# joejep/FOCNeRF

Measured on AMD Instinct MI355X. Metric: train_samples_per_sec, higher is better.
Workload: dtype f16

## Files before the change

focnerf_amd/_lib.py:

```python
import ctypes
import os

import torch

_HERE = os.path.dirname(os.path.abspath(__file__))
LIB_PATH = os.environ.get("FOCNERF_LIB_PATH") or os.path.join(_HERE, "libfocnerf_hip.so")

c_u8p = ctypes.c_void_p
c_vp = ctypes.c_void_p
u32 = ctypes.c_uint32
u64 = ctypes.c_uint64
f32 = ctypes.c_float
f64 = ctypes.c_double
i32 = ctypes.c_int

FOC_F32 = 0
FOC_F16 = 1
FOC_U8 = 2


class FocOccTrainNode(ctypes.Structure):
    _fields_ = [
        ("struct_bytes", u32),
        ("n_rays", u32), ("max_steps", u32), ("cascade", u32), ("grid_size", u32), ("cap", u32), ("pad_align", u32),
# ... 33 lines not shown
        ("ray_sumsq", c_vp),
        ("grad_sumsq", c_vp),
        ("grad_obj", c_vp),
    ]


class FocOccTrainTail(ctypes.Structure):
    _fields_ = [
        ("struct_bytes", u32),
        ("ray_dist", c_vp), ("ray_wm", c_vp), ("depth_raw", c_vp),
        ("grad_dist", c_vp), ("grad_depth", c_vp),
    ]


class FocCulledField(ctypes.Structure):
    _fields_ = [
        ("mask", c_vp), ("offsets", c_vp), ("sigma_c", c_vp), ("rgb_c", c_vp),
        ("m_occ", u32), ("density_scale", f32), ("thresh", f32), ("sigma_gain", f32),
    ]


class FocOptimTensor(ctypes.Structure):
    _fields_ = [
        ("param", c_vp), ("grad", c_vp), ("exp_avg", c_vp), ("exp_avg_sq", c_vp), ("step", c_vp),
        ("lr_tensor", c_vp),
        ("n", ctypes.c_int64),
        ("lr", f64), ("beta1", f64), ("beta2", f64), ("eps", f64), ("weight_decay", f64),
    ]


class FocOptimStep(ctypes.Structure):
    _fields_ = [
        ("struct_bytes", u32),
        ("tensor_bytes", u32),
        ("n_tensors", ctypes.c_int32),
        ("phase", u32), ("zero_grads", u32),
        ("growth_interval", ctypes.c_int32),
        ("growth_factor", f32), ("backoff_factor", f32),
        ("tensors", ctypes.POINTER(FocOptimTensor)),
        ("scale", c_vp),
        ("growth_tracker", c_vp),
        ("grad_scale", c_vp), ("found_inf", c_vp),
        ("workspace", c_vp),
        ("workspace_bytes", u64),
    ]


SIGNATURES = {
    "foc_abi_version": (i32, []),
    "foc_last_error": (ctypes.c_char_p, []),
    "foc_arch": (ctypes.c_char_p, []),
    "foc_near_far_from_aabb": (i32, [c_vp, c_vp, c_vp, u32, f32, c_vp, c_vp, c_vp]),
    "foc_sph_from_ray": (i32, [c_vp, c_vp, f32, u32, c_vp, c_vp]),
    "foc_morton3D": (i32, [c_vp, u32, c_vp, c_vp]),
    "foc_morton3D_invert": (i32, [c_vp, u32, c_vp, c_vp]),
    "foc_packbits": (i32, [c_vp, u32, f32, c_vp, c_vp]),
    "foc_march_rays_train": (i32, [c_vp, c_vp, c_vp, f32, f32, u32, u32, u32, u32, u32, c_vp, c_vp,
                                   c_vp, c_vp, c_vp, c_vp, c_vp, c_vp, c_vp, c_vp]),
    "foc_march_rays_train_field": (i32, [c_vp, c_vp, c_vp, f32, f32, u32, u32, u32, u32, u32, c_vp, c_vp,
                                         c_vp, c_vp, c_vp, c_vp, c_vp, c_vp, c_vp, u32, c_vp, f32, c_vp]),
    "foc_set_option": (i32, [ctypes.c_char_p, i32]),
    "foc_get_option": (i32, [ctypes.c_char_p, c_vp]),
    "foc_guard_pick_device": (i32, [i32, i32, i32, i32]),
    "foc_grid_forward_index_path": (i32, [u32, u32, u32]),
    "foc_view_tile_order": (i32, [c_vp, u32, u32, u32, c_vp, c_vp, c_vp]),
    "foc_occ_train_forward": (i32, [ctypes.POINTER(FocOccTrainNode), c_vp]),
    "foc_occ_train_backward": (i32, [ctypes.POINTER(FocOccTrainNode), c_vp]),
    "foc_occ_train_forward_pad31": (i32, [ctypes.POINTER(FocOccTrainNode), f32, c_vp]),
    "foc_occ_train_backward_pad31": (i32, [ctypes.POINTER(FocOccTrainNode), f32, c_vp]),
    "foc_occ_train_forward_obj": (i32, [ctypes.POINTER(FocOccTrainNode), ctypes.POINTER(FocOccTrainObject), c_vp]),
    "foc_occ_train_backward_obj": (i32, [ctypes.POINTER(FocOccTrainNode), ctypes.POINTER(FocOccTrainObject), c_vp]),
    "foc_occ_tail_forward_sumsq": (i32, [c_vp, c_vp, u32, c_vp, c_vp, u32, u32, f32, f32, c_vp, f32, c_vp, c_vp, c_vp, c_vp, c_vp, c_vp, c_vp, c_vp]),
    "foc_occ_tail_backward_sumsq": (i32, [c_vp, c_vp, c_vp, c_vp, u32, c_vp, c_vp, c_vp, c_vp, c_vp, u32, u32, f32, f32, c_vp, f32, c_vp, c_vp, c_vp, c_vp]),
    "foc_occ_tail_forward": (i32, [c_vp, c_vp, u32, c_vp, c_vp, u32, u32, f32, f32, c_vp, f32, c_vp, c_vp, c_vp, c_vp, c_vp, c_vp, c_vp]),
    "foc_occ_tail_backward": (i32, [c_vp, c_vp, c_vp, c_vp, u32, c_vp, c_vp, c_vp, c_vp, c_vp, u32, u32, f32, f32, c_vp, f32, c_vp, c_vp, c_vp]),
    "foc_occ_tail_forward_dist": (i32, [c_vp, c_vp, u32, c_vp, c_vp, u32, u32, f32, f32, c_vp, f32, c_vp, c_vp, c_vp, c_vp, c_vp, c_vp, c_vp, c_vp, c_vp,
                                        c_vp]),
    "foc_occ_tail_backward_dist": (i32, [c_vp, c_vp, c_vp, c_vp, u32, c_vp, c_vp, c_vp, c_vp, c_vp, u32, u32, f32, f32, c_vp, f32, c_vp, c_vp, c_vp, c_vp,
                                         c_vp, c_vp, c_vp]),
    "foc_occ_tail_forward_depth": (i32, [c_vp, c_vp, u32, c_vp, c_vp, u32, u32, f32, f32, c_vp, f32, c_vp, c_vp, c_vp, c_vp, c_vp, c_vp, c_vp, c_vp, c_vp,
                                         c_vp, c_vp]),
    "foc_occ_tail_backward_depth": (i32, [c_vp, c_vp, c_vp, c_vp, u32, c_vp, c_vp, c_vp, c_vp, c_vp, u32, u32, f32, f32, c_vp, f32, c_vp, c_vp, c_vp, c_vp,
                                          c_vp, c_vp, c_vp, c_vp, c_vp, c_vp, c_vp]),
    "foc_occ_train_forward_tail": (i32, [ctypes.POINTER(FocOccTrainNode), ctypes.POINTER(FocOccTrainObject), f32, ctypes.POINTER(FocOccTrainTail), c_vp]),
    "foc_occ_train_backward_tail": (i32, [ctypes.POINTER(FocOccTrainNode), ctypes.POINTER(FocOccTrainObject), f32, ctypes.POINTER(FocOccTrainTail), c_vp]),
    "foc_march_rays_train_scratch_bytes": (u64, [u32, u32]),
    "foc_composite_rays_train_forward": (i32, [c_vp, c_vp, c_vp, c_vp, u32, u32, f32, c_vp, c_vp, c_vp, c_vp]),
    "foc_composite_rays_train_backward": (i32, [c_vp, c_vp, c_vp, c_vp, c_vp, c_vp, c_vp, c_vp, u32, u32, f32,
                                                c_vp, c_vp, c_vp]),
    "foc_march_rays": (i32, [u32, u32, c_vp, c_vp, c_vp, c_vp, f32, f32, u32, u32, u32, c_vp, c_vp, c_vp,
                             c_vp, c_vp, c_vp, c_vp, c_vp]),
    "foc_composite_rays": (i32, [u32, u32, f32, c_vp, c_vp, c_vp, c_vp, c_vp, c_vp, c_vp, c_vp, c_vp]),
    "foc_compact_alive": (i32, [c_vp, u32, c_vp, c_vp, c_vp, c_vp]),
    "foc_march_rays_two_phase": (i32, [u32, u32, c_vp, c_vp, c_vp, c_vp, f32, f32, u32, u32, u32, c_vp, c_vp, c_vp, c_vp, c_vp, c_vp, c_vp, c_vp, i32, c_vp]),
    "foc_composite_compact": (i32, [u32, u32, f32, c_vp, c_vp, c_vp, c_vp, c_vp, c_vp, c_vp, c_vp, c_vp, c_vp, c_vp, c_vp, u32, u32, i32, c_vp]),
    "foc_march_rays_two_phase_fills": (i32, [u32, i32]),
    "foc_march_rays_two_phase_sample_major": (i32, [u32, u32, i32]),
    "foc_occ_render_step_scratch_bytes": (u64, [u32]),
    "foc_occ_render_step": (i32, [u32, u32, c_vp, c_vp, c_vp, c_vp, c_vp, c_vp, f32, f32, u32, u32, u32, c_vp, c_vp, c_vp, c_vp, c_vp, c_vp, c_vp, c_vp,
                                  c_vp, c_vp, c_vp, u32, f32, u32, c_vp, u32, c_vp, u32, u32, c_vp, f32, c_vp, c_vp, c_vp, c_vp, u32, c_vp, u32, u32, c_vp]),
    "foc_occ_render_step_pad31": (i32, [u32, u32, c_vp, c_vp, c_vp, c_vp, c_vp, c_vp, f32, f32, u32, u32, u32, c_vp, c_vp, c_vp, c_vp, c_vp, c_vp, c_vp, c_vp,
                                        c_vp, c_vp, c_vp, u32, f32, u32, c_vp, u32, c_vp, u32, u32, c_vp, f32, c_vp, c_vp, c_vp, c_vp, u32, c_vp, u32, u32, f32,
                                        c_vp]),
    "foc_occ_render_step_pad": (i32, [u32, u32, c_vp, c_vp, c_vp, c_vp, c_vp, c_vp, f32, f32, u32, u32, u32, c_vp, c_vp, c_vp, c_vp, c_vp, c_vp, c_vp, c_vp,
                                      c_vp, c_vp, c_vp, u32, f32, u32, c_vp, u32, c_vp, u32, u32, c_vp, f32, c_vp, c_vp, c_vp, c_vp, u32, c_vp, u32, u32, f32,
                                      c_vp]),
    "foc_grid_encode_forward": (i32, [c_vp, c_vp, c_vp, c_vp, u32, u32, u32, u32, f32, u32, c_vp, u32, i32, u32,
                                      i32, c_vp, c_vp]),
    "foc_grid_encode_forward_bl": (i32, [c_vp, c_vp, c_vp, c_vp, u32, u32, u32, u32, f32, u32, c_vp, u32, i32, u32,
                                         i32, c_vp, c_vp]),
    "foc_grid_encode_backward": (i32, [c_vp, c_vp, c_vp, c_vp, c_vp, u32, u32, u32, u32, f32, u32, c_vp, c_vp,
                                       u32, i32, u32, i32, i32, c_vp, c_vp]),
    "foc_grid_encode_backward_workspace_bytes": (u64, [u32, u32, u32, u32, i32]),
    "foc_grid_planes_to_rows": (i32, [c_vp, c_vp, u32, u32, u32, c_vp]),
    "foc_grid_rows_to_planes": (i32, [c_vp, c_vp, u32, u32, u32, c_vp]),
    "foc_grid_encode_backward_binned": (i32, [c_vp, c_vp, c_vp, c_vp, c_vp, u32, u32, u32, u32, f32, u32, c_vp, c_vp,
                                              u32, i32, u32, i32, i32, c_vp, c_vp, u64, c_vp]),
    "foc_grid_encode_forward_counted": (i32, [c_vp, c_vp, c_vp, c_vp, u32, u32, u32, u32, f32, u32, u32, i32, u32, i32, c_vp, c_vp, u64, c_vp]),
    "foc_grid_encode_backward_count": (i32, [c_vp, c_vp, u32, u32, u32, u32, f32, u32, u32, i32, u32, i32, c_vp, c_vp, u64, c_vp]),
    "foc_grid_encode_backward_binned_counted": (i32, [c_vp, c_vp, c_vp, c_vp, c_vp, u32, u32, u32, u32, f32, u32, c_vp, c_vp,
                                                      u32, i32, u32, i32, i32, c_vp, c_vp, u64, c_vp]),
    "foc_grad_total_variation": (i32, [c_vp, c_vp, c_vp, c_vp, f32, u32, u32, u32, u32, f32, u32, u32, i32, i32, c_vp]),
    "foc_freq_encode_forward": (i32, [c_vp, u32, u32, u32, u32, c_vp, c_vp]),
    "foc_freq_encode_backward": (i32, [c_vp, c_vp, u32, u32, u32, u32, c_vp, c_vp]),
    "foc_ffmlp_forward": (i32, [c_vp, c_vp, u32, u32, u32, u32, u32, u32, u32, c_vp, c_vp, c_vp]),
    "foc_ffmlp_inference": (i32, [c_vp, c_vp, u32, u32, u32, u32, u32, u32, u32, c_vp, c_vp, c_vp]),
    "foc_ffmlp_backward": (i32, [c_vp, c_vp, c_vp, c_vp, u32, u32, u32, u32, u32, u32, u32, i32,
                                 c_vp, c_vp, c_vp, c_vp, u64, c_vp]),
    "foc_ffmlp_backward_workspace_bytes": (u64, [u32, u32, u32]),
    "foc_ffmlp_forward_planar": (i32, [c_vp, c_vp, u32, u32, u32, u32, u32, u32, u32, c_vp, c_vp]),
    "foc_ffmlp_backward_planar": (i32, [c_vp, c_vp, c_vp, u32, u32, u32, u32, u32, u32, u32, i32, c_vp, c_vp, c_vp, u64, c_vp]),
    "foc_allocate_splitk": (i32, [u64]),
    "foc_free_splitk": (i32, []),
    "foc_combine_select": (i32, [c_vp, c_vp, c_vp, c_vp, u64, c_vp]),
    "foc_combine_pack_keys": (i32, [c_vp, u32, c_vp, u64, c_vp]),
    "foc_combine_unpack": (i32, [c_vp, u32, c_vp, c_vp, c_vp, u64, c_vp]),
    "foc_combine_select_composite": (i32, [c_vp, u32, c_vp, c_vp, u32, u32, c_vp, u32, c_vp, c_vp, c_vp, c_vp]),
    "foc_combine_select4": (i32, [c_vp, c_vp, u64, c_vp]),
    "foc_combine_select_composite_attr": (i32, [c_vp, u32, c_vp, c_vp, u32, c_vp, c_vp, u32, u32, c_vp, u32, c_vp, c_vp, c_vp, c_vp, c_vp, c_vp, c_vp, c_vp]),
    "foc_combine_select_composite_culled": (i32, [ctypes.POINTER(FocCulledField), u32, u32, c_vp, u32, c_vp, c_vp, u32, u32, c_vp, u32, c_vp, c_vp, c_vp, c_vp,
                                                  c_vp, c_vp, c_vp, c_vp]),
    "foc_combine_select4_ids": (i32, [c_vp, u32, c_vp, c_vp, u64, c_vp]),
    "foc_mo_select": (i32, [c_vp, c_vp, c_vp, c_vp, u64, u32, u32, c_vp]),
    "foc_fixed_field_pack": (i32, [c_vp, c_vp, c_vp, c_vp, c_vp, c_vp, f32, u32, u32, f32, f32, c_vp, c_vp, c_vp, c_vp, u32, c_vp]),
    "foc_fixed_cull_scratch_bytes": (u64, [u32, u32]),
    "foc_fixed_cull": (i32, [c_vp, c_vp, c_vp, c_vp, c_vp, u32, u32, f32, c_vp, u32, u32, c_vp, c_vp, c_vp, c_vp, u64, c_vp]),
    "foc_fixed_cull_emit": (i32, [c_vp, c_vp, c_vp, c_vp, c_vp, u32, u32, f32, c_vp, c_vp, u32, c_vp, c_vp, c_vp]),
    "foc_fixed_field_pack_culled": (i32, [c_vp, c_vp, c_vp, c_vp, u32, c_vp, c_vp, u32, u32, f32, f32, c_vp, c_vp]),
    "foc_fixed_cull_placed": (i32, [c_vp, c_vp, c_vp, c_vp, c_vp, u32, u32, c_vp, c_vp, f32, c_vp, u32, u32, c_vp, c_vp, c_vp, c_vp, u64, c_vp]),
    "foc_fixed_cull_emit_placed": (i32, [c_vp, c_vp, c_vp, c_vp, c_vp, u32, u32, c_vp, f32, f32, c_vp, c_vp, u32, c_vp, c_vp, c_vp]),
    "foc_fixed_field_pack_culled_gain": (i32, [c_vp, c_vp, c_vp, c_vp, u32, c_vp, c_vp, u32, u32, f32, f32, f32, c_vp, c_vp]),
    "foc_composite_fixed_steps":(i32, [c_vp, c_vp, c_vp, c_vp, u32, u32, f32, c_vp, c_vp, c_vp]),
    "foc_fixed_sample": (i32, [c_vp, c_vp, c_vp, c_vp, c_vp, c_vp, u32, u32, f32, c_vp, c_vp, c_vp, u32, c_vp]),
    "foc_fixed_tail_forward": (i32, [c_vp, c_vp, c_vp, c_vp, c_vp, c_vp, f32, u32, u32, f32, f32, c_vp, c_vp, c_vp, c_vp, c_vp, c_vp, u32, c_vp, c_vp]),
    "foc_fixed_tail_backward": (i32, [c_vp, c_vp, c_vp, c_vp, c_vp, c_vp, c_vp, c_vp, c_vp, c_vp, c_vp, f32, u32, u32, f32, f32, c_vp, c_vp, u32, c_vp, c_vp]),
    "foc_fixed_tail_forward_dist": (i32, [c_vp, c_vp, c_vp, c_vp, c_vp, c_vp, f32, u32, u32, f32, f32, c_vp, c_vp, c_vp, c_vp, c_vp, c_vp, u32, c_vp, c_vp,
                                          c_vp, c_vp]),
    "foc_fixed_tail_backward_dist": (i32, [c_vp, c_vp, c_vp, c_vp, c_vp, c_vp, c_vp, c_vp, c_vp, c_vp, c_vp, c_vp, f32, u32, u32, f32, f32, c_vp, c_vp, u32,
                                           c_vp, c_vp, c_vp, c_vp, c_vp]),
    "foc_fixed_head_forward": (i32, [c_vp, c_vp, c_vp, c_vp, c_vp, u32, u32, f32, c_vp, c_vp, c_vp, c_vp, c_vp, c_vp, c_vp, u32, c_vp]),
    "foc_fixed_head_backward": (i32, [c_vp, c_vp, c_vp, c_vp, c_vp, c_vp, c_vp, c_vp, c_vp, c_vp, u32, u32, f32, c_vp, u32, c_vp]),
    "foc_color_head_forward": (i32, [c_vp, c_vp, u32, c_vp, u32, u32, u32, u32, c_vp, u32, c_vp, c_vp]),
    "foc_field_forward_train": (i32, [c_vp, c_vp, u32, c_vp, u32, c_vp, u32, u32, u32, u32, c_vp, c_vp, u32, c_vp, c_vp]),
    "foc_color_head_backward": (i32, [c_vp, c_vp, c_vp, u32, c_vp, c_vp, u32, u32, u32, u32, c_vp, c_vp, c_vp, u64, u32, c_vp, c_vp, c_vp]),
    "foc_color_head_forward_pad": (i32, [c_vp, c_vp, u32, c_vp, u32, u32, u32, u32, c_vp, u32, c_vp, f32, c_vp]),
    "foc_color_head_backward_pad": (i32, [c_vp, c_vp, c_vp, u32, c_vp, c_vp, u32, u32, u32, u32, c_vp, c_vp, c_vp, u64, u32, c_vp, c_vp, f32, c_vp]),
    "foc_field_forward_train_pad": (i32, [c_vp, c_vp, u32, c_vp, u32, c_vp, u32, u32, u32, u32, c_vp, c_vp, u32, c_vp, f32, c_vp]),
    "foc_color_head_forward_pad31": (i32, [c_vp, c_vp, u32, c_vp, u32, u32, u32, u32, c_vp, u32, c_vp, f32, c_vp]),
    "foc_color_head_backward_pad31": (i32, [c_vp, c_vp, c_vp, u32, c_vp, c_vp, u32, u32, u32, u32, c_vp, c_vp, c_vp, u64, u32, c_vp, c_vp, f32, c_vp]),
    "foc_field_forward_train_pad31": (i32, [c_vp, c_vp, u32, c_vp, u32, c_vp, u32, u32, u32, u32, c_vp, c_vp, u32, c_vp, f32, c_vp]),
    "foc_fixed_composite_forward": (i32, [c_vp, c_vp, c_vp, f32, u32, u32, f32, c_vp, c_vp]),
    "foc_fixed_composite_backward": (i32, [c_vp, c_vp, c_vp, c_vp, f32, u32, u32, f32, c_vp, c_vp, c_vp]),
    "foc_sample_head_forward": (i32, [c_vp, c_vp, u64, c_vp, c_vp, c_vp, u32, c_vp]),
    "foc_sample_head_backward": (i32, [c_vp, c_vp, c_vp, u64, c_vp, u32, c_vp]),
    "foc_sh_encode": (i32, [c_vp, u64, c_vp, c_vp]),
    "foc_rgb_head_forward": (i32, [c_vp, u64, c_vp, c_vp]),
    "foc_rgb_head_backward": (i32, [c_vp, c_vp, u64, c_vp, c_vp]),
    "foc_fixed_render_inference": (i32, [c_vp, c_vp, c_vp, c_vp, c_vp, c_vp, f32, u32, u32, f32, f32, c_vp, c_vp, c_vp, c_vp, u32, c_vp, c_vp]),
    "foc_nerf_field_inference": (i32, [c_vp, i32, c_vp, u32, u32, u32, c_vp, u32, c_vp, u32, u32, u32, u32, c_vp, c_vp, c_vp, c_vp]),
    "foc_nerf_field_inference_pad": (i32, [c_vp, i32, c_vp, u32, u32, u32, c_vp, u32, c_vp, u32, u32, u32, u32, c_vp, c_vp, c_vp, f32, c_vp]),
    "foc_nerf_field_inference_pad31": (i32, [c_vp, i32, c_vp, u32, u32, u32, c_vp, u32, c_vp, u32, u32, u32, u32, c_vp, c_vp, c_vp, f32, c_vp]),
    "foc_field_normals": (i32, [c_vp, u32, c_vp, c_vp, u32, u32, u32, f32, u32, u32, i32, u32, i32, c_vp, c_vp, u32, u32, u32, c_vp, c_vp, c_vp, c_vp, c_vp,
                                c_vp]),
    "foc_mark_untrained_grid": (i32, [c_vp, u32, f32, f32, f32, f32, f32, u32, u32, c_vp, c_vp, c_vp]),
    "foc_grid_cells_xyz": (i32, [u32, u32, f32, c_vp, c_vp, c_vp]),
    "foc_grid_update_sample_workspace_bytes": (u64, [u32, u32]),
    "foc_grid_update_sample": (i32, [c_vp, u32, u32, f32, u32, c_vp, c_vp, c_vp, c_vp, c_vp, c_vp, u64, c_vp]),
    "foc_grid_update_apply_workspace_bytes": (u64, [u32, u32]),
    "foc_grid_update_apply": (i32, [c_vp, u32, u32, c_vp, c_vp, u32, f32, f32, f32, c_vp, c_vp, c_vp, u64, c_vp]),
    "foc_background_forward": (i32, [c_vp, c_vp, c_vp, f32, u32, c_vp, c_vp, f32, u32, c_vp, c_vp, c_vp]),
    "foc_background_backward_workspace_bytes": (u64, [u32]),
    "foc_background_backward": (i32, [c_vp, c_vp, c_vp, c_vp, f32, u32, c_vp, c_vp, f32, u32, c_vp, c_vp, c_vp, c_vp, u64, c_vp]),
    "foc_mc_workspace_bytes": (u64, [u32, u32, u32]),
    "foc_mc_count": (i32, [c_vp, u32, u32, u32, f32, c_vp, c_vp, c_vp]),
    "foc_mc_emit": (i32, [c_vp, u32, u32, u32, f32, c_vp, c_vp, c_vp, c_vp, c_vp, c_vp, c_vp]),
    "foc_lattice_cull_scratch_bytes": (u64, [u32]),
    "foc_lattice_cull": (i32, [c_vp, c_vp, c_vp, u32, u32, u32, u32, u32, c_vp, c_vp, f32, c_vp, u32, u32, c_vp, c_vp, c_vp, c_vp, u64, c_vp]),
    "foc_lattice_cull_emit": (i32, [c_vp, c_vp, c_vp, u32, u32, u32, u32, u32, c_vp, c_vp, c_vp, u32, c_vp, c_vp]),
    "foc_volume_scatter_max": (i32, [c_vp, c_vp, c_vp, f32, c_vp, u32, c_vp]),
    "foc_score_workspace_bytes": (u64, [u32, u32, u32]),
    "foc_score_quantize": (i32, [c_vp, c_vp, c_vp, c_vp, u32, u32, u32, c_vp, c_vp, c_vp, c_vp]),
    "foc_score_view": (i32, [c_vp, c_vp, u32, u32, u32, c_vp, u32, f64, f64, c_vp, c_vp, u64, c_vp]),
    "foc_optim_workspace_bytes": (ctypes.c_size_t, [i32]),
    "foc_optim_step": (i32, [ctypes.POINTER(FocOptimStep), c_vp]),
    "foc_philox4x32_10": (i32, [ctypes.POINTER(u32), ctypes.POINTER(u32), ctypes.POINTER(u32)]),
    "foc_batch_workspace_bytes": (u64, []),
    "foc_batch_sample": (i32, [c_vp, i32, u32, u32, u32, u32, c_vp, f32, f32, f32, f32, c_vp, c_vp, u64, u32, c_vp, i32, i32, c_vp, c_vp, c_vp, c_vp, c_vp, c_vp,
                               c_vp, u64, u32, c_vp]),
    "foc_view_rays": (i32, [c_vp, f32, f32, f32, f32, u32, u32, c_vp, c_vp, c_vp]),
    "foc_photo_loss_workspace_bytes": (u64, []),
    "foc_photo_loss": (i32, [c_vp, i32, c_vp, u32, i32, f32, c_vp, u32, c_vp, c_vp, c_vp, c_vp, c_vp, c_vp, u64, c_vp]),
}


def _load():
    if not os.path.exists(LIB_PATH):
        raise ImportError(
            f"focnerf_amd: {LIB_PATH} is missing. Build it with `python -c 'import __graft_entry__ as g; g.build()'` "
            f"or `make -C focnerf_amd/csrc`. There is no CPU or PyTorch fallback for these ops.")
    try:
        lib = ctypes.CDLL(LIB_PATH)
    except OSError as e:
        raise ImportError(f"focnerf_amd: failed to load {LIB_PATH}: {e}") from e
    for name, (res, args) in SIGNATURES.items():
        fn = getattr(lib, name)
        fn.restype = res
        fn.argtypes = args
    return lib


class _Stream(ctypes.c_void_p):
    device_index = None


_multi_device = None


def _on_tensor_device(fn):
    def call(*args):
        global _multi_device
        if _multi_device is None:
            _multi_device = torch.cuda.device_count() > 1
        if _multi_device and args:
            idx = getattr(args[-1], "device_index", None)
            if idx is not None and idx != torch.cuda.current_device():
                with torch.cuda.device(idx):
                    return fn(*args)
        return fn(*args)
    call.__name__ = getattr(fn, "__name__", "foc_call")
    return call


class _Lib:

    def __init__(self, cdll):
        self._cdll = cdll
        for name, (_, args) in SIGNATURES.items():
            fn = getattr(cdll, name)
            setattr(self, name, _on_tensor_device(fn) if args and args[-1] is c_vp and not name.endswith("_bytes") else fn)


lib = _Lib(_load())


def check(rc, what=""):
    if rc != 0:
        msg = lib.foc_last_error().decode("utf-8", "replace")
        raise RuntimeError(f"focnerf_amd {what}: {msg} (code {rc})")


def ptr(t):
    if t is None:
        return None
    return ctypes.c_void_p(t.data_ptr())


_raw_stream = getattr(torch._C, "_cuda_getCurrentRawStream", None) if os.environ.get("FOC_RAW_STREAM", "1") != "0" else None


def raw_stream(index):
    if _raw_stream is not None:
        return _raw_stream(index)
    return torch.cuda.current_stream(index).cuda_stream


def stream_of(t=None):
    dev = t.device if t is not None else None
    index = dev.index if dev is not None and dev.index is not None else torch.cuda.current_device()
    s = _Stream(raw_stream(index))
    s.device_index = index
    return s


def require_cuda(*tensors):
    for t in tensors:
        if t is not None and not t.is_cuda:
            raise RuntimeError("focnerf_amd: expected a CUDA(HIP) tensor; these ops have no CPU implementation")


def dtype_code(t):
    if t.dtype == torch.float32:
        return FOC_F32
    if t.dtype == torch.float16:
        return FOC_F16
    raise RuntimeError(f"focnerf_amd: unsupported dtype {t.dtype} (float32 or float16 expected)")


def get_option(name):
# ... 23 lines not shown
```

focnerf_amd/csrc/combine.hip:

```cpp
#include "common.h"
#include "fs_common.h"
#include <string.h>
#include <cmath>

static thread_local char g_err[512] = "";

void foc_set_error(const char *fmt, ...) {
    va_list ap;
    va_start(ap, fmt);
    vsnprintf(g_err, sizeof(g_err), fmt, ap);
    va_end(ap);
}

__global__ void __launch_bounds__(256) k_combine_select(const float *__restrict__ dens, const float *__restrict__ rgb,
                                                        float *__restrict__ max_dens, float *__restrict__ best_rgb, uint64_t n) {
    for (uint64_t i = (uint64_t)blockIdx.x * 256 + threadIdx.x; i < n; i += (uint64_t)gridDim.x * 256) {
        const float d = dens[i], m = max_dens[i];
        if (d > m) { best_rgb[i * 3] = rgb[i * 3]; best_rgb[i * 3 + 1] = rgb[i * 3 + 1]; best_rgb[i * 3 + 2] = rgb[i * 3 + 2]; }
        max_dens[i] = (d != d || m != m) ? __builtin_nanf("") : (d > m ? d : m);
    }
}

__global__ void __launch_bounds__(256) k_combine_pack(const float *__restrict__ dens, uint32_t rank, uint64_t *__restrict__ keys, uint64_t n) {
    for (uint64_t i = (uint64_t)blockIdx.x * 256 + threadIdx.x; i < n; i += (uint64_t)gridDim.x * 256) {
// ... 207 lines not shown
template <int KMAX> struct CulledObjs { CulledObj o[KMAX]; };

#define CC_NO_BIT 0xFFFFFFFFu
template <int KMAX, int NOBJ>
__global__ void __launch_bounds__(256) k_combine_culled(CulledObjs<KMAX> objs, CombineAttr at, uint32_t K, const float *__restrict__ nears,
                                                        const float *__restrict__ fars, uint32_t N, uint32_t T, float bg0, float bg1, uint32_t n_bg,
                                                        float *__restrict__ image4, float *__restrict__ depth, float4 *__restrict__ merged4) {
    const uint32_t lane = threadIdx.x & 63;
    const uint32_t n = __builtin_amdgcn_readfirstlane(blockIdx.x * 4 + (threadIdx.x >> 6));
    if (n >= N) return;
    const FsGeom geo = fs_geom(nears, fars, n, T);
    const uint32_t bit = n % FS_RAY_BLOCK;
    const uint64_t below = (1ull << bit) - 1ull;
    const uint64_t row0 = (uint64_t)(n / FS_RAY_BLOCK) * T;
    CombineAcc<NOBJ> A;
    combine_acc_init(A);
    float Tk[KMAX];
#pragma unroll
    for (int k = 0; k < KMAX; k++) Tk[k] = 1.0f;
    for (uint32_t base = 0; base < T; base += 64) {
        const uint32_t i = base + lane;
        const bool valid = i < T;
        const uint32_t ic = valid ? i : T - 1;
        const uint64_t row = row0 + ic, s = (uint64_t)n * T + ic;
        const FsSample p = fs_sample(geo, i, ic, T, false, 0.0f, 0.0f);
        uint32_t pre[KMAX];
        bool any = false, plain = fabsf(p.delta) < INFINITY && p.oz == p.oz;
#pragma unroll
        for (int k = 0; k < KMAX; k++) {
            pre[k] = CC_NO_BIT;
            if ((uint32_t)k < K) {
                const uint64_t m = objs.o[k].mask[row];
                if (valid && ((m >> bit) & 1ull)) { pre[k] = (uint32_t)__popcll(m & below); any = true; }
                plain = plain && fabsf(p.delta * objs.o[k].density_scale) < INFINITY;
            }
        }
        if (__ballot(any || !plain) == 0 && fabsf(A.Tc) < INFINITY) {
            if (valid) {
                uint32_t win = 0xFFu;
                if constexpr (NOBJ > 0) win = at.id[0];
                combine_store<NOBJ>(make_float4(0.0f, 0.0f, 0.0f, 0.0f), win, s, merged4, &at);
            }
            continue;
        }
        float4 best = make_float4(0.0f, 0.0f, 0.0f, 0.0f);
        uint32_t win = 0xFFu;
#pragma unroll
        for (int k = 0; k < KMAX; k++) {
            if ((uint32_t)k < K) {
                const CulledObj &o = objs.o[k];
                float sigma = 0, c0 = 0, c1 = 0, c2 = 0;
                if (pre[k] != CC_NO_BIT) {
                    const uint32_t slot = o.offsets[row] + pre[k];
                    if (slot < o.m_occ) {
                        sigma = o.sigma_c[slot];
                        if (o.sigma_gain != 1.0f) sigma *= o.sigma_gain;
                        c0 = o.rgb_c[(uint64_t)slot * 3]; c1 = o.rgb_c[(uint64_t)slot * 3 + 1]; c2 = o.rgb_c[(uint64_t)slot * 3 + 2];
                    }
                }
                const bool on = fs_infer_weight(Tk[k], p, valid, sigma, o.density_scale, lane) > o.thresh;
                const float4 f = make_float4(sigma, on ? c0 : 0.0f, on ? c1 : 0.0f, on ? c2 : 0.0f);
                if (k == 0) {
                    best = f;
                    if constexpr (NOBJ > 0) win = at.id[0];
                } else {
                    combine_select_step<NOBJ>(best, win, f, at.id[k]);
                }
            }
        }
        CombineSample q = combine_no_sample();
        if (valid) {
            combine_store<NOBJ>(best, win, s, merged4, &at);
            q = combine_take(best, win, p);
        }
        combine_accumulate(A, q, valid, lane);
    }
    combine_finish(A, &at, n, N, lane, bg0, bg1, n_bg, image4, depth);
}

struct CulledLaunch {
    const FocCulledField *objs; uint32_t K; CombineAttr at; const float *nears, *fars; uint32_t N, T; float bg0, bg1; uint32_t n_bg;
    float *image4, *depth; float4 *merged4; hipStream_t stream;
};
template <int KMAX, int NOBJ>
static void cc_launch(const CulledLaunch &L) {
    CulledObjs<KMAX> o;
    memset(&o, 0, sizeof(o));
    for (uint32_t k = 0; k < L.K; k++) {
        const FocCulledField &f = L.objs[k];
        o.o[k] = CulledObj{f.mask, f.offsets, f.sigma_c, f.rgb_c, f.m_occ, f.density_scale, f.thresh, f.sigma_gain};
    }
    hipLaunchKernelGGL((k_combine_culled<KMAX, NOBJ>), dim3(foc_div_up(L.N, 4)), dim3(256), 0, L.stream, o, L.at, L.K, L.nears, L.fars, L.N, L.T, L.bg0,
                       L.bg1, L.n_bg, L.image4, L.depth, L.merged4);
}
template <int KMAX>
static void cc_launch_k(const CulledLaunch &L, uint32_t n_obj) {
    if (n_obj == 0) cc_launch<KMAX, 0>(L);
    else if (n_obj <= 4) cc_launch<KMAX, 4>(L);
    else if (n_obj <= 8) cc_launch<KMAX, 8>(L);
    else cc_launch<KMAX, 16>(L);
}

__global__ void __launch_bounds__(256) k_combine_select4(const float4 *__restrict__ f4, float4 *__restrict__ acc4, uint64_t n) {
    for (uint64_t i = (uint64_t)blockIdx.x * 256 + threadIdx.x; i < n; i += (uint64_t)gridDim.x * 256) {
        const float4 f = f4[i];
        float4 best = acc4[i];
        const float m = best.x;
        if (f.x > m) { best.y = f.y; best.z = f.z; best.w = f.w; }
        best.x = (f.x != f.x || m != m) ? __builtin_nanf("") : (f.x > m ? f.x : m);
        acc4[i] = best;
    }
}

__global__ void __launch_bounds__(256) k_combine_select4_ids(const float4 *__restrict__ f4, uint8_t id, float4 *__restrict__ acc4,
                                                             uint8_t *__restrict__ acc_ids, uint64_t n) {
    for (uint64_t i = (uint64_t)blockIdx.x * 256 + threadIdx.x; i < n; i += (uint64_t)gridDim.x * 256) {
        const float4 f = f4[i];
        float4 best = acc4[i];
        const float m = best.x;
        if (f.x > m) { best.y = f.y; best.z = f.z; best.w = f.w; acc_ids[i] = id; }
        best.x = (f.x != f.x || m != m) ? __builtin_nanf("") : (f.x > m ? f.x : m);
        acc4[i] = best;
    }
}

template <typename T>
__global__ void __launch_bounds__(256) k_mo_select(const T *__restrict__ sig_new, const T *__restrict__ feat_new, T *__restrict__ sig_best,
                                                   T *__restrict__ feat_best, uint64_t n, uint32_t width) {
    const uint64_t s0 = ((uint64_t)blockIdx.x * 4u + (threadIdx.x >> 6)) * 64u;
    if (s0 >= n) return;
    const uint32_t lane = threadIdx.x & 63u;
    bool take = false;
    if (s0 + lane < n) {
        const T a_raw = sig_new[s0 + lane];
        const float a = (float)a_raw, b = (float)sig_best[s0 + lane];
        take = (a != a) || (b == b && a >= b);
        if (take) sig_best[s0 + lane] = a_raw;
    }
    const uint64_t rows = __ballot(take);
    const uint32_t live = (uint32_t)(n - s0 < 64u ? n - s0 : 64u);
    const uint64_t base = s0 * width;
    for (uint32_t e = lane; e < live * width; e += 64u)
        if ((rows >> (e / width)) & 1ull) feat_best[base + e] = feat_new[base + e];
}

#include <stdlib.h>
#include <string.h>
#include <atomic>
#include <mutex>
struct FocOptionRow { const char *name; std::atomic<int> value; };
static FocOptionRow foc_option_table[FOC_OPT_COUNT] = {
    {"FOC_MLP_BWD_FUSED", 1}, {"FOC_FIELD_FWD_FUSED", 1}, {"FOC_GB_MERGE_MAX_RES", 480}, {"FOC_GB_FACTORED", 1}, {"FOC_GB_TAIL_SPLIT", 16}, {"FOC_GRID_FUSE_SMALL", 1},
    {"FOC_GRID_PAIRS", 1}, {"FOC_GRID_FAST", 1}, {"FOC_MARCH_SERIAL", -1}, {"FOC_MARCH_RAYS_ROW_MAX", 131072}, {"FOC_OCC_MARCH_FORM", -1},
    {"FOC_OCC_SAMPLE_MAJOR", 1}, {"FOC_OCC_FIELD_PIECE", 1 << 23}, {"FOC_DETERMINISTIC", 0},
};
static int foc_option_parse(int which, const char *text) {
    if (which == FOC_OPT_OCC_MARCH_FORM) {
        if (text[0] == 't') return 0;
        if (text[0] == 'r') return 1;
        if (text[0] == 'l') return 2;
        if (text[0] == 's') return 3;
    }
    return atoi(text);
}
static void foc_options_init() {
    static std::once_flag once;
    std::call_once(once, [] {
        for (int i = 0; i < FOC_OPT_COUNT; i++) {
            const char *e = getenv(foc_option_table[i].name);
            if (e && e[0]) foc_option_table[i].value.store(foc_option_parse(i, e), std::memory_order_relaxed);
        }
    });
}
int foc_opt(FocOpt which) { foc_options_init(); return foc_option_table[which].value.load(std::memory_order_relaxed); }

extern "C" {

int foc_set_option(const char *name, int value) {
    foc_options_init();
    for (int i = 0; i < FOC_OPT_COUNT; i++)
        if (name && strcmp(name, foc_option_table[i].name) == 0) { foc_option_table[i].value.store(value, std::memory_order_relaxed); return FOC_OK; }
    foc_set_error("set_option: unknown option '%s'", name ? name : "(null)");
    return FOC_E_INVALID;
}

int foc_get_option(const char *name, int *value) {
    foc_options_init();
    for (int i = 0; i < FOC_OPT_COUNT; i++)
        if (name && value && strcmp(name, foc_option_table[i].name) == 0) { *value = foc_option_table[i].value.load(std::memory_order_relaxed); return FOC_OK; }
    foc_set_error("get_option: unknown option '%s'", name ? name : "(null)");
    return FOC_E_INVALID;
}

int foc_guard_pick_device(int stream_is_null, int stream_device, int pointer_device, int current_device) {
    return foc_guard_pick(stream_is_null != 0, stream_device, pointer_device, current_device);
}


int foc_combine_select_composite(const float *const *fields4, uint32_t K, const float *nears, const float *fars, uint32_t N, uint32_t T,
                                 const float *bgs, uint32_t n_bg, float *image4, float *depth, float *merged4, void *stream) {
    FocDeviceGuard foc_guard_(stream, nears);
    FOC_REQUIRE(K >= 1 && K <= FOC_COMBINE_MAX_OBJECTS, FOC_E_INVALID, "combine_select_composite: 1 <= K <= %d objects per call (got %u)",
                FOC_COMBINE_MAX_OBJECTS, K);
    FOC_REQUIRE(n_bg >= 1 && n_bg <= 2 && bgs, FOC_E_INVALID, "combine_select_composite: one or two backgrounds");
    FOC_REQUIRE(T >= 2, FOC_E_INVALID, "combine_select_composite: T must be >= 2");
    if (N == 0) return FOC_OK;
    FOC_REQUIRE(fields4 && nears && fars && image4 && depth, FOC_E_INVALID, "combine_select_composite: null pointer");
    CombineFields f;
    for (uint32_t k = 0; k < FOC_COMBINE_MAX_OBJECTS; k++) {
        f.p[k] = reinterpret_cast<const float4 *>(k < K ? fields4[k] : fields4[0]);
        FOC_REQUIRE(f.p[k] && ((uintptr_t)f.p[k] & 15) == 0, FOC_E_INVALID, "combine_select_composite: field %u is null or not 16-byte aligned", k);
    }
    FOC_REQUIRE(((uintptr_t)merged4 & 15) == 0, FOC_E_INVALID, "combine_select_composite: merged4 must be 16-byte aligned");
    hipLaunchKernelGGL(k_combine_select_composite, dim3(foc_div_up(N, 4)), dim3(256), 0, (hipStream_t)stream, f, K, nears, fars, N, T, bgs[0],
                       n_bg > 1 ? bgs[1] : 0.0f, n_bg, image4, depth, reinterpret_cast<float4 *>(merged4));
    FOC_CHECK_LAUNCH("combine_select_composite");
    return FOC_OK;
}

int foc_combine_select4(const float *field4, float *acc4, uint64_t n, void *stream) {
    FocDeviceGuard foc_guard_(stream, field4);
    FOC_REQUIRE(n == 0 || (field4 && acc4), FOC_E_INVALID, "combine_select4: null pointer");
    FOC_REQUIRE((((uintptr_t)field4 | (uintptr_t)acc4) & 15) == 0, FOC_E_INVALID, "combine_select4: fields must be 16-byte aligned");
    if (n == 0) return FOC_OK;
    hipLaunchKernelGGL(k_combine_select4, dim3(foc_grid_1d(n, 256)), dim3(256), 0, (hipStream_t)stream, reinterpret_cast<const float4 *>(field4),
                       reinterpret_cast<float4 *>(acc4), n);
    FOC_CHECK_LAUNCH("combine_select4");
    return FOC_OK;
}

int foc_combine_select_composite_attr(const float *const *fields4, uint32_t K, const uint8_t *const *id_planes, const uint32_t *ids,
                                      uint32_t n_obj, const float *nears, const float *fars, uint32_t N, uint32_t T, const float *bgs,
                                      uint32_t n_bg, float *image4, float *depth, float *merged4, float *obj_weights, float *obj_depth,
                                      int32_t *instance, uint8_t *winner, void *stream) {
    FocDeviceGuard foc_guard_(stream, nears);
    FOC_REQUIRE(K >= 1 && K <= FOC_COMBINE_MAX_OBJECTS, FOC_E_INVALID, "combine_select_composite_attr: 1 <= K <= %d fields per call (got %u)",
                FOC_COMBINE_MAX_OBJECTS, K);
    FOC_REQUIRE(n_obj >= 1 && n_obj <= FOC_COMBINE_MAX_OBJECTS, FOC_E_INVALID, "combine_select_composite_attr: 1 <= n_obj <= %d objects (got %u)",
                FOC_COMBINE_MAX_OBJECTS, n_obj);
    FOC_REQUIRE(n_bg >= 1 && n_bg <= 2 && bgs, FOC_E_INVALID, "combine_select_composite_attr: one or two backgrounds");
    FOC_REQUIRE(T >= 2, FOC_E_INVALID, "combine_select_composite_attr: T must be >= 2");
    FOC_REQUIRE(fields4, FOC_E_INVALID, "combine_select_composite_attr: fields4 is null");
    CombineFields f;
    CombineAttr at;
    for (uint32_t k = 0; k < FOC_COMBINE_MAX_OBJECTS; k++) {
        const uint32_t j = k < K ? k : 0;
        at.plane[k] = id_planes ? id_planes[j] : nullptr;
        FOC_REQUIRE(at.plane[k] || ids, FOC_E_INVALID, "combine_select_composite_attr: field %u has neither an id plane nor a constant id (ids is null)", j);
        at.id[k] = at.plane[k] ? 0u : ids[j];
        FOC_REQUIRE(at.id[k] < n_obj, FOC_E_INVALID, "combine_select_composite_attr: ids[%u] = %u is not below n_obj = %u", j, at.id[k], n_obj);
    }
    if (N == 0) return FOC_OK;
    FOC_REQUIRE(nears && fars && image4 && depth, FOC_E_INVALID, "combine_select_composite_attr: null pointer");
    FOC_REQUIRE(obj_weights && obj_depth && instance, FOC_E_INVALID, "combine_select_composite_attr: obj_weights, obj_depth and instance must not be null");
    for (uint32_t k = 0; k < FOC_COMBINE_MAX_OBJECTS; k++) {
        f.p[k] = reinterpret_cast<const float4 *>(k < K ? fields4[k] : fields4[0]);
        FOC_REQUIRE(f.p[k] && ((uintptr_t)f.p[k] & 15) == 0, FOC_E_INVALID, "combine_select_composite_attr: field %u is null or not 16-byte aligned", k);
    }
    FOC_REQUIRE(((uintptr_t)merged4 & 15) == 0, FOC_E_INVALID, "combine_select_composite_attr: merged4 must be 16-byte aligned");
    FOC_REQUIRE(((uintptr_t)obj_weights & 3) == 0 && ((uintptr_t)obj_depth & 3) == 0 && ((uintptr_t)instance & 3) == 0, FOC_E_INVALID,
                "combine_select_composite_attr: obj_weights, obj_depth and instance must be 4-byte aligned");
    at.n_obj = n_obj;
    at.obj_weights = obj_weights; at.obj_depth = obj_depth; at.instance = instance; at.winner = winner;
    const dim3 grid(foc_div_up(N, 4)), block(256);
    const float bg1 = n_bg > 1 ? bgs[1] : 0.0f;
    float4 *m4 = reinterpret_cast<float4 *>(merged4);
    if (n_obj <= 4)
        hipLaunchKernelGGL(k_combine_select_composite_attr<4>, grid, block, 0, (hipStream_t)stream, f, at, K, nears, fars, N, T, bgs[0], bg1, n_bg, image4, depth, m4);
    else if (n_obj <= 8)
        hipLaunchKernelGGL(k_combine_select_composite_attr<8>, grid, block, 0, (hipStream_t)stream, f, at, K, nears, fars, N, T, bgs[0], bg1, n_bg, image4, depth, m4);
    else
        hipLaunchKernelGGL(k_combine_select_composite_attr<16>, grid, block, 0, (hipStream_t)stream, f, at, K, nears, fars, N, T, bgs[0], bg1, n_bg, image4, depth, m4);
    FOC_CHECK_LAUNCH("combine_select_composite_attr");
    return FOC_OK;
}

int foc_combine_select_composite_culled(const FocCulledField *objs, uint32_t K, uint32_t struct_bytes, const uint32_t *ids, uint32_t n_obj,
                                        const float *nears, const float *fars, uint32_t N, uint32_t T, const float *bgs, uint32_t n_bg, float *image4,
                                        float *depth, float *merged4, float *obj_weights, float *obj_depth, int32_t *instance, uint8_t *winner,
                                        void *stream) {
    const char *who = "combine_select_composite_culled";
    FocDeviceGuard foc_guard_(stream, nears);
    FOC_REQUIRE(K >= 1 && K <= FOC_COMBINE_MAX_OBJECTS, FOC_E_INVALID, "%s: 1 <= K <= %d objects per call (got %u)", who, FOC_COMBINE_MAX_OBJECTS, K);
    FOC_REQUIRE(struct_bytes == sizeof(FocCulledField), FOC_E_INVALID, "%s: FocCulledField of %u bytes, this library's has %u", who, struct_bytes,
                (uint32_t)sizeof(FocCulledField));
    FOC_REQUIRE(objs, FOC_E_INVALID, "%s: objs is null", who);
    FOC_REQUIRE(n_obj <= FOC_COMBINE_MAX_OBJECTS, FOC_E_INVALID, "%s: n_obj <= %d objects (got %u)", who, FOC_COMBINE_MAX_OBJECTS, n_obj);
    FOC_REQUIRE(n_bg >= 1 && n_bg <= 2 && bgs, FOC_E_INVALID, "%s: one or two backgrounds", who);
    FOC_REQUIRE(T >= 2, FOC_E_INVALID, "%s: T must be >= 2", who);
    FOC_REQUIRE((uint64_t)foc_div_up(N, FS_RAY_BLOCK) * FS_RAY_BLOCK * T < (1ull << 31), FOC_E_INVALID,
                "%s: ceil(N/64)*64*T must stay below 2^31 (foc_fixed_cull's limit)", who);
    CulledLaunch L;
    memset(&L.at, 0, sizeof(L.at));
    for (uint32_t k = 0; k < K; k++) {
        const FocCulledField &f = objs[k];
        FOC_REQUIRE(std::isfinite(f.sigma_gain) && f.sigma_gain > 0, FOC_E_INVALID, "%s: object %u: sigma_gain must be finite and > 0 (got %g)", who, k,
                    (double)f.sigma_gain);
        L.at.id[k] = ids ? ids[k] : k;
        FOC_REQUIRE(n_obj == 0 || L.at.id[k] < n_obj, FOC_E_INVALID, "%s: ids[%u] = %u is not below n_obj = %u", who, k, L.at.id[k], n_obj);
    }
    if (N == 0) return FOC_OK;
    FOC_REQUIRE(nears && fars && image4 && depth, FOC_E_INVALID, "%s: null pointer", who);
    FOC_REQUIRE(n_obj == 0 || (obj_weights && obj_depth && instance), FOC_E_INVALID, "%s: obj_weights, obj_depth and instance must not be null when n_obj > 0", who);
    for (uint32_t k = 0; k < K; k++) {
        const FocCulledField &f = objs[k];
        FOC_REQUIRE(f.mask && f.offsets, FOC_E_INVALID, "%s: object %u: null pointer (mask / offsets)", who, k);
        FOC_REQUIRE(f.m_occ == 0 || (f.sigma_c && f.rgb_c), FOC_E_INVALID, "%s: object %u: null sigma / rgb with %u occupied samples", who, k, f.m_occ);
// ... 93 lines not shown
```

focnerf_amd/csrc/common.h:

```cpp
#pragma once
#include <hip/hip_runtime.h>
#include <hip/hip_fp16.h>
#include <stdint.h>
#include <stdio.h>
#include <stdarg.h>
#include <map>
#include <mutex>
#include <tuple>
#include "../../include/focnerf.h"

#define FOC_WAVE 64

void foc_set_error(const char *fmt, ...);

enum FocOpt {
    FOC_OPT_MLP_BWD_FUSED,
    FOC_OPT_FIELD_FWD_FUSED,
    FOC_OPT_GB_MERGE_MAX_RES,
    FOC_OPT_GB_FACTORED,
    FOC_OPT_GB_TAIL_SPLIT,
    FOC_OPT_GRID_FUSE_SMALL,
    FOC_OPT_GRID_PAIRS,
    FOC_OPT_GRID_FAST,
    FOC_OPT_MARCH_SERIAL,
    FOC_OPT_MARCH_RAYS_ROW_MAX,
    FOC_OPT_OCC_MARCH_FORM,
    FOC_OPT_OCC_SAMPLE_MAJOR,
    FOC_OPT_OCC_FIELD_PIECE,
    FOC_OPT_DETERMINISTIC,
    FOC_OPT_COUNT
};
int foc_opt(FocOpt which);

#define FOC_REQUIRE(cond, code, ...)                    \
    do {                                                \
        if (!(cond)) {                                  \
            foc_set_error(__VA_ARGS__);                 \
            return (code);                              \
        }                                               \
    } while (0)

#define FOC_CHECK_LAUNCH(name)                                                     \
    do {                                                                           \
        hipError_t e_ = hipGetLastError();                                         \
        if (e_ != hipSuccess) {                                                    \
            foc_set_error("%s: launch failed: %s", name, hipGetErrorString(e_));   \
            return FOC_E_LAUNCH;                                                   \
        }                                                                          \
    } while (0)

static inline int foc_guard_pick(bool stream_is_null, int stream_device, int pointer_device, int current_device) {
    if (!stream_is_null && stream_device >= 0) return stream_device;
    if (pointer_device >= 0) return pointer_device;
    return current_device;
}
struct FocDeviceGuard {
    int prev = -1;
    explicit FocDeviceGuard(void *stream, const void *first_pointer = nullptr) {
        static int n_devices = -1;
        if (n_devices < 0 && hipGetDeviceCount(&n_devices) != hipSuccess) { (void)hipGetLastError(); n_devices = 0; }
        if (n_devices == 1) return;
        int cur = 0;
        if (hipGetDevice(&cur) != hipSuccess) return;
        int sdev = -1, pdev = -1;
        if (stream != nullptr) {
            if (hipStreamGetDevice(static_cast<hipStream_t>(stream), &sdev) != hipSuccess) { (void)hipGetLastError(); sdev = -1; }
        } else if (first_pointer != nullptr) {
            hipPointerAttribute_t attr;
            if (hipPointerGetAttributes(&attr, first_pointer) == hipSuccess && attr.type == hipMemoryTypeDevice) pdev = attr.device;
            else (void)hipGetLastError();
        }
        const int want = foc_guard_pick(stream == nullptr, sdev, pdev, cur);
        if (want != cur && hipSetDevice(want) == hipSuccess) prev = cur;
    }
    ~FocDeviceGuard() { if (prev >= 0) (void)hipSetDevice(prev); }
    FocDeviceGuard(const FocDeviceGuard &) = delete;
    FocDeviceGuard &operator=(const FocDeviceGuard &) = delete;
};

static inline uint32_t foc_div_up(uint64_t a, uint64_t b) { return (uint32_t)((a + b - 1) / b); }

static inline uint32_t foc_grid_1d(uint64_t n, uint32_t block, uint32_t max_blocks = 256 * 8) {
    uint64_t g = (n + block - 1) / block;
    if (g < 1) g = 1;
    if (g > max_blocks) g = max_blocks;
    return (uint32_t)g;
}

static inline int foc_current_device() {
    int dev = 0;
    if (hipGetDevice(&dev) != hipSuccess || dev < 0) dev = 0;
    return dev;
}
static inline uint32_t foc_num_cus(int dev = foc_current_device()) {
    static std::mutex mu;
    static std::map<int, uint32_t> cus;
    std::lock_guard<std::mutex> lock(mu);
    uint32_t &n = cus[dev];
    if (!n) {
        int v = 0;
        if (hipDeviceGetAttribute(&v, hipDeviceAttributeMultiprocessorCount, dev) != hipSuccess || v <= 0) v = 256;
        n = (uint32_t)v;
    }
    return n;
}
static inline uint32_t foc_resident_blocks(const void *kern, uint32_t block, size_t lds, int dev = foc_current_device()) {
    static std::mutex mu;
    static std::map<std::tuple<int, const void *, uint32_t, size_t>, uint32_t> seen;
    std::lock_guard<std::mutex> lock(mu);
    uint32_t &n = seen[std::make_tuple(dev, kern, block, lds)];
    if (!n) {
        int v = 0;
        if (hipOccupancyMaxActiveBlocksPerMultiprocessor(&v, kern, (int)block, lds) != hipSuccess || v < 1) v = 2;
        n = (uint32_t)(v > 8 ? 8 : v);
    }
    return n;
}
template <typename K>
static inline uint32_t foc_persistent_grid(K kern, uint32_t block, size_t lds, uint32_t grid, uint32_t per_cu = 0) {
    const void *k = reinterpret_cast<const void *>(kern);
    if (lds > 64 * 1024) (void)hipFuncSetAttribute(k, hipFuncAttributeMaxDynamicSharedMemorySize, (int)lds);
    const int dev = foc_current_device();
    const uint32_t cap = foc_num_cus(dev) * (per_cu ? per_cu : foc_resident_blocks(k, block, lds, dev));
    return grid < cap ? grid : cap;
}

__device__ __forceinline__ _Float16 foc_f2h(float v) { asm volatile("" : "+v"(v)); return (_Float16)v; }

__global__ static void __launch_bounds__(256) k_foc_zero(uint32_t *__restrict__ p, uint64_t n_words) {
    for (uint64_t i = (uint64_t)blockIdx.x * 256 + threadIdx.x; i < n_words; i += (uint64_t)gridDim.x * 256) p[i] = 0u;
}
static inline hipError_t foc_zero_async(void *p, size_t bytes, hipStream_t st) {
    const uint64_t n = bytes / 4;
    if (n == 0) return hipSuccess;
    uint64_t blocks = (n + 255) / 256;
    if (blocks > 4096) blocks = 4096;
    hipLaunchKernelGGL(k_foc_zero, dim3((uint32_t)blocks), dim3(256), 0, st, reinterpret_cast<uint32_t *>(p), n);
    return hipGetLastError();
}

__device__ __forceinline__ void foc_lds_barrier() { asm volatile("s_waitcnt lgkmcnt(0)\n\ts_barrier" ::: "memory"); }

__device__ __forceinline__ float wave_sum(float v) {
#pragma unroll
    for (int o = 32; o > 0; o >>= 1) v += __shfl_xor(v, o, 64);
    return v;
}
__device__ __forceinline__ int wave_sum_i(int v) {
#pragma unroll
    for (int o = 32; o > 0; o >>= 1) v += __shfl_xor(v, o, 64);
    return v;
}
__device__ __forceinline__ float wave_incl_prod(float v, int lane) {
#pragma unroll
    for (int o = 1; o < 64; o <<= 1) {
        float u = __shfl_up(v, o, 64);
        if (lane >= o) v *= u;
    }
    return v;
}
__device__ __forceinline__ float wave_prod_scan(float om, uint32_t lane, float &P) {
    P = wave_incl_prod(om, (int)lane);
    float Pex = __shfl_up(P, 1, 64);
    if (lane == 0) Pex = 1.0f;
    return Pex;
}
__device__ __forceinline__ float wave_incl_sum(float v, int lane) {
#pragma unroll
    for (int o = 1; o < 64; o <<= 1) {
        float u = __shfl_up(v, o, 64);
        if (lane >= o) v += u;
    }
    return v;
}
__device__ __forceinline__ int wave_incl_sum_i(int v, int lane) {
#pragma unroll
    for (int o = 1; o < 64; o <<= 1) {
        int u = __shfl_up(v, o, 64);
        if (lane >= o) v += u;
    }
    return v;
}
// ... 1 lines not shown
```

focnerf_amd/csrc/fixedstep.hip:

```cpp
#include "common.h"
#include "fs_common.h"
#include <float.h>

__global__ void __launch_bounds__(256) k_fs_sample(const float *__restrict__ rays_o, const float *__restrict__ rays_d, const float *__restrict__ nears,
                                                   const float *__restrict__ fars, const float *__restrict__ aabb, const float *__restrict__ noise,
                                                   uint32_t N, uint32_t T, float bound, float *__restrict__ xyzs, float *__restrict__ enc_in,
                                                   _Float16 *__restrict__ ray_sh, uint32_t ray_block) {
    const uint64_t total = ray_block ? (uint64_t)((N + FS_RAY_BLOCK - 1) / FS_RAY_BLOCK) * FS_RAY_BLOCK * T : (uint64_t)N * T;
    const FsBox box = fs_box(aabb);
    const float two_b = 2 * bound;
    for (uint64_t s = (uint64_t)blockIdx.x * 256 + threadIdx.x; s < total; s += (uint64_t)gridDim.x * 256) {
        uint32_t n, i;
        bool own = true;
        if (ray_block) {
            const uint32_t blk = (uint32_t)(s / ((uint64_t)FS_RAY_BLOCK * T)), in = (uint32_t)(s - (uint64_t)blk * FS_RAY_BLOCK * T);
            i = in / FS_RAY_BLOCK;
            n = blk * FS_RAY_BLOCK + in % FS_RAY_BLOCK;
            own = n < N;
            n = own ? n : N - 1;
        } else {
            n = (uint32_t)(s / T); i = (uint32_t)(s - (uint64_t)n * T);
        }
        const FsGeom g = fs_geom(nears, fars, n, T);
        const float z = fs_z(g, i, T, noise, (uint64_t)n * T + i);
        float x, y, w;
        fs_point(rays_o[n * 3], rays_o[n * 3 + 1], rays_o[n * 3 + 2], rays_d[n * 3], rays_d[n * 3 + 1], rays_d[n * 3 + 2], z, box, x, y, w);
        if (xyzs) { xyzs[s * 3] = x; xyzs[s * 3 + 1] = y; xyzs[s * 3 + 2] = w; }
        if (enc_in) { enc_in[s * 3] = fs_norm(x, bound, two_b); enc_in[s * 3 + 1] = fs_norm(y, bound, two_b); enc_in[s * 3 + 2] = fs_norm(w, bound, two_b); }
        if (ray_sh && i == 0 && own) {
            h8 lo, hi;
            foc_sh16_h(rays_d[n * 3], rays_d[n * 3 + 1], rays_d[n * 3 + 2], lo, hi);
            h8 *dst = reinterpret_cast<h8 *>(ray_sh + (uint64_t)n * 16);
            dst[0] = lo; dst[1] = hi;
        }
    }
}

__global__ void __launch_bounds__(256) k_fs_head_fwd(const _Float16 *__restrict__ h, const float *__restrict__ rays_d, const float *__restrict__ nears,
                                                     const float *__restrict__ fars, const float *__restrict__ noise, uint32_t N, uint32_t T,
                                                     float density_scale, float *__restrict__ sigma_out, float *__restrict__ trans_out,
                                                     float *__restrict__ weights_out, float *__restrict__ weights_sum, float *__restrict__ depth,
                                                     _Float16 *__restrict__ cin, const _Float16 *__restrict__ obj, uint32_t cin_ld) {
    const uint32_t lane = threadIdx.x & 63;
    const uint32_t n = blockIdx.x * 4 + (threadIdx.x >> 6);
    if (n >= N) return;
    const FsGeom g = fs_geom(nears, fars, n, T);
    h8 shlo, shhi;
    h8 ob1 = {0, 0, 0, 0, 0, 0, 0, 0}, ob2 = {0, 0, 0, 0, 0, 0, 0, 0};
    _Float16 ob0 = (_Float16)0;
    if (cin) {
        foc_sh16_h(rays_d[n * 3], rays_d[n * 3 + 1], rays_d[n * 3 + 2], shlo, shhi);
        if (obj) {
            ob0 = obj[0];
#pragma unroll
            for (int k = 0; k < 8; k++) ob1[k] = obj[1 + k];
#pragma unroll
            for (int k = 0; k < 7; k++) ob2[k] = obj[9 + k];
        }
    }
    float Tc = 1.0f, ws = 0, dp = 0;
    for (uint32_t base = 0; base < T; base += 64) {
        const uint32_t i = base + lane;
        const bool valid = i < T;
        const uint64_t s = (uint64_t)n * T + (valid ? i : T - 1);
        h8 r0, r1;
        if (cin) { r0 = *reinterpret_cast<const h8 *>(h + s * 16); r1 = *reinterpret_cast<const h8 *>(h + s * 16 + 8); }
        else r0[0] = h[s * 16];
        const float sigma = expf((float)r0[0]);
        const FsSample p = fs_sample_ld(g, i, valid ? i : T - 1, T, noise, s);
        const float alpha = valid ? 1 - expf((-p.delta * density_scale) * sigma) : 0.0f;
        const float om = valid ? (1 - alpha + 1e-15f) : 1.0f;
        const float Tb = fs_trans_scan(om, lane, Tc);
        const float w = alpha * Tb;
        if (valid) {
            sigma_out[s] = sigma; trans_out[s] = Tb; weights_out[s] = w;
            ws += w; dp += w * p.oz;
            if (cin) {
                h8 c2, c3;
#pragma unroll
                for (int k = 0; k < 7; k++) { c2[k] = r0[k + 1]; c3[k] = r1[k + 1]; }
                c2[7] = r1[0]; c3[7] = ob0;
                h8 *dst = reinterpret_cast<h8 *>(cin + s * cin_ld);
                dst[0] = shlo; dst[1] = shhi; dst[2] = c2; dst[3] = c3;
                if (cin_ld == 48) { dst[4] = ob1; dst[5] = ob2; }
            }
        }
    }
    ws = wave_sum(ws); dp = wave_sum(dp);
    if (lane == 0) { weights_sum[n] = ws; depth[n] = dp; }
}

__global__ void __launch_bounds__(256) k_fs_head_bwd(const _Float16 *__restrict__ h, const float *__restrict__ sigma_in, const float *__restrict__ trans_in,
                                                     const float *__restrict__ nears, const float *__restrict__ fars, const float *__restrict__ noise,
                                                     const float *__restrict__ grad_w, const float *__restrict__ grad_ws, const float *__restrict__ grad_depth,
                                                     const _Float16 *__restrict__ grad_cin, uint32_t N, uint32_t T, float density_scale,
                                                     _Float16 *__restrict__ grad_h, uint32_t cin_ld) {
    const uint32_t lane = threadIdx.x & 63;
    const uint32_t n = blockIdx.x * 4 + (threadIdx.x >> 6);
    if (n >= N) return;
    const FsGeom g = fs_geom(nears, fars, n, T);
    const float gws = grad_ws ? grad_ws[n] : 0.0f, gdp = grad_depth ? grad_depth[n] : 0.0f;
    float S_carry = 0.0f;
    const uint32_t n_chunks = (T + 63) / 64;
    for (uint32_t cidx = n_chunks; cidx-- > 0;) {
        const uint32_t i = cidx * 64 + lane;
        const bool valid = i < T;
        const uint64_t s = (uint64_t)n * T + (valid ? i : T - 1);
        const float sigma = sigma_in[s], Tb = trans_in[s];
        const FsSample p = fs_sample_ld(g, i, valid ? i : T - 1, T, noise, s);
        const float dsigma = fs_head_bwd_step(p, valid, sigma, Tb, (grad_w ? grad_w[s] : 0.0f) + gws, gdp, density_scale, lane, S_carry);
        const float dh0 = dsigma * foc_trunc_exp_bwd((float)h[s * 16]);
        if (valid) {
            h8 o0, o1;
            if (grad_cin) {
                const h8 c2 = *reinterpret_cast<const h8 *>(grad_cin + s * cin_ld + 16), c3 = *reinterpret_cast<const h8 *>(grad_cin + s * cin_ld + 24);
#pragma unroll
                for (int k = 0; k < 7; k++) { o0[k + 1] = c2[k]; o1[k + 1] = c3[k]; }
                o1[0] = c2[7];
            } else {
#pragma unroll
                for (int k = 0; k < 8; k++) { o0[k] = (_Float16)0; o1[k] = (_Float16)0; }
            }
            o0[0] = foc_f2h(dh0);
            h8 *dst = reinterpret_cast<h8 *>(grad_h + s * 16);
            dst[0] = o0; dst[1] = o1;
        }
    }
}

__global__ void __launch_bounds__(256) k_fs_composite_fwd(const _Float16 *__restrict__ c, const float *__restrict__ weights, const float *__restrict__ bg_ray,
                                                          float bg_scalar, uint32_t N, uint32_t T, float thresh, float *__restrict__ image) {
    const uint32_t lane = threadIdx.x & 63;
    const uint32_t n = blockIdx.x * 4 + (threadIdx.x >> 6);
    if (n >= N) return;
    float r = 0, g = 0, b = 0, ws = 0;
    for (uint32_t i = lane; i < T; i += 64) {
        const uint64_t s = (uint64_t)n * T + i;
        const float w = weights[s];
        ws += w;
        if (w > thresh) {
            const uint2 raw = *reinterpret_cast<const uint2 *>(c + s * 16);
            const _Float16 *cc = reinterpret_cast<const _Float16 *>(&raw);
            r += w * foc_sigmoid_h((float)cc[0]); g += w * foc_sigmoid_h((float)cc[1]); b += w * foc_sigmoid_h((float)cc[2]);
        }
    }
    r = wave_sum(r); g = wave_sum(g); b = wave_sum(b); ws = wave_sum(ws);
    if (lane == 0) {
        const FocBg bg = foc_bg(bg_ray, bg_scalar, n);
        image[n * 3] = r + (1 - ws) * bg.b0; image[n * 3 + 1] = g + (1 - ws) * bg.b1; image[n * 3 + 2] = b + (1 - ws) * bg.b2;
    }
}

__global__ void __launch_bounds__(256) k_fs_composite_bwd(const float *__restrict__ grad_image, const _Float16 *__restrict__ c, const float *__restrict__ weights,
                                                          const float *__restrict__ bg_ray, float bg_scalar, uint32_t N, uint32_t T, float thresh,
                                                          _Float16 *__restrict__ grad_c, float *__restrict__ grad_w) {
    const uint64_t total = (uint64_t)N * T;
    for (uint64_t s = (uint64_t)blockIdx.x * 256 + threadIdx.x; s < total; s += (uint64_t)gridDim.x * 256) {
        const uint32_t n = (uint32_t)(s / T);
        const FsRayGrad q = fs_ray_grad(grad_image, bg_ray, bg_scalar, n);
        h8 o0;
        const h8 o1 = {0, 0, 0, 0, 0, 0, 0, 0};
        grad_w[s] = fs_composite_bwd_sample(q, weights[s], thresh, c + s * 16, o0);
        h8 *dst = reinterpret_cast<h8 *>(grad_c + s * 16);
        dst[0] = o0; dst[1] = o1;
    }
}

template <bool NOISE, bool DIST>
__global__ void __launch_bounds__(256) k_fs_tail_fwd(const _Float16 *__restrict__ h, const _Float16 *__restrict__ c, const float *__restrict__ nears,
                                                     const float *__restrict__ fars, const float *__restrict__ noise, const float *__restrict__ bg_ray,
                                                     float bg_scalar, uint32_t N, uint32_t T, float density_scale, float thresh,
                                                     float *__restrict__ sigma_out, float *__restrict__ trans_out, float *__restrict__ weights_out,
                                                     float *__restrict__ weights_sum, float *__restrict__ depth, float *__restrict__ image, uint32_t c_ld,
                                                     float *__restrict__ ray_sumsq, float *__restrict__ ray_dist, float *__restrict__ ray_wm) {
    const uint32_t lane = threadIdx.x & 63;
    const uint32_t n = blockIdx.x * 4 + (threadIdx.x >> 6);
    if (n >= N) return;
    const FsGeom g = fs_geom(nears, fars, n, T);
    float Tc = 1.0f, ws = 0, dp = 0, r = 0, gg = 0, b = 0, sq = 0;
    FsDist dist = {0, 0, 0};
    const bool live = g.far > g.near;
    for (uint32_t base = 0; base < T; base += 64) {
        const uint32_t i = base + lane;
        const bool valid = i < T;
        const uint32_t ic = valid ? i : T - 1;
        const uint64_t s = (uint64_t)n * T + ic;
        const _Float16 h0 = h[s * 16];
        const uint2 raw = *reinterpret_cast<const uint2 *>(c + s * c_ld);
        float u0 = 0.0f, u1 = 0.0f;
        if (NOISE) { u0 = noise[s]; u1 = noise[(uint64_t)n * T + min(ic + 1u, T - 1u)]; }
        const float sigma = expf((float)h0);
        const FsSample p = fs_sample(g, i, ic, T, NOISE, u0, u1);
        const float alpha = valid ? 1 - expf((-p.delta * density_scale) * sigma) : 0.0f;
        const float om = valid ? (1 - alpha + 1e-15f) : 1.0f;
        const float Tb = fs_trans_scan(om, lane, Tc);
        const float w = alpha * Tb;
        if constexpr (DIST) {
            if (live) fs_dist_fwd_step(dist, w, fs_dist_m(g, p), p.delta, lane);
        }
        if (valid) {
            sigma_out[s] = sigma; trans_out[s] = Tb; weights_out[s] = w;
            ws += w; dp += w * p.oz; sq = fmaf(sigma, sigma, sq);
            if (w > thresh) {
                const _Float16 *cc = reinterpret_cast<const _Float16 *>(&raw);
                r += w * foc_sigmoid_h((float)cc[0]); gg += w * foc_sigmoid_h((float)cc[1]); b += w * foc_sigmoid_h((float)cc[2]);
            }
        }
    }
    ws = wave_sum(ws); dp = wave_sum(dp); r = wave_sum(r); gg = wave_sum(gg); b = wave_sum(b);
    if (ray_sumsq) {
        sq = wave_sum(sq);
        if (lane == 0) ray_sumsq[n] = sq;
    }
    if constexpr (DIST) {
        const float ds = wave_sum(dist.acc);
        if (lane == 0) { ray_dist[n] = ds; ray_wm[n] = dist.WM; }
    }
    if (lane == 0) {
        const FocBg bg = foc_bg(bg_ray, bg_scalar, n);
        image[n * 3] = r + (1 - ws) * bg.b0; image[n * 3 + 1] = gg + (1 - ws) * bg.b1; image[n * 3 + 2] = b + (1 - ws) * bg.b2;
        weights_sum[n] = ws; depth[n] = dp;
    }
}

template <bool NOISE, bool DIST>
__global__ void __launch_bounds__(256) k_fs_tail_bwd(const float *__restrict__ grad_image, const float *__restrict__ grad_ws, const float *__restrict__ grad_depth,
                                                     const _Float16 *__restrict__ c, const float *__restrict__ sigma_in, const float *__restrict__ trans_in,
                                                     const float *__restrict__ weights, const float *__restrict__ nears, const float *__restrict__ fars,
                                                     const float *__restrict__ noise, const float *__restrict__ bg_ray, float bg_scalar, uint32_t N, uint32_t T,
                                                     float density_scale, float thresh, _Float16 *__restrict__ grad_c, _Float16 *__restrict__ grad_h0, uint32_t c_ld,
                                                     const float *__restrict__ grad_sumsq, const float *__restrict__ weights_sum,
                                                     const float *__restrict__ ray_wm, const float *__restrict__ grad_dist) {
    const uint32_t lane = threadIdx.x & 63;
    const uint32_t n = blockIdx.x * 4 + (threadIdx.x >> 6);
    if (n >= N) return;
    const FsGeom g = fs_geom(nears, fars, n, T);
    const float gws = grad_ws ? grad_ws[n] : 0.0f, gdp = grad_depth ? grad_depth[n] : 0.0f;
    const float gsq2 = grad_sumsq ? 2.0f * grad_sumsq[n] : 0.0f;
    float gdist = 0.0f, W_total = 0.0f, WM_total = 0.0f;
    FsDist dist = {0, 0, 0};
    if constexpr (DIST) {
        if (g.far > g.near) gdist = grad_dist[n];
        W_total = weights_sum[n]; WM_total = ray_wm[n];
    }
    const FsRayGrad q = fs_ray_grad(grad_image, bg_ray, bg_scalar, n);
    const FocExp15 e15 = foc_exp15();
    float S_carry = 0.0f;
    const uint32_t n_chunks = (T + 63) / 64;
    for (uint32_t cidx = n_chunks; cidx-- > 0;) {
        const uint32_t i = cidx * 64 + lane;
        const bool valid = i < T;
        const uint32_t ic = valid ? i : T - 1;
        const uint64_t s = (uint64_t)n * T + ic;
        const float sigma = sigma_in[s], Tb = trans_in[s], w = weights[s];
        const uint2 raw = *reinterpret_cast<const uint2 *>(c + s * c_ld);
        float u0 = 0.0f, u1 = 0.0f;
        if (NOISE) { u0 = noise[s]; u1 = noise[(uint64_t)n * T + min(ic + 1u, T - 1u)]; }
        h8 o0;
        const h8 o1 = {0, 0, 0, 0, 0, 0, 0, 0};
        const float gw = fs_composite_bwd_sample(q, w, thresh, reinterpret_cast<const _Float16 *>(&raw), o0);
        if (valid) {
            if (c_ld == 4u) *reinterpret_cast<uint2 *>(grad_c + s * 4) = *reinterpret_cast<const uint2 *>(&o0);
            else { h8 *dst = reinterpret_cast<h8 *>(grad_c + s * 16); dst[0] = o0; dst[1] = o1; }
        }
        const FsSample p = fs_sample(g, i, ic, T, NOISE, u0, u1);
        float gi = gw + gws;
        if constexpr (DIST) {
            if (gdist != 0.0f) gi = fmaf(gdist, fs_dist_bwd_step(dist, valid ? w : 0.0f, fs_dist_m(g, p), p.delta, W_total, WM_total, lane), gi);
        }
        float dsigma = fs_head_bwd_step(p, valid, sigma, Tb, gi, gdp, density_scale, lane, S_carry);
        if (gsq2 != 0.0f) dsigma = fmaf(gsq2, sigma, dsigma);
        const float dh0 = dsigma * foc_trunc_exp_bwd_of_sigma(sigma, e15);
        if (valid) grad_h0[s] = foc_f2h(dh0);
    }
}


template <bool PACK>
__device__ __forceinline__ void fs_infer_finish(FsRayAcc &a, uint32_t n, uint32_t lane, const float *__restrict__ bg_ray, float bg_scalar,
                                                float *__restrict__ image, float *__restrict__ depth, float *__restrict__ weights_sum) {
    const float ws = wave_sum(a.ws), dp = wave_sum(a.dp), r = wave_sum(a.r), gg = wave_sum(a.g), b = wave_sum(a.b);
    if (lane == 0 && (!PACK || image)) {
        const FocBg bg = foc_bg(bg_ray, bg_scalar, n);
        image[n * 3] = r + (1 - ws) * bg.b0; image[n * 3 + 1] = gg + (1 - ws) * bg.b1; image[n * 3 + 2] = b + (1 - ws) * bg.b2;
        depth[n] = dp;
        weights_sum[n] = ws;
    }
}

template <bool PACK>
__global__ void __launch_bounds__(256) k_fs_render_infer(const float *__restrict__ sigma_in, const float *__restrict__ rgb_in, const float *__restrict__ nears,
                                                         const float *__restrict__ fars, const float *__restrict__ noise, const float *__restrict__ bg_ray,
                                                         float bg_scalar, uint32_t N, uint32_t T, float density_scale, float thresh,
                                                         float *__restrict__ image, float *__restrict__ depth, float *__restrict__ weights_sum,
                                                         float *__restrict__ rgb_masked, float4 *__restrict__ field4) {
    const uint32_t lane = threadIdx.x & 63;
    const uint32_t n = blockIdx.x * 4 + (threadIdx.x >> 6);
    if (n >= N) return;
    const FsGeom g = fs_geom(nears, fars, n, T);
    FsRayAcc a = {1.0f, 0, 0, 0, 0, 0};
    for (uint32_t base = 0; base < T; base += 64) {
        const uint32_t i = base + lane;
        const bool valid = i < T;
        const uint64_t s = (uint64_t)n * T + (valid ? i : T - 1);
        const float sigma = sigma_in[s];
        float c0 = 0, c1 = 0, c2 = 0;
        if (valid) { c0 = rgb_in[s * 3]; c1 = rgb_in[s * 3 + 1]; c2 = rgb_in[s * 3 + 2]; }
        fs_infer_tile<PACK>(a, g, n, i, lane, T, sigma, c0, c1, c2, noise, density_scale, thresh, rgb_masked, field4, nullptr);
    }
    fs_infer_finish<PACK>(a, n, lane, bg_ray, bg_scalar, image, depth, weights_sum);
}

#define FS_BLK_RAYS 16u
template <bool PACK>
__global__ void __launch_bounds__(1024) k_fs_render_infer_blk(const float *__restrict__ sigma_in, const float *__restrict__ rgb_in, const float *__restrict__ nears,
                                                              const float *__restrict__ fars, const float *__restrict__ noise, const float *__restrict__ bg_ray,
                                                              float bg_scalar, uint32_t N, uint32_t T, float density_scale, float thresh,
                                                              float *__restrict__ image, float *__restrict__ depth, float *__restrict__ weights_sum,
                                                              float *__restrict__ rgb_masked, float4 *__restrict__ field4, float *__restrict__ sigma_rm) {
    __shared__ float tile_s[64][FS_BLK_RAYS + 1];
    __shared__ float tile_c[64][FS_BLK_RAYS * 3 + 1];
    const uint32_t tid = threadIdx.x, lane = tid & 63;
    const uint32_t wv = __builtin_amdgcn_readfirstlane(tid >> 6);
    const uint32_t n0 = blockIdx.x * FS_BLK_RAYS;
    const uint64_t row0 = fs_block_row(n0, 0, T);
    const bool is_s = tid < 256;
    const uint32_t li = is_s ? tid : tid - 256;
    const uint32_t l_step = is_s ? li >> 2 : li / 12, l_part = is_s ? (li & 3) : li % 12;
    const float *src = is_s ? sigma_in + row0 + l_part * 4 : rgb_in + row0 * 3 + l_part * 4;
    const uint32_t src_ld = is_s ? FS_RAY_BLOCK : FS_RAY_BLOCK * 3;
    float *dst = is_s ? &tile_s[l_step][l_part * 4] : &tile_c[l_step][l_part * 4];
    float4 nx = make_float4(0, 0, 0, 0);
    if (l_step < T) nx = *reinterpret_cast<const float4 *>(src + (uint64_t)l_step * src_ld);
    const uint32_t n = n0 + wv;
    const bool own = n < N;
    const FsGeom g = fs_geom(nears, fars, own ? n : N - 1, T);
    FsRayAcc a = {1.0f, 0, 0, 0, 0, 0};
    for (uint32_t base = 0; base < T; base += 64) {
        dst[0] = nx.x; dst[1] = nx.y; dst[2] = nx.z; dst[3] = nx.w;
        __syncthreads();
        if (base + 64 + l_step < T) nx = *reinterpret_cast<const float4 *>(src + (uint64_t)(base + 64 + l_step) * src_ld);
        if (own)
            fs_infer_tile<PACK>(a, g, n, base + lane, lane, T, tile_s[lane][wv], tile_c[lane][wv * 3], tile_c[lane][wv * 3 + 1], tile_c[lane][wv * 3 + 2],
                                noise, density_scale, thresh, rgb_masked, field4, sigma_rm);
        __syncthreads();
    }
    if (own) fs_infer_finish<PACK>(a, n, lane, bg_ray, bg_scalar, image, depth, weights_sum);
}

struct VtState { uint32_t count, first_enc, bad, pad; };

__device__ __forceinline__ bool vt_turn(const float *__restrict__ d, uint32_t i) {
    const float ax = d[(i + 1) * 3] - d[i * 3], ay = d[(i + 1) * 3 + 1] - d[i * 3 + 1], az = d[(i + 1) * 3 + 2] - d[i * 3 + 2];
    const float bx = d[(i + 2) * 3] - d[(i + 1) * 3], by = d[(i + 2) * 3 + 1] - d[(i + 1) * 3 + 1], bz = d[(i + 2) * 3 + 2] - d[(i + 1) * 3 + 2];
    return (bx * ax + by * ay) + bz * az < 0.0f;
}

__global__ void __launch_bounds__(256) k_vt_find(const float *__restrict__ d, uint32_t N, VtState *__restrict__ st) {
    for (uint32_t i = blockIdx.x * 256 + threadIdx.x; i + 2 < N; i += gridDim.x * 256)
        if (vt_turn(d, i)) { atomicAdd(&st->count, 1u); atomicMax(&st->first_enc, N - i); }
}

__global__ void __launch_bounds__(256) k_vt_check(const float *__restrict__ d, uint32_t N, VtState *__restrict__ st) {
    const uint32_t fe = st->first_enc;
    if (fe == 0u) return;
    const uint32_t W = N - fe + 2u;
    for (uint32_t i = blockIdx.x * 256 + threadIdx.x; i + 2 < N; i += gridDim.x * 256) {
        const bool expect = (i + 2u) % W == 0u || (i + 1u) % W == 0u;
        if (vt_turn(d, i) != expect) st->bad = 1u;
    }
}

__global__ void __launch_bounds__(256) k_vt_perm(uint32_t N, uint32_t th, uint32_t tw, const VtState *__restrict__ st, int64_t *__restrict__ perm) {
    const uint32_t fe = st->first_enc, W = fe ? N - fe + 2u : 0u;
    const uint32_t H = W ? N / W : 0u;
    const bool grid = W >= 16u && N % W == 0u && H >= 8u && st->count == 2u * (H - 1u) && st->bad == 0u;
    for (uint32_t p = blockIdx.x * 256 + threadIdx.x; p < N; p += gridDim.x * 256) {
        uint32_t src = p;
        if (grid) {
            const uint64_t wt = (uint64_t)W * th;
            const uint32_t ty = (uint32_t)(p / wt), rem = (uint32_t)(p - ty * wt);
            const uint32_t rows_here = min(th, H - ty * th);
            const uint32_t tx = min(rem / (rows_here * tw), (W - 1u) / tw), r2 = rem - tx * rows_here * tw;
            const uint32_t cols_here = min(tw, W - tx * tw);
            src = (ty * th + r2 / cols_here) * W + tx * tw + r2 % cols_here;
        }
        perm[p] = (int64_t)src;
    }
}

extern "C" {

int foc_fixed_sample(const float *rays_o, const float *rays_d, const float *nears, const float *fars, const float *aabb, const float *noise,
                     uint32_t N, uint32_t T, float bound, float *xyzs, float *enc_in, void *ray_sh, uint32_t ray_block, void *stream) {
    FocDeviceGuard foc_guard_(stream, rays_o);
    if (N == 0) return FOC_OK;
    FOC_REQUIRE(rays_o && rays_d && nears && fars && aabb && (xyzs || enc_in), FOC_E_INVALID, "fixed_sample: null pointer");
    FOC_REQUIRE(T >= 2, FOC_E_INVALID, "fixed_sample: T must be >= 2");
    FOC_REQUIRE(ray_block == 0 || ray_block == FS_RAY_BLOCK, FOC_E_INVALID, "fixed_sample: ray_block must be 0 (ray-major) or %u (got %u)", FS_RAY_BLOCK, ray_block);
    const uint64_t rows = ray_block ? (uint64_t)foc_div_up(N, FS_RAY_BLOCK) * FS_RAY_BLOCK * T : (uint64_t)N * T;
    hipLaunchKernelGGL(k_fs_sample, dim3(foc_grid_1d(rows, 256, 256 * 16)), dim3(256), 0, (hipStream_t)stream, rays_o, rays_d, nears, fars, aabb,
                       noise, N, T, bound, xyzs, enc_in, (_Float16 *)ray_sh, ray_block);
    FOC_CHECK_LAUNCH("fixed_sample");
    return FOC_OK;
}

int foc_fixed_head_forward(const void *h, const float *rays_d, const float *nears, const float *fars, const float *noise, uint32_t N, uint32_t T,
                           float density_scale, float *sigma, float *trans, float *weights, float *weights_sum, float *depth, void *cin,
                           const void *obj_feat, uint32_t cin_width, void *stream) {
    FocDeviceGuard foc_guard_(stream, h);
    if (N == 0) return FOC_OK;
    FOC_REQUIRE(h && rays_d && nears && fars && sigma && trans && weights && weights_sum && depth, FOC_E_INVALID, "fixed_head_forward: null pointer");
    FOC_REQUIRE(T >= 2, FOC_E_INVALID, "fixed_head_forward: T must be >= 2");
    FOC_REQUIRE(cin_width == 32 || cin_width == 48, FOC_E_INVALID, "fixed_head_forward: cin_width must be 32 or 48 (got %u)", cin_width);
    FOC_REQUIRE(!obj_feat || cin_width == 48, FOC_E_INVALID, "fixed_head_forward: an object feature needs the 48-wide colour input");
    hipLaunchKernelGGL(k_fs_head_fwd, dim3(foc_div_up(N, 4)), dim3(256), 0, (hipStream_t)stream, (const _Float16 *)h, rays_d, nears, fars, noise, N, T,
                       density_scale, sigma, trans, weights, weights_sum, depth, (_Float16 *)cin, (const _Float16 *)obj_feat, cin_width);
    FOC_CHECK_LAUNCH("fixed_head_forward");
    return FOC_OK;
}

int foc_fixed_head_backward(const void *h, const float *sigma, const float *trans, const float *nears, const float *fars, const float *noise,
                            const float *grad_w, const float *grad_ws, const float *grad_depth, const void *grad_cin, uint32_t N, uint32_t T,
                            float density_scale, void *grad_h, uint32_t cin_width, void *stream) {
    FocDeviceGuard foc_guard_(stream, h);
    if (N == 0) return FOC_OK;
    FOC_REQUIRE(h && sigma && trans && nears && fars && grad_h, FOC_E_INVALID, "fixed_head_backward: null pointer");
    FOC_REQUIRE(T >= 2, FOC_E_INVALID, "fixed_head_backward: T must be >= 2");
    FOC_REQUIRE(cin_width == 32 || cin_width == 48, FOC_E_INVALID, "fixed_head_backward: cin_width must be 32 or 48 (got %u)", cin_width);
    hipLaunchKernelGGL(k_fs_head_bwd, dim3(foc_div_up(N, 4)), dim3(256), 0, (hipStream_t)stream, (const _Float16 *)h, sigma, trans, nears, fars, noise,
                       grad_w, grad_ws, grad_depth, (const _Float16 *)grad_cin, N, T, density_scale, (_Float16 *)grad_h, cin_width);
    FOC_CHECK_LAUNCH("fixed_head_backward");
    return FOC_OK;
}

int foc_fixed_composite_forward(const void *c, const float *weights, const float *bg_ray, float bg_scalar, uint32_t N, uint32_t T, float thresh,
                                float *image, void *stream) {
    FocDeviceGuard foc_guard_(stream, c);
    if (N == 0) return FOC_OK;
    FOC_REQUIRE(c && weights && image, FOC_E_INVALID, "fixed_composite_forward: null pointer");
    hipLaunchKernelGGL(k_fs_composite_fwd, dim3(foc_div_up(N, 4)), dim3(256), 0, (hipStream_t)stream, (const _Float16 *)c, weights, bg_ray, bg_scalar, N, T,
                       thresh, image);
    FOC_CHECK_LAUNCH("fixed_composite_forward");
    return FOC_OK;
}

int foc_fixed_composite_backward(const float *grad_image, const void *c, const float *weights, const float *bg_ray, float bg_scalar, uint32_t N,
                                 uint32_t T, float thresh, void *grad_c, float *grad_w, void *stream) {
    FocDeviceGuard foc_guard_(stream, grad_image);
    if (N == 0) return FOC_OK;
    FOC_REQUIRE(grad_image && c && weights && grad_c && grad_w, FOC_E_INVALID, "fixed_composite_backward: null pointer");
    hipLaunchKernelGGL(k_fs_composite_bwd, dim3(foc_grid_1d((uint64_t)N * T, 256, 256 * 16)), dim3(256), 0, (hipStream_t)stream, grad_image,
                       (const _Float16 *)c, weights, bg_ray, bg_scalar, N, T, thresh, (_Float16 *)grad_c, grad_w);
    FOC_CHECK_LAUNCH("fixed_composite_backward");
    return FOC_OK;
}

static int fixed_tail_forward(const char *who, const void *h, const void *c, const float *nears, const float *fars, const float *noise, const float *bg_ray,
                              float bg_scalar, uint32_t N, uint32_t T, float density_scale, float thresh, float *sigma, float *trans, float *weights,
                              float *weights_sum, float *depth, float *image, uint32_t c_width, float *ray_sumsq, float *ray_dist, float *ray_wm, void *stream) {
    FocDeviceGuard foc_guard_(stream, h);
    if (N == 0) return FOC_OK;
    FOC_REQUIRE(c_width == 16 || c_width == 4, FOC_E_INVALID, "%s: c_width must be 16 or 4 (got %u)", who, c_width);
    FOC_REQUIRE(h && c && nears && fars && sigma && trans && weights && weights_sum && depth && image, FOC_E_INVALID, "%s: null pointer", who);
    FOC_REQUIRE(T >= 2, FOC_E_INVALID, "%s: T must be >= 2", who);
    auto kern = ray_dist ? (noise ? k_fs_tail_fwd<true, true> : k_fs_tail_fwd<false, true>) : (noise ? k_fs_tail_fwd<true, false> : k_fs_tail_fwd<false, false>);
    hipLaunchKernelGGL(kern, dim3(foc_div_up(N, 4)), dim3(256), 0, (hipStream_t)stream, (const _Float16 *)h, (const _Float16 *)c, nears, fars, noise,
                       bg_ray, bg_scalar, N, T, density_scale, thresh, sigma, trans, weights, weights_sum, depth, image, c_width, ray_sumsq, ray_dist, ray_wm);
    FOC_CHECK_LAUNCH(who);
    return FOC_OK;
}

int foc_fixed_tail_forward(const void *h, const void *c, const float *nears, const float *fars, const float *noise, const float *bg_ray, float bg_scalar,
                           uint32_t N, uint32_t T, float density_scale, float thresh, float *sigma, float *trans, float *weights, float *weights_sum,
                           float *depth, float *image, uint32_t c_width, float *ray_sumsq, void *stream) {
    return fixed_tail_forward("fixed_tail_forward", h, c, nears, fars, noise, bg_ray, bg_scalar, N, T, density_scale, thresh, sigma, trans, weights, weights_sum,
                              depth, image, c_width, ray_sumsq, nullptr, nullptr, stream);
}

int foc_fixed_tail_forward_dist(const void *h, const void *c, const float *nears, const float *fars, const float *noise, const float *bg_ray, float bg_scalar,
                                uint32_t N, uint32_t T, float density_scale, float thresh, float *sigma, float *trans, float *weights, float *weights_sum,
                                float *depth, float *image, uint32_t c_width, float *ray_sumsq, float *ray_dist, float *ray_wm, void *stream) {
    FOC_REQUIRE((ray_dist && ray_wm) || N == 0, FOC_E_INVALID, "fixed_tail_forward_dist: null ray_dist / ray_wm");
    return fixed_tail_forward("fixed_tail_forward_dist", h, c, nears, fars, noise, bg_ray, bg_scalar, N, T, density_scale, thresh, sigma, trans, weights,
                              weights_sum, depth, image, c_width, ray_sumsq, ray_dist, ray_wm, stream);
}

static int fixed_tail_backward(const char *who, const float *grad_image, const float *grad_ws, const float *grad_depth, const void *c, const float *sigma,
                               const float *trans, const float *weights, const float *nears, const float *fars, const float *noise, const float *bg_ray,
                               float bg_scalar, uint32_t N, uint32_t T, float density_scale, float thresh, void *grad_c, void *grad_h0, uint32_t c_width,
                               const float *grad_sumsq, const float *weights_sum, const float *ray_wm, const float *grad_dist, void *stream) {
    FocDeviceGuard foc_guard_(stream, grad_image);
    if (N == 0) return FOC_OK;
    FOC_REQUIRE(c_width == 16 || c_width == 4, FOC_E_INVALID, "%s: c_width must be 16 or 4 (got %u)", who, c_width);
    FOC_REQUIRE(grad_image && c && sigma && trans && weights && nears && fars && grad_c && grad_h0, FOC_E_INVALID, "%s: null pointer", who);
    FOC_REQUIRE(T >= 2, FOC_E_INVALID, "%s: T must be >= 2", who);
    auto kern = grad_dist ? (noise ? k_fs_tail_bwd<true, true> : k_fs_tail_bwd<false, true>) : (noise ? k_fs_tail_bwd<true, false> : k_fs_tail_bwd<false, false>);
    hipLaunchKernelGGL(kern, dim3(foc_div_up(N, 4)), dim3(256), 0, (hipStream_t)stream, grad_image, grad_ws, grad_depth, (const _Float16 *)c, sigma,
                       trans, weights, nears, fars, noise, bg_ray, bg_scalar, N, T, density_scale, thresh, (_Float16 *)grad_c, (_Float16 *)grad_h0, c_width,
                       grad_sumsq, weights_sum, ray_wm, grad_dist);
    FOC_CHECK_LAUNCH(who);
    return FOC_OK;
}

int foc_fixed_tail_backward(const float *grad_image, const float *grad_ws, const float *grad_depth, const void *c, const float *sigma, const float *trans,
                            const float *weights, const float *nears, const float *fars, const float *noise, const float *bg_ray, float bg_scalar,
                            uint32_t N, uint32_t T, float density_scale, float thresh, void *grad_c, void *grad_h0, uint32_t c_width, const float *grad_sumsq,
                            void *stream) {
    return fixed_tail_backward("fixed_tail_backward", grad_image, grad_ws, grad_depth, c, sigma, trans, weights, nears, fars, noise, bg_ray, bg_scalar, N, T,
                               density_scale, thresh, grad_c, grad_h0, c_width, grad_sumsq, nullptr, nullptr, nullptr, stream);
}

int foc_fixed_tail_backward_dist(const float *grad_image, const float *grad_ws, const float *grad_depth, const void *c, const float *sigma, const float *trans,
                                 const float *weights, const float *weights_sum, const float *nears, const float *fars, const float *noise, const float *bg_ray,
                                 float bg_scalar, uint32_t N, uint32_t T, float density_scale, float thresh, void *grad_c, void *grad_h0, uint32_t c_width,
                                 const float *grad_sumsq, const float *ray_wm, const float *ray_dist, const float *grad_dist, void *stream) {
    (void)ray_dist;
    FOC_REQUIRE(!grad_dist || (weights_sum && ray_wm) || N == 0, FOC_E_INVALID, "fixed_tail_backward_dist: grad_dist needs weights_sum and ray_wm");
    return fixed_tail_backward("fixed_tail_backward_dist", grad_image, grad_ws, grad_depth, c, sigma, trans, weights, nears, fars, noise, bg_ray, bg_scalar, N,
                               T, density_scale, thresh, grad_c, grad_h0, c_width, grad_sumsq, weights_sum, ray_wm, grad_dist, stream);
}

int foc_fixed_render_inference(const float *sigma, const float *rgb, const float *nears, const float *fars, const float *noise, const float *bg_ray,
                               float bg_scalar, uint32_t N, uint32_t T, float density_scale, float thresh, float *image, float *depth, float *weights_sum,
                               float *rgb_masked, uint32_t ray_block, float *sigma_raymajor, void *stream) {
    FocDeviceGuard foc_guard_(stream, sigma);
    if (N == 0) return FOC_OK;
    FOC_REQUIRE(sigma && rgb && nears && fars && image && depth && weights_sum, FOC_E_INVALID, "fixed_render_inference: null pointer");
    FOC_REQUIRE(T >= 2, FOC_E_INVALID, "fixed_render_inference: T must be >= 2");
    FOC_REQUIRE(ray_block == 0 || ray_block == FS_RAY_BLOCK, FOC_E_INVALID, "fixed_render_inference: ray_block must be 0 or %u (got %u)", FS_RAY_BLOCK, ray_block);
    FOC_REQUIRE(ray_block || !sigma_raymajor, FOC_E_INVALID, "fixed_render_inference: sigma_raymajor is the un-blocked copy of a blocked sigma (ray_block == 0: sigma already is ray-major)");
    if (ray_block) {
        FOC_REQUIRE((((uintptr_t)sigma | (uintptr_t)rgb) & 15) == 0, FOC_E_INVALID, "fixed_render_inference: blocked sigma / rgb must be 16-byte aligned");
        hipLaunchKernelGGL(k_fs_render_infer_blk<false>, dim3(foc_div_up(N, FS_BLK_RAYS)), dim3(1024), 0, (hipStream_t)stream, sigma, rgb, nears, fars, noise, bg_ray, bg_scalar,
                           N, T, density_scale, thresh, image, depth, weights_sum, rgb_masked, (float4 *)nullptr, sigma_raymajor);
        FOC_CHECK_LAUNCH("fixed_render_inference");
        return FOC_OK;
    }
    hipLaunchKernelGGL(k_fs_render_infer<false>, dim3(foc_div_up(N, 4)), dim3(256), 0, (hipStream_t)stream, sigma, rgb, nears, fars, noise, bg_ray, bg_scalar, N, T,
                       density_scale, thresh, image, depth, weights_sum, rgb_masked, (float4 *)nullptr);
    FOC_CHECK_LAUNCH("fixed_render_inference");
    return FOC_OK;
}

int foc_fixed_field_pack(const float *sigma, const float *rgb, const float *nears, const float *fars, const float *noise, const float *bg_ray,
                         float bg_scalar, uint32_t N, uint32_t T, float density_scale, float thresh, float *image, float *depth, float *weights_sum,
                         float *field4, uint32_t ray_block, void *stream) {
    FocDeviceGuard foc_guard_(stream, sigma);
    if (N == 0) return FOC_OK;
    FOC_REQUIRE(sigma && rgb && nears && fars && field4, FOC_E_INVALID, "fixed_field_pack: null pointer");
    FOC_REQUIRE((image && depth && weights_sum) || (!image && !depth && !weights_sum), FOC_E_INVALID,
                "fixed_field_pack: image, depth and weights_sum go together (all or none)");
    FOC_REQUIRE(((uintptr_t)field4 & 15) == 0, FOC_E_INVALID, "fixed_field_pack: field4 must be 16-byte aligned");
    FOC_REQUIRE(T >= 2, FOC_E_INVALID, "fixed_field_pack: T must be >= 2");
    FOC_REQUIRE(ray_block == 0 || ray_block == FS_RAY_BLOCK, FOC_E_INVALID, "fixed_field_pack: ray_block must be 0 or %u (got %u)", FS_RAY_BLOCK, ray_block);
    if (ray_block) {
        FOC_REQUIRE((((uintptr_t)sigma | (uintptr_t)rgb) & 15) == 0, FOC_E_INVALID, "fixed_field_pack: blocked sigma / rgb must be 16-byte aligned");
        hipLaunchKernelGGL(k_fs_render_infer_blk<true>, dim3(foc_div_up(N, FS_BLK_RAYS)), dim3(1024), 0, (hipStream_t)stream, sigma, rgb, nears, fars, noise, bg_ray, bg_scalar,
                           N, T, density_scale, thresh, image, depth, weights_sum, (float *)nullptr, (float4 *)field4, (float *)nullptr);
        FOC_CHECK_LAUNCH("fixed_field_pack");
        return FOC_OK;
    }
    hipLaunchKernelGGL(k_fs_render_infer<true>, dim3(foc_div_up(N, 4)), dim3(256), 0, (hipStream_t)stream, sigma, rgb, nears, fars, noise, bg_ray, bg_scalar, N, T,
                       density_scale, thresh, image, depth, weights_sum, (float *)nullptr, (float4 *)field4);
    FOC_CHECK_LAUNCH("fixed_field_pack");
    return FOC_OK;
}

int foc_view_tile_order(const float *rays_d, uint32_t N, uint32_t tile_h, uint32_t tile_w, int64_t *perm, void *state16, void *stream) {
    FocDeviceGuard foc_guard_(stream, rays_d);
    if (N == 0) return FOC_OK;
    FOC_REQUIRE(rays_d && perm && state16, FOC_E_INVALID, "view_tile_order: null pointer");
    FOC_REQUIRE(tile_h >= 1 && tile_w >= 1 && tile_h * tile_w <= 4096, FOC_E_INVALID, "view_tile_order: tile %u x %u", tile_h, tile_w);
    FOC_REQUIRE(N < (1u << 31), FOC_E_INVALID, "view_tile_order: N too large");
    hipStream_t st = (hipStream_t)stream;
    VtState *state = reinterpret_cast<VtState *>(state16);
    if (foc_zero_async(state, sizeof(VtState), st) != hipSuccess) { foc_set_error("view_tile_order: zero fill failed"); return FOC_E_LAUNCH; }
    if (N >= 3) {
        hipLaunchKernelGGL(k_vt_find, dim3(foc_grid_1d(N, 256)), dim3(256), 0, st, rays_d, N, state);
        hipLaunchKernelGGL(k_vt_check, dim3(foc_grid_1d(N, 256)), dim3(256), 0, st, rays_d, N, state);
    }
    hipLaunchKernelGGL(k_vt_perm, dim3(foc_grid_1d(N, 256)), dim3(256), 0, st, N, tile_h, tile_w, state, perm);
    FOC_CHECK_LAUNCH("view_tile_order");
    return FOC_OK;
}

}
```

focnerf_amd/csrc/fs_common.h:

```cpp
#pragma once
#include "common.h"
#include "sample_math.h"

struct FsGeom { float near, far, span, sample_dist, step; };

#define FS_RAY_BLOCK 64u
__host__ __device__ __forceinline__ uint64_t fs_block_row(uint32_t n, uint32_t i, uint32_t T) {
    return (uint64_t)(n / FS_RAY_BLOCK) * FS_RAY_BLOCK * T + (uint64_t)i * FS_RAY_BLOCK + n % FS_RAY_BLOCK;
}

__device__ __forceinline__ FsGeom fs_geom(const float *__restrict__ nears, const float *__restrict__ fars, uint32_t n, uint32_t T) {
    FsGeom g;
    g.near = nears[n]; g.far = fars[n];
    g.span = g.far - g.near;
    g.sample_dist = g.span / (float)T;
    g.step = 1.0f / (float)(T - 1);
    return g;
}
__device__ __forceinline__ float fs_z0(const FsGeom &g, uint32_t i, uint32_t T) {
    const float lin = (i < T / 2) ? (g.step * (float)i) : fmaf(-g.step, (float)(T - 1 - i), 1.0f);
    return g.near + g.span * lin;
}
__device__ __forceinline__ float fs_jitter(const FsGeom &g, float z, float u) { return z + (u - 0.5f) * g.sample_dist; }
__device__ __forceinline__ float fs_z(const FsGeom &g, uint32_t i, uint32_t T, const float *__restrict__ noise, uint64_t s) {
    float z = fs_z0(g, i, T);
    if (noise) z = fs_jitter(g, z, noise[s]);
    return z;
}
__device__ __forceinline__ float fs_zu(const FsGeom &g, uint32_t i, uint32_t T, bool jitter, float u) {
    float z = fs_z0(g, i, T);
    if (jitter) z = fs_jitter(g, z, u);
    return z;
}

struct FsSample { float z, delta, oz; };
__device__ __forceinline__ FsSample fs_sample(const FsGeom &g, uint32_t i, uint32_t ic, uint32_t T, bool jitter, float u0, float u1) {
    FsSample p;
    p.z = fs_zu(g, ic, T, jitter, u0);
    p.delta = g.sample_dist;
    if (i + 1 < T) p.delta = fs_zu(g, i + 1, T, jitter, u1) - p.z;
    p.oz = (p.z - g.near) / g.span;
    p.oz = p.oz < 0.0f ? 0.0f : (p.oz > 1.0f ? 1.0f : p.oz);
    return p;
}
__device__ __forceinline__ FsSample fs_sample_ld(const FsGeom &g, uint32_t i, uint32_t ic, uint32_t T, const float *__restrict__ noise, uint64_t s) {
    const bool jitter = noise != nullptr;
    return fs_sample(g, i, ic, T, jitter, jitter ? noise[s] : 0.0f, jitter && i + 1 < T ? noise[s + 1] : 0.0f);
}

__device__ __forceinline__ float fs_trans_scan(float om, uint32_t lane, float &Tc) {
    float P;
    const float Tb = Tc * wave_prod_scan(om, lane, P);
    Tc *= __shfl(P, 63, 64);
    return Tb;
}

__device__ __forceinline__ float wave_suffix_incl_sum(float v, int lane) {
#pragma unroll
    for (int o = 1; o < 64; o <<= 1) {
        const float u = __shfl_down(v, o, 64);
        if (lane + o < 64) v += u;
    }
    return v;
}
__device__ __forceinline__ float fs_head_bwd_step(const FsSample &p, bool valid, float sigma, float Tb, float gi, float gdp, float density_scale, uint32_t lane,
                                                  float &S_carry) {
    const float ex = expf((-p.delta * density_scale) * sigma);
    const float alpha = 1 - ex;
    const float om = 1 - alpha + 1e-15f;
    if (gdp != 0.0f) gi += gdp * p.oz;
    const float gw_i = valid ? gi * (alpha * Tb) : 0.0f;
    const float incl = wave_suffix_incl_sum(gw_i, (int)lane);
    const float S_i = S_carry + (incl - gw_i);
    const float dalpha = gi * Tb - S_i / om;
    S_carry += __shfl(incl, 0, 64);
    return dalpha * (p.delta * density_scale) * ex;
}

struct FsDist { float W, WM, acc; };
__device__ __forceinline__ float fs_dist_m(const FsGeom &g, const FsSample &p) { return (p.z - g.near) + 0.5f * p.delta; }
__device__ __forceinline__ void fs_dist_fwd_step(FsDist &d, float w, float m, float delta, uint32_t lane) {
    const float wm = w * m;
    const float iw = wave_incl_sum(w, (int)lane), iwm = wave_incl_sum(wm, (int)lane);
    float ew = __shfl_up(iw, 1, 64), ewm = __shfl_up(iwm, 1, 64);
    if (lane == 0) { ew = 0.0f; ewm = 0.0f; }
    const float Wb = d.W + ew, WMb = d.WM + ewm;
    d.acc += (1.0f / 3.0f) * delta * (w * w) + 2.0f * (w * (m * Wb - WMb));
    d.W += __shfl(iw, 63, 64); d.WM += __shfl(iwm, 63, 64);
}
__device__ __forceinline__ float fs_dist_bwd_step(FsDist &d, float w, float m, float delta, float W_total, float WM_total, uint32_t lane) {
    const float wm = w * m;
    const float iw = wave_suffix_incl_sum(w, (int)lane), iwm = wave_suffix_incl_sum(wm, (int)lane);
    float ew = __shfl_down(iw, 1, 64), ewm = __shfl_down(iwm, 1, 64);
    if (lane == 63) { ew = 0.0f; ewm = 0.0f; }
    const float Wa = d.W + ew, WMa = d.WM + ewm;
    const float Wb = (W_total - Wa) - w, WMb = (WM_total - WMa) - wm;
    d.W += __shfl(iw, 0, 64); d.WM += __shfl(iwm, 0, 64);
    return (2.0f / 3.0f) * delta * w + 2.0f * (m * (Wb - Wa) + (WMa - WMb));
}

struct FsRayGrad { float g0, g1, g2; FocBg bg; };
__device__ __forceinline__ FsRayGrad fs_ray_grad(const float *__restrict__ grad_image, const float *__restrict__ bg_ray, float bg_scalar, uint32_t n) {
    return FsRayGrad{grad_image[n * 3], grad_image[n * 3 + 1], grad_image[n * 3 + 2], foc_bg(bg_ray, bg_scalar, n)};
}
__device__ __forceinline__ float fs_composite_bwd_sample(const FsRayGrad &q, float w, float thresh, const _Float16 *cc, h8 &o0) {
    float gw = -(q.g0 * q.bg.b0 + q.g1 * q.bg.b1 + q.g2 * q.bg.b2);
#pragma unroll
    for (int k = 0; k < 8; k++) o0[k] = (_Float16)0;
    if (w > thresh) {
        const uint2 raw = *reinterpret_cast<const uint2 *>(cc);
        const _Float16 *y = reinterpret_cast<const _Float16 *>(&raw);
        const float y0 = foc_sigmoid_h((float)y[0]), y1 = foc_sigmoid_h((float)y[1]), y2 = foc_sigmoid_h((float)y[2]);
        gw += q.g0 * y0 + q.g1 * y1 + q.g2 * y2;
        o0[0] = foc_f2h(q.g0 * w * y0 * (1 - y0)); o0[1] = foc_f2h(q.g1 * w * y1 * (1 - y1)); o0[2] = foc_f2h(q.g2 * w * y2 * (1 - y2));
    }
    return gw;
}

struct FsBox { float a0, a1, a2, a3, a4, a5; };
__device__ __forceinline__ FsBox fs_box(const float *__restrict__ aabb) { return FsBox{aabb[0], aabb[1], aabb[2], aabb[3], aabb[4], aabb[5]}; }
__device__ __forceinline__ void fs_point(float ox, float oy, float oz, float dx, float dy, float dz, float z, const FsBox &b, float &x, float &y, float &w) {
    x = ox + dx * z; y = oy + dy * z; w = oz + dz * z;
    x = fminf(fmaxf(x, b.a0), b.a3); y = fminf(fmaxf(y, b.a1), b.a4); w = fminf(fmaxf(w, b.a2), b.a5);
}
__device__ __forceinline__ float fs_norm(float x, float bound, float two_b) { return (x + bound) / two_b; }

struct FsRayAcc { float Tc, ws, dp, r, g, b; };

__device__ __forceinline__ float fs_infer_weight(float &Tc, const FsSample &p, bool valid, float sigma, float density_scale, uint32_t lane) {
    const float alpha = valid ? 1 - expf((-p.delta * density_scale) * sigma) : 0.0f;
    const float om = valid ? (1 - alpha + 1e-15f) : 1.0f;
    return alpha * fs_trans_scan(om, lane, Tc);
}

template <bool PACK>
__device__ __forceinline__ void fs_infer_tile(FsRayAcc &a, const FsGeom &g, uint32_t n, uint32_t i, uint32_t lane, uint32_t T, float sigma, float c0, float c1,
                                              float c2, const float *__restrict__ noise, float density_scale, float thresh, float *__restrict__ rgb_masked,
                                              float4 *__restrict__ field4, float *__restrict__ sigma_rm) {
    const bool valid = i < T;
    const uint64_t s = (uint64_t)n * T + (valid ? i : T - 1);
    const FsSample p = fs_sample_ld(g, i, valid ? i : T - 1, T, noise, s);
    const float w = fs_infer_weight(a.Tc, p, valid, sigma, density_scale, lane);
    if (valid) {
        a.ws += w; a.dp += w * p.oz;
        const bool on = w > thresh;
        if (on) { a.r += w * c0; a.g += w * c1; a.b += w * c2; }
        if (rgb_masked) { rgb_masked[s * 3] = on ? c0 : 0.0f; rgb_masked[s * 3 + 1] = on ? c1 : 0.0f; rgb_masked[s * 3 + 2] = on ? c2 : 0.0f; }
        if (PACK) field4[s] = make_float4(sigma, on ? c0 : 0.0f, on ? c1 : 0.0f, on ? c2 : 0.0f);
        if (sigma_rm) sigma_rm[s] = sigma;
    }
}
```

focnerf_amd/csrc/raymarching.hip:

```cpp
#include "common.h"
#include "occ_cell.h"
#include "sample_math.h"
#include "ragged.h"
#include <float.h>

#define RM_SQRT3 1.7320508075688772f
#define RM_RPI   0.3183098861837907f

__device__ __forceinline__ float rm_sign(float x) { return copysignf(1.0f, x); }

__device__ __forceinline__ void rm_near_far(float ox, float oy, float oz, float dx, float dy, float dz, float a0, float a1, float a2, float a3, float a4, float a5,
                                            float min_near, float &near_out, float &far_out) {
    const float rdx = 1 / dx, rdy = 1 / dy, rdz = 1 / dz;
    float near = (a0 - ox) * rdx, far = (a3 - ox) * rdx, t;
    if (near > far) { t = near; near = far; far = t; }
    float near_y = (a1 - oy) * rdy, far_y = (a4 - oy) * rdy;
    if (near_y > far_y) { t = near_y; near_y = far_y; far_y = t; }
    bool miss = (near > far_y || near_y > far);
    if (!miss) {
        if (near_y > near) near = near_y;
        if (far_y < far) far = far_y;
        float near_z = (a2 - oz) * rdz, far_z = (a5 - oz) * rdz;
        if (near_z > far_z) { t = near_z; near_z = far_z; far_z = t; }
        miss = (near > far_z || near_z > far);
        if (!miss) {
            if (near_z > near) near = near_z;
            if (far_z < far) far = far_z;
            if (near < min_near) near = min_near;
        }
    }
    near_out = miss ? FLT_MAX : near;
    far_out = miss ? FLT_MAX : far;
}

__global__ void __launch_bounds__(256) k_near_far_from_aabb(const float *__restrict__ rays_o, const float *__restrict__ rays_d,
                                     const float *__restrict__ aabb, uint32_t N, float min_near,
                                     float *__restrict__ nears, float *__restrict__ fars) {
    const float a0 = aabb[0], a1 = aabb[1], a2 = aabb[2], a3 = aabb[3], a4 = aabb[4], a5 = aabb[5];
    for (uint32_t n = blockIdx.x * blockDim.x + threadIdx.x; n < N; n += gridDim.x * blockDim.x) {
        float near, far;
        rm_near_far(rays_o[n * 3], rays_o[n * 3 + 1], rays_o[n * 3 + 2], rays_d[n * 3], rays_d[n * 3 + 1], rays_d[n * 3 + 2], a0, a1, a2, a3, a4, a5, min_near, near, far);
        nears[n] = near;
        fars[n] = far;
    }
}

__global__ void __launch_bounds__(256) k_sph_from_ray(const float *__restrict__ rays_o, const float *__restrict__ rays_d, float radius,
                               uint32_t N, float *__restrict__ coords) {
    for (uint32_t n = blockIdx.x * blockDim.x + threadIdx.x; n < N; n += gridDim.x * blockDim.x) {
        const float ox = rays_o[n * 3], oy = rays_o[n * 3 + 1], oz = rays_o[n * 3 + 2];
        const float dx = rays_d[n * 3], dy = rays_d[n * 3 + 1], dz = rays_d[n * 3 + 2];
        const float A = fmaf(dz, dz, fmaf(dy, dy, dx * dx));
        const float B = fmaf(oz, dz, fmaf(oy, dy, ox * dx));
        const float C = fmaf(-radius, radius, fmaf(oz, oz, fmaf(oy, oy, ox * ox)));
        const float t = (-B + sqrtf(fmaf(B, B, -(A * C)))) / A;
        const float x = fmaf(t, dx, ox), y = fmaf(t, dy, oy), z = fmaf(t, dz, oz);
        const float theta = atan2f(sqrtf(fmaf(z, z, x * x)), y);
        const float phi = atan2f(z, x);
        coords[n * 2] = fmaf(2 * theta, RM_RPI, -1.0f);
        coords[n * 2 + 1] = phi * RM_RPI;
    }
}

__global__ void __launch_bounds__(256) k_morton3D(const int32_t *__restrict__ coords, uint32_t N, int32_t *__restrict__ indices) {
    for (uint32_t n = blockIdx.x * blockDim.x + threadIdx.x; n < N; n += gridDim.x * blockDim.x)
        indices[n] = (int32_t)rm_morton3D((uint32_t)coords[n * 3], (uint32_t)coords[n * 3 + 1], (uint32_t)coords[n * 3 + 2]);
}
__global__ void __launch_bounds__(256) k_morton3D_invert(const int32_t *__restrict__ indices, uint32_t N, int32_t *__restrict__ coords) {
    for (uint32_t n = blockIdx.x * blockDim.x + threadIdx.x; n < N; n += gridDim.x * blockDim.x) {
        const int32_t ind = indices[n];
        coords[n * 3] = (int32_t)rm_morton3D_invert((uint32_t)(ind >> 0));
        coords[n * 3 + 1] = (int32_t)rm_morton3D_invert((uint32_t)(ind >> 1));
        coords[n * 3 + 2] = (int32_t)rm_morton3D_invert((uint32_t)(ind >> 2));
    }
}

__global__ void __launch_bounds__(256) k_packbits_x4(const float4 *__restrict__ grid4, uint32_t N4, float thresh,
                              uint32_t *__restrict__ bitfield4) {
    for (uint32_t n = blockIdx.x * blockDim.x + threadIdx.x; n < N4; n += gridDim.x * blockDim.x) {
        uint32_t bits = 0;
#pragma unroll
        for (int q = 0; q < 8; q++) {
            const float4 v = grid4[(uint64_t)n * 8 + q];
            bits |= (v.x > thresh ? 1u : 0u) << (q * 4 + 0);
            bits |= (v.y > thresh ? 1u : 0u) << (q * 4 + 1);
            bits |= (v.z > thresh ? 1u : 0u) << (q * 4 + 2);
            bits |= (v.w > thresh ? 1u : 0u) << (q * 4 + 3);
        }
        bitfield4[n] = bits;
    }
}
__global__ void __launch_bounds__(256) k_packbits_tail(const float *__restrict__ grid, uint32_t n0, uint32_t N, float thresh,
                                uint8_t *__restrict__ bitfield) {
    for (uint32_t n = n0 + blockIdx.x * blockDim.x + threadIdx.x; n < N; n += gridDim.x * blockDim.x) {
        uint32_t bits = 0;
#pragma unroll
        for (int i = 0; i < 8; i++) bits |= (grid[(uint64_t)n * 8 + i] > thresh ? 1u : 0u) << i;
        bitfield[n] = (uint8_t)bits;
    }
}

struct RmCell { float x, y, z, dt, mip_bound; int nx, ny, nz; };

struct RmParams {
    float bound, dt_gamma, dt_min, dt_max, rH, H3, Hf, Cf, Hm1;
    uint32_t H;
    float norm_inv;
    int rederive;
    int gamma_pow2;
};
__device__ __forceinline__ float rm_out(const RmParams &p, float x) { return p.norm_inv != 0.0f ? (x + p.bound) * p.norm_inv : x; }

struct RmRay { float ox, oy, oz, dx, dy, dz, rdx, rdy, rdz; };
template <typename I>
__device__ __forceinline__ RmRay rm_load_ray(const float *__restrict__ rays_o, const float *__restrict__ rays_d, I i) {
    RmRay r;
    r.ox = rays_o[i * 3]; r.oy = rays_o[i * 3 + 1]; r.oz = rays_o[i * 3 + 2];
    r.dx = rays_d[i * 3]; r.dy = rays_d[i * 3 + 1]; r.dz = rays_d[i * 3 + 2];
    r.rdx = 1 / r.dx; r.rdy = 1 / r.dy; r.rdz = 1 / r.dz;
    return r;
}
__device__ __forceinline__ float rm_dt(const RmParams &p, float t) { return rm_clamp(t * p.dt_gamma, p.dt_min, p.dt_max); }
__device__ __forceinline__ float rm_start(const RmParams &p, float t, float noise) { return fmaf(rm_dt(p, t), noise, t); }
__device__ __forceinline__ void rm_pos(const RmParams &p, const RmRay &r, float t, float &x, float &y, float &z) {
    x = rm_clamp(fmaf(t, r.dx, r.ox), -p.bound, p.bound);
    y = rm_clamp(fmaf(t, r.dy, r.oy), -p.bound, p.bound);
    z = rm_clamp(fmaf(t, r.dz, r.oz), -p.bound, p.bound);
}

__device__ __forceinline__ bool rm_cell(const uint8_t *__restrict__ grid, const RmParams &p, const RmRay &r, float t, RmCell &c) {
    rm_pos(p, r, t, c.x, c.y, c.z);
    c.dt = rm_dt(p, t);
    const int l1 = rm_mip_from_pos(c.x, c.y, c.z, p.Cf);
    const float mdt = (float)((double)(c.dt * p.Hf) * 0.5);
    const int l2 = (int)fminf(p.Cf - 1, fmaxf(0.0f, (float)rm_frexp_exp(mdt)));
    const int level = l1 > l2 ? l1 : l2;
    return rm_cell_bit(grid, rm_cell_index(c.x, c.y, c.z, level, p.bound, p.H, p.Hm1, p.H3, c.mip_bound, c.nx, c.ny, c.nz));
}

__device__ __forceinline__ float rm_skip_target(const RmParams &p, const RmCell &c, float t, const RmRay &r) {
    const float tx = fmaf(fmaf(fmaf(0.5f, rm_sign(r.dx), (float)c.nx + 0.5f) * p.rH, 2.0f, -1.0f), c.mip_bound, -c.x) * r.rdx;
    const float ty = fmaf(fmaf(fmaf(0.5f, rm_sign(r.dy), (float)c.ny + 0.5f) * p.rH, 2.0f, -1.0f), c.mip_bound, -c.y) * r.rdy;
    const float tz = fmaf(fmaf(fmaf(0.5f, rm_sign(r.dz), (float)c.nz + 0.5f) * p.rH, 2.0f, -1.0f), c.mip_bound, -c.z) * r.rdz;
    return t + fmaxf(0.0f, fminf(tx, fminf(ty, tz)));
}

__device__ __forceinline__ float rm_skip(const RmParams &p, const RmCell &c, float t, const RmRay &r) {
    const float tt = rm_skip_target(p, c, t, r);
    do { t += rm_dt(p, t); } while (t < tt);
    return t;
}

static RmParams rm_make_params(float bound, float dt_gamma, uint32_t max_steps, uint32_t C, uint32_t H) {
    RmParams p;
    p.bound = bound; p.dt_gamma = dt_gamma;
    p.dt_min = 2 * RM_SQRT3 / (float)max_steps;
    p.dt_max = 2 * RM_SQRT3 * (float)(1 << (C - 1)) / (float)H;
    p.rH = 1 / (float)H;
    p.H3 = (float)(H * H * H);
    p.Hf = (float)H; p.Cf = (float)C; p.Hm1 = (float)(H - 1);
    p.H = H;
    p.norm_inv = 0.0f;
    p.rederive = 0;
    int e = 0;
    p.gamma_pow2 = (dt_gamma > 0.0f && frexpf(dt_gamma, &e) == 0.5f) ? 1 : 0;
    return p;
}

__device__ __forceinline__ void rm_train_range(const RmRay &r, uint32_t n, const float *__restrict__ aabb, float min_near, bool writer,
                                               float *__restrict__ nears, float *__restrict__ fars, float &near, float &far) {
    if (aabb) {
        rm_near_far(r.ox, r.oy, r.oz, r.dx, r.dy, r.dz, aabb[0], aabb[1], aabb[2], aabb[3], aabb[4], aabb[5], min_near, near, far);
        if (writer) { nears[n] = near; fars[n] = far; }
    } else { near = nears[n]; far = fars[n]; }
}

template <int DPP, uint32_t COUNT, bool MED3>
__device__ __forceinline__ void rm_lattice(const RmParams &p, float t_cur, float &T, float &t_next) {
    constexpr uint32_t UNROLL = COUNT > 16u ? 8u : COUNT;
    T = t_cur; t_next = t_cur;
#pragma unroll UNROLL
    for (uint32_t j = 0; j < COUNT; j++) {
        T = __builtin_bit_cast(float, __builtin_amdgcn_update_dpp(__builtin_bit_cast(int, t_next), __builtin_bit_cast(int, T), DPP, 0xf, 0xf, false));
        const float raw = t_next * p.dt_gamma;
        t_next += MED3 ? __builtin_amdgcn_fmed3f(raw, p.dt_min, p.dt_max) : rm_clamp(raw, p.dt_min, p.dt_max);
    }
// ... 1033 lines not shown
```

focnerf_amd/csrc/sample_math.h:

```cpp
#pragma once
#include "common.h"

typedef _Float16 h8 __attribute__((ext_vector_type(8)));

__device__ __forceinline__ void foc_sh16(float x, float y, float z, float (&o)[16]) {
    const float xy = x * y, xz = x * z, yz = y * z, x2 = x * x, y2 = y * y, z2 = z * z;
    o[0] = 0.28209479177387814f;
    o[1] = -0.48860251190291987f * y;
    o[2] = 0.48860251190291987f * z;
    o[3] = -0.48860251190291987f * x;
    o[4] = 1.0925484305920792f * xy;
    o[5] = -1.0925484305920792f * yz;
    o[6] = 0.94617469575755997f * z2 - 0.31539156525251999f;
    o[7] = -1.0925484305920792f * xz;
    o[8] = 0.54627421529603959f * x2 - 0.54627421529603959f * y2;
    o[9] = 0.59004358992664352f * y * (-3.0f * x2 + y2);
    o[10] = 2.8906114426405538f * xy * z;
    o[11] = 0.45704579946446572f * y * (1.0f - 5.0f * z2);
    o[12] = 0.3731763325901154f * z * (5.0f * z2 - 3.0f);
    o[13] = 0.45704579946446572f * x * (1.0f - 5.0f * z2);
    o[14] = 1.4453057213202769f * z * (x2 - y2);
    o[15] = 0.59004358992664352f * x * (-x2 + 3.0f * y2);
}
__device__ __forceinline__ void foc_sh16_h(float x, float y, float z, h8 &lo, h8 &hi) {
    float sh[16];
    foc_sh16(x, y, z, sh);
#pragma unroll
    for (int k = 0; k < 8; k++) { lo[k] = foc_f2h(sh[k]); hi[k] = foc_f2h(sh[8 + k]); }
}

__device__ __forceinline__ float foc_sigmoid_h(float x) { return (float)(_Float16)(1.0f / (1.0f + expf(-x))); }

__device__ __forceinline__ float foc_clamp15(float x) { return x < -15.0f ? -15.0f : (x > 15.0f ? 15.0f : x); }
__device__ __forceinline__ float foc_trunc_exp_bwd(float x) { return expf(foc_clamp15(x)); }
__device__ __forceinline__ float foc_trunc_exp_bwd(float x, float e) {
    const float xc = foc_clamp15(x);
    return xc != x ? expf(xc) : e;
}
struct FocExp15 { float lo, hi; };
__device__ __forceinline__ FocExp15 foc_exp15() {
    float a = -15.0f, b = 15.0f;
    asm volatile("" : "+v"(a));
    asm volatile("" : "+v"(b));
    return FocExp15{expf(a), expf(b)};
}
__device__ __forceinline__ float foc_trunc_exp_bwd_of_sigma(float sigma, const FocExp15 &e) { return fminf(fmaxf(sigma, e.lo), e.hi); }

struct FocBg { float b0, b1, b2; };
__device__ __forceinline__ FocBg foc_bg(const float *__restrict__ bg_ray, float bg_scalar, uint32_t k) {
    return FocBg{bg_ray ? bg_ray[k * 3] : bg_scalar, bg_ray ? bg_ray[k * 3 + 1] : bg_scalar, bg_ray ? bg_ray[k * 3 + 2] : bg_scalar};
}
```

focnerf_amd/fixedstep.py:

```python
import torch
from torch.autograd import Function

from . import raymarching
from ._lib import lib, ptr, stream_of, check
from .gridencoder import grid_encode


RAY_BLOCK = 64


def ray_block_default():
    import os
    return RAY_BLOCK if os.environ.get("FOC_RAY_BLOCK", str(RAY_BLOCK)) != "0" else 0


def blocked_rows(N, T, ray_block):
    return N * T if not ray_block else -(-N // ray_block) * ray_block * T


def fixed_sample(rays_o, rays_d, nears, fars, aabb, noise, T, bound, want_xyzs=False, want_ray_sh=False, ray_block=0):
    N = rays_o.shape[0]
    dev = rays_o.device
    rows = blocked_rows(N, T, ray_block)
    enc_in = torch.empty(rows, 3, dtype=torch.float32, device=dev)
    xyzs = torch.empty(rows, 3, dtype=torch.float32, device=dev) if want_xyzs else None
    ray_sh = torch.empty(N, 16, dtype=torch.float16, device=dev) if want_ray_sh else None
    check(lib.foc_fixed_sample(ptr(rays_o), ptr(rays_d), ptr(nears), ptr(fars), ptr(aabb), ptr(noise), N, T, float(bound), ptr(xyzs), ptr(enc_in),
                               ptr(ray_sh), int(ray_block), stream_of(rays_o)), "fixed_sample")
    if want_ray_sh:
        return enc_in, xyzs, ray_sh
    return enc_in, xyzs


def ray_sh_rows(rays_d):
    rays_d = rays_d.contiguous().float()
    N, dev = rays_d.shape[0], rays_d.device
    zeros, ones = torch.zeros(N, device=dev), torch.ones(N, device=dev)
    aabb = torch.tensor([-1., -1., -1., 1., 1., 1.], device=dev)
    return fixed_sample(torch.zeros_like(rays_d), rays_d, zeros, ones, aabb, None, 2, 1.0, want_ray_sh=True)[2]


class _density_head(Function):

    @staticmethod
    def forward(ctx, h, rays_d, nears, fars, noise, N, T, density_scale, obj_feat=None):
        from .field import object_feature_half
        h = h.contiguous()
        assert h.dtype == torch.float16 and h.shape == (N * T, 16)
        dev = h.device
        M = N * T
        sigma = torch.empty(M, dtype=torch.float32, device=dev)
        trans = torch.empty(M, dtype=torch.float32, device=dev)
        weights = torch.empty(M, dtype=torch.float32, device=dev)
        ws = torch.empty(N, dtype=torch.float32, device=dev)
        depth = torch.empty(N, dtype=torch.float32, device=dev)
        width = 32 if obj_feat is None else 48
        obj_feat = object_feature_half(obj_feat, "_density_head")
        cin = torch.empty(M, width, dtype=torch.float16, device=dev)
        check(lib.foc_fixed_head_forward(ptr(h), ptr(rays_d), ptr(nears), ptr(fars), ptr(noise), N, T, float(density_scale), ptr(sigma), ptr(trans),
                                         ptr(weights), ptr(ws), ptr(depth), ptr(cin), ptr(obj_feat), width, stream_of(h)), "fixed_head_forward")
        ctx.save_for_backward(h, sigma, trans, nears, fars, noise if noise is not None else torch.empty(0, device=dev))
        ctx.has_noise = noise is not None
        ctx.dims = (N, T, float(density_scale))
        ctx.width = width
        ctx.mark_non_differentiable(sigma)
        ctx.set_materialize_grads(False)
        return weights, ws, depth, sigma, cin

    @staticmethod
    def backward(ctx, g_weights, g_ws, g_depth, g_sigma, g_cin):
        h, sigma, trans, nears, fars, noise = ctx.saved_tensors
        N, T, ds = ctx.dims
        noise = noise if ctx.has_noise else None
        g_weights = g_weights.contiguous().float() if g_weights is not None else None
        g_ws = g_ws.contiguous().float() if g_ws is not None else None
        g_depth = g_depth.contiguous().float() if g_depth is not None else None
        g_cin = g_cin.contiguous().half() if g_cin is not None else None
        grad_h = torch.empty_like(h)
        check(lib.foc_fixed_head_backward(ptr(h), ptr(sigma), ptr(trans), ptr(nears), ptr(fars), ptr(noise), ptr(g_weights), ptr(g_ws), ptr(g_depth),
                                          ptr(g_cin), N, T, ds, ptr(grad_h), ctx.width, stream_of(h)), "fixed_head_backward")
        g_obj = None
        if ctx.width == 48 and ctx.needs_input_grad[8] and g_cin is not None:
            g_obj = g_cin[:, 31:47].float().sum(0)
        return grad_h, None, None, None, None, None, None, None, g_obj


class _fixed_composite(Function):

    @staticmethod
    def forward(ctx, c, weights, bg_ray, bg_scalar, N, T, thresh, weights_sum=None):
        c = c.contiguous()
        weights = weights.contiguous()
        assert c.dtype == torch.float16 and c.shape == (N * T, 16) and weights.dtype == torch.float32
        image = torch.empty(N, 3, dtype=torch.float32, device=c.device)
        check(lib.foc_fixed_composite_forward(ptr(c), ptr(weights), ptr(bg_ray), float(bg_scalar), N, T, float(thresh), ptr(image), stream_of(c)),
              "fixed_composite_forward")
        ctx.bg_grad = bg_ray is not None and ctx.needs_input_grad[2]
        if ctx.bg_grad and weights_sum is None:
            raise RuntimeError("_fixed_composite: a background that needs a gradient needs weights_sum")
        empty = torch.empty(0, device=c.device)
        ctx.save_for_backward(c, weights, bg_ray if bg_ray is not None else empty, weights_sum.detach() if ctx.bg_grad else empty)
        ctx.has_bg = bg_ray is not None
        ctx.dims = (N, T, float(thresh), float(bg_scalar))
        return image

    @staticmethod
    def backward(ctx, g_image):
        c, weights, bg_ray, weights_sum = ctx.saved_tensors
        N, T, thresh, bg_scalar = ctx.dims
        bg_ray = bg_ray if ctx.has_bg else None
        g_image = g_image.contiguous().float()
        grad_c = torch.empty_like(c)
        grad_w = torch.empty_like(weights)
        check(lib.foc_fixed_composite_backward(ptr(g_image), ptr(c), ptr(weights), ptr(bg_ray), bg_scalar, N, T, thresh, ptr(grad_c), ptr(grad_w),
                                               stream_of(c)), "fixed_composite_backward")
        g_bg = g_image * (1 - weights_sum).unsqueeze(-1) if ctx.bg_grad else None
        return grad_c, grad_w, g_bg, None, None, None, None, None


_C_WIDTH = 4


class _render_tail(Function):

    @staticmethod
    def forward(ctx, h, cweights, ray_sh, nears, fars, noise, bg_ray, bg_scalar, N, T, density_scale, thresh, num_layers, activation, obj_feat=None,
                want_sumsq=False, c_pre=None, w16_pre=None, input_pad=0.0, want_dist=False):
        from .field import _half_of, pad_twin, object_feature_half
        h = h.contiguous()
        assert h.dtype == torch.float16 and h.shape == (N * T, 16)
        assert ray_sh.dtype == torch.float16 and ray_sh.shape == (N, 16) and ray_sh.is_contiguous()
        dev, M = h.device, N * T
        st = stream_of(h)
        w16 = w16_pre if w16_pre is not None else _half_of(cweights)
        obj16 = object_feature_half(obj_feat, "_render_tail")
        assert obj16 is None or w16.numel() == 64 * (48 + 64 * (int(num_layers) - 1) + 16)
        if c_pre is not None:
            assert c_pre.dtype == torch.float16 and c_pre.shape == (M, _C_WIDTH) and c_pre.is_contiguous()
            c = c_pre
        else:
            c = torch.empty(M, _C_WIDTH, dtype=torch.float16, device=dev)
            args = (ptr(h), ptr(ray_sh), T, ptr(w16), M, 64, int(num_layers), int(activation), ptr(c), _C_WIDTH, ptr(obj16))
            fn, extra = pad_twin("foc_color_head_forward", input_pad, obj16 is not None)
            check(fn(*args, *extra, st), "color_head_forward")
        sigma = torch.empty(M, dtype=torch.float32, device=dev)
        trans = torch.empty(M, dtype=torch.float32, device=dev)
        weights = torch.empty(M, dtype=torch.float32, device=dev)
        ws = torch.empty(N, dtype=torch.float32, device=dev)
        depth = torch.empty(N, dtype=torch.float32, device=dev)
        image = torch.empty(N, 3, dtype=torch.float32, device=dev)
        sumsq = torch.empty(N, dtype=torch.float32, device=dev) if want_sumsq else None
        tail = (ptr(h), ptr(c), ptr(nears), ptr(fars), ptr(noise), ptr(bg_ray), float(bg_scalar), N, T, float(density_scale), float(thresh), ptr(sigma),
                ptr(trans), ptr(weights), ptr(ws), ptr(depth), ptr(image), _C_WIDTH, ptr(sumsq))
        dist = wm = None
        if want_dist:
            dist, wm = torch.empty(N, dtype=torch.float32, device=dev), torch.empty(N, dtype=torch.float32, device=dev)
            check(lib.foc_fixed_tail_forward_dist(*tail, ptr(dist), ptr(wm), st), "fixed_tail_forward_dist")
        else:
            check(lib.foc_fixed_tail_forward(*tail, st), "fixed_tail_forward")
        empty = torch.empty(0, device=dev)
        ctx.bg_grad = bg_ray is not None and ctx.needs_input_grad[6]
        ctx.save_for_backward(h, w16, sigma, trans, weights, c, ray_sh, nears, fars, noise if noise is not None else empty,
                              bg_ray if bg_ray is not None else empty, obj16 if obj16 is not None else empty,
                              ws if ctx.bg_grad or want_dist else empty, wm if want_dist else empty)
        ctx.outputs = (bool(want_sumsq), bool(want_dist))
        ctx.flags = (noise is not None, bg_ray is not None, obj16 is not None, obj_feat.dtype if obj_feat is not None else None,
                     tuple(obj_feat.shape) if obj_feat is not None else None)
        ctx.dims = (N, T, float(density_scale), float(thresh), float(bg_scalar), int(num_layers), int(activation), float(input_pad))
        ctx.mark_non_differentiable(sigma, weights, c)
        ctx.set_materialize_grads(False)
        return (image, ws, depth, sigma, weights, c) + ((sumsq,) if want_sumsq else ()) + ((dist,) if want_dist else ())

    @staticmethod
    def backward(ctx, g_image, g_ws, g_depth, _g_sigma, _g_weights, _g_c, *g_extra):
        from .backend import _scratch
        from .field import pad_twin
        h, w16, sigma, trans, weights, c, ray_sh, nears, fars, noise, bg_ray, obj16, ws, wm = ctx.saved_tensors
        g_extra = list(g_extra)
        g_sumsq = g_extra.pop(0) if ctx.outputs[0] else None
        g_dist = g_extra.pop(0) if ctx.outputs[1] else None
        has_noise, has_bg, has_obj, obj_dtype, obj_shape = ctx.flags
        obj16 = obj16 if has_obj else None
        N, T, ds, thresh, bg_scalar, num_layers, activation, input_pad = ctx.dims
        noise = noise if has_noise else None
        bg_ray = bg_ray if has_bg else None
        dev, M = h.device, N * T
        st = stream_of(h)
        g_image = g_image.contiguous().float() if g_image is not None else torch.zeros(N, 3, dtype=torch.float32, device=dev)
        g_ws = g_ws.contiguous().float() if g_ws is not None else None
        g_depth = g_depth.contiguous().float() if g_depth is not None else None
        g_sumsq = g_sumsq.contiguous().float() if g_sumsq is not None else None
        grad_c = torch.empty_like(c)
        grad_h0 = torch.empty(M, dtype=torch.float16, device=dev)
        if g_dist is not None:
            g_dist = g_dist.contiguous().float()
            check(lib.foc_fixed_tail_backward_dist(ptr(g_image), ptr(g_ws), ptr(g_depth), ptr(c), ptr(sigma), ptr(trans), ptr(weights), ptr(ws), ptr(nears),
                                                   ptr(fars), ptr(noise), ptr(bg_ray), bg_scalar, N, T, ds, thresh, ptr(grad_c), ptr(grad_h0), _C_WIDTH,
                                                   ptr(g_sumsq), ptr(wm), None, ptr(g_dist), st), "fixed_tail_backward_dist")
        else:
            check(lib.foc_fixed_tail_backward(ptr(g_image), ptr(g_ws), ptr(g_depth), ptr(c), ptr(sigma), ptr(trans), ptr(weights), ptr(nears), ptr(fars),
                                              ptr(noise), ptr(bg_ray), bg_scalar, N, T, ds, thresh, ptr(grad_c), ptr(grad_h0), _C_WIDTH, ptr(g_sumsq), st),
                  "fixed_tail_backward")
        grad_h = torch.empty_like(h)
        g_w = torch.empty_like(w16)
        wsb = _scratch.get("ffmlp_ws", lib.foc_ffmlp_backward_workspace_bytes(48 if has_obj else 32, 64, num_layers), dev)
        g_obj32 = torch.empty(16, dtype=torch.float32, device=dev) if has_obj and ctx.needs_input_grad[14] else None
        args = (ptr(grad_c), ptr(h), ptr(ray_sh), T, ptr(grad_h0), ptr(w16), M, 64, num_layers, activation, ptr(grad_h), ptr(g_w), ptr(wsb),
                wsb.numel(), _C_WIDTH, ptr(obj16), ptr(g_obj32))
        fn, extra = pad_twin("foc_color_head_backward", input_pad, has_obj)
        check(fn(*args, *extra, st), "color_head_backward")
        g_obj = g_obj32.to(obj_dtype).view(obj_shape) if g_obj32 is not None else None
        g_bg = g_image * (1 - ws).unsqueeze(-1) if ctx.bg_grad else None
        return (grad_h, g_w, None, None, None, None, g_bg) + (None,) * 7 + (g_obj, None, None, None, None, None)


class _masked_norm(Function):

    @staticmethod
    def forward(ctx, sumsq, outside):
        crit = torch.sqrt((sumsq * outside).sum())
        ctx.save_for_backward(crit, outside)
        return crit

    @staticmethod
    def backward(ctx, g):
        crit, outside = ctx.saved_tensors
        coef = torch.where(crit > 0, g / (2 * crit), torch.zeros_like(crit))
        return outside * coef, None


def _unfused_distortion(weights, nears, fars, noise, N, T):
    from .loss import ray_distortion
    span = (fars - nears).unsqueeze(-1)
    z = span * torch.linspace(0.0, 1.0, T, device=weights.device).unsqueeze(0)
    if noise is not None:
        z = z + (noise.view(N, T) - 0.5) * (span / T)
    delta = torch.cat([z[:, 1:] - z[:, :-1], span / T], dim=-1)
    live = (fars > nears).unsqueeze(-1)
    zero = torch.zeros_like(z)
    return ray_distortion(torch.where(live, weights.view(N, T), zero), torch.where(live, z + 0.5 * delta, zero), torch.where(live, delta, zero))


def _background(bg_color, N, dev):
    if bg_color is None:
        return None, 1.0
    if torch.is_tensor(bg_color):
        if bg_color.numel() > 1:
            return bg_color.to(dev, torch.float32).reshape(-1, 3).expand(N, 3).contiguous(), 0.0
        return None, float(bg_color)
    return None, float(bg_color)


def render_fixed_steps(model, rays_o, rays_d, yolo_details=None, num_steps=512, bg_color=None, perturb=False, weight_thresh=1e-10,
                       return_fields=None, _out=None, distortion=False, **kwargs):
    import time
    if return_fields is None:
        return_fields = not model.training
    t_start = time.time()
    prefix = rays_o.shape[:-1]
    rays_o = rays_o.contiguous().view(-1, 3).float()
    rays_d = rays_d.contiguous().view(-1, 3).float()
    N, T = rays_o.shape[0], int(num_steps)
    dev = rays_o.device
    aabb = model.aabb_train if model.training else model.aabb_infer
    nears, fars = raymarching.near_far_from_aabb(rays_o, rays_d, aabb, model.min_near)
    noise = torch.rand(N * T, dtype=torch.float32, device=dev) if perturb else None
    from .field import field_plan, field_infer
    plan = field_plan(model)
    if getattr(model, "bg_radius", 0) > 0:
        bg_color = model._background_colour(rays_o, rays_d, bg_color)
    want_tail = plan.tail and model.training and torch.is_grad_enabled()
    fused_infer = not torch.is_grad_enabled() and plan.infer
    if distortion and not torch.is_grad_enabled():
        raise ValueError("render_fixed_steps: distortion=True needs the training route (gradients enabled): the inference paths form no "
                         "differentiable weights; call it under torch.enable_grad() with model.train()")
    rb = ray_block_default() if fused_infer else 0
    enc_in, _, ray_sh = fixed_sample(rays_o, rays_d, nears, fars, aabb, noise, T, model.bound, want_ray_sh=True) if want_tail else \
        fixed_sample(rays_o, rays_d, nears, fars, aabb, noise, T, model.bound, ray_block=rb) + (None,)

    if fused_infer:
        obj_feat = model.encode_object_feature(yolo_details, dev) if plan.uses_object_feature else None
        sigma, rgb = field_infer(model, enc_in, rays_d, dir_div=T, dir_block=rb, obj_feat=obj_feat)
        bg_ray, bg_scalar = _background(bg_color, N, dev)
        direct = (_out is not None and _out[0].dtype == torch.float32 and _out[1].dtype == torch.float32 and _out[0].is_contiguous()
                  and _out[1].is_contiguous() and _out[0].numel() == N and _out[1].numel() == 3 * N and _out[0].device == dev)
        depth, image = (_out[0].view(N), _out[1].view(N, 3)) if direct else (torch.empty(N, dtype=torch.float32, device=dev),
                                                                              torch.empty(N, 3, dtype=torch.float32, device=dev))
        weights_sum = torch.empty(N, dtype=torch.float32, device=dev)
        rgb_masked = densities = None
        if return_fields:
            if direct and len(_out) == 4 and all(t.dtype == torch.float32 and t.is_contiguous() and t.device == dev for t in _out[2:]) \
                    and _out[2].numel() == N * T and _out[3].numel() == 3 * N * T and rb:
                densities, rgb_masked = _out[2].view(N * T), _out[3].view(N * T, 3)
            else:
                rgb_masked = torch.empty(N * T, 3, dtype=torch.float32, device=dev)
                densities = torch.empty(N * T, dtype=torch.float32, device=dev) if rb else None
        check(lib.foc_fixed_render_inference(ptr(sigma), ptr(rgb), ptr(nears), ptr(fars), ptr(noise), ptr(bg_ray), float(bg_scalar), N, T,
                                             float(model.density_scale), float(weight_thresh), ptr(image), ptr(depth), ptr(weights_sum), ptr(rgb_masked),
                                             rb, ptr(densities), stream_of(sigma)), "fixed_render_inference")
        t_mid = time.time()
        results = {'depth': depth.view(*prefix), 'image': image.view(*prefix, 3), 'weights_sum': weights_sum, 'criterion_outside_mask': None,
                   'timing': [t_mid - t_start, time.time() - t_mid]}
        if return_fields:
            results['densities'] = (densities if rb else sigma).view(N, T, 1)
            results['rgbs'] = rgb_masked.view(N, T, 3)
        return results

    enc = model.encoder
    from .field import hashgrid_mlp, fused_mlp
    c_pre = obj_feat = None
    cweights = fused_mlp(model, "color_net").weights if want_tail else None
    with torch.autocast("cuda", dtype=torch.float16):
        if plan.uses_object_feature:
            obj_feat = model.encode_object_feature(yolo_details, dev)
        if plan.field:
            colour = wc16 = None
            if want_tail and plan.train_forward:
                from .field import _half_of
                wc16 = _half_of(cweights)
                colour = (wc16, plan.colour, ray_sh, T, _C_WIDTH, obj_feat, plan.colour_input_pad)
            h = hashgrid_mlp(enc, fused_mlp(model, "sigma_net"), enc_in, None, colour)
            if colour is not None:
                h, c_pre = h
        else:
            feats = grid_encode(enc_in, enc.embeddings, enc.offsets, enc.per_level_scale, enc.base_resolution, False, enc.gridtype_id,
                                enc.align_corners, enc.interp_id)
            h = fused_mlp(model, "sigma_net")(feats)
        if h.shape[1] != 16:
            raise RuntimeError("render_fixed_steps expects a 16-wide sigma head (1 + geo_feat_dim = 16)")
        fused_tail = want_tail
        want_crit = model.training and yolo_details is not None and yolo_details[0] is not None
        criterion_outside_mask = None
        if fused_tail:
            cn = fused_mlp(model, "color_net")
            bg_ray, bg_scalar = _background(bg_color, N, dev)
            outs = _render_tail.apply(h, cweights, ray_sh, nears, fars, noise, bg_ray, bg_scalar, N, T, model.density_scale, weight_thresh,
                                      cn.num_layers, cn.activation, obj_feat, want_crit and yolo_details[0].numel() == N, c_pre,
                                      wc16 if c_pre is not None else None, plan.colour_input_pad, *((True,) if distortion else ()))
            image, weights_sum, depth, sigma, weights, c = outs[:6]
            ray_dist = outs[-1] if distortion else None
            if len(outs) - bool(distortion) == 7:
                criterion_outside_mask = _masked_norm.apply(outs[6], (~yolo_details[0].reshape(N)).to(torch.float32))
        else:
            weights, weights_sum, depth, sigma, cin = _density_head.apply(h, rays_d, nears, fars, noise, N, T, model.density_scale, obj_feat)
            if plan.colour_input_pad != 0:
                cin = torch.cat([cin[:, :-1], cin.new_full((cin.shape[0], 1), plan.colour_input_pad)], dim=1)
            if distortion:
                ray_dist = _unfused_distortion(weights, nears, fars, noise, N, T)
        if want_crit and criterion_outside_mask is None:
            from .activation import trunc_exp
            criterion_outside_mask = torch.norm(trunc_exp(h[:, 0]).view(N, T)[~yolo_details[0].squeeze(0)] - 0)
        if not fused_tail:
            c = fused_mlp(model, "color_net").forward_padded(cin)
    t_mid = time.time()

    if not fused_tail:
        bg_ray, bg_scalar = _background(bg_color, N, dev)
        image = _fixed_composite.apply(c, weights, bg_ray, bg_scalar, N, T, weight_thresh, weights_sum)

    results = {'depth': depth.view(*prefix), 'image': image.view(*prefix, 3), 'weights_sum': weights_sum,
               'criterion_outside_mask': criterion_outside_mask, 'timing': [t_mid - t_start, time.time() - t_mid]}
    if distortion:
        results['distortion'] = ray_dist.view(*prefix)
    if return_fields:
        from .head import rgb_head
        c16 = c.detach()
        if c16.shape[1] != 16:
            c16 = torch.nn.functional.pad(c16, (0, 16 - c16.shape[1]))
        rgb = rgb_head(c16) * (weights > weight_thresh).unsqueeze(-1)
        results['densities'] = sigma.view(N, T, 1)
        results['rgbs'] = rgb.view(N, T, 3)
    return results


@torch.no_grad()
def render_field4(model, rays_o, rays_d, num_steps=512, weight_thresh=1e-10, yolo_details=None, out=None, occupancy=None, placement=None,
                  scene_aabb=None, channels="rgb"):
    from .field import field_plan, field_infer
    from .normals import check_channels, field_normals
    if placement is None and scene_aabb is not None:
        raise ValueError("render_field4: scene_aabb belongs to a placement; without one the object is rendered in its own box")
    if placement is not None and occupancy is None:
        raise ValueError("render_field4: placement needs occupancy= (the placed path is the occupancy-culled one): pass "
                         "fixedcull.Occupancy.of(model) for a cuda_ray network or fixedcull.Occupancy.estimate(model) for any other")
    rays_o = rays_o.contiguous().view(-1, 3).float()
    rays_d = rays_d.contiguous().view(-1, 3).float()
    N, T = rays_o.shape[0], int(num_steps)
    dev = rays_o.device
    if out is None:
        out = torch.empty(N, T, 4, dtype=torch.float32, device=dev)
    assert out.shape == (N, T, 4) and out.dtype == torch.float32 and out.is_contiguous()
    plan = field_plan(model)
    want_normal = check_channels("render_field4", channels, plan)
    if placement is not None:
        from .fixedcull import render_field4_placed
        return render_field4_placed(model, plan, rays_o, rays_d, T, weight_thresh, yolo_details, out, occupancy, placement, scene_aabb, channels)
    if occupancy is not None:
        from .fixedcull import render_field4_culled
        return render_field4_culled(model, plan, rays_o, rays_d, T, weight_thresh, yolo_details, out, occupancy, channels)
    if want_normal and not (plan.infer and model.bg_radius <= 0):
        raise ValueError("render_field4: channels='normal' needs a network the fused inference serves (field_plan(model).infer) without a "
                         "background model")
    if plan.infer and model.bg_radius <= 0:
        aabb = model.aabb_train if model.training else model.aabb_infer
        nears, fars = raymarching.near_far_from_aabb(rays_o, rays_d, aabb, model.min_near)
        rb = ray_block_default()
        enc_in, _ = fixed_sample(rays_o, rays_d, nears, fars, aabb, None, T, model.bound, ray_block=rb)
        obj_feat = model.encode_object_feature(yolo_details, dev) if plan.uses_object_feature else None
        if want_normal:
            sigma, rgb = field_normals(model, enc_in)
        else:
            sigma, rgb = field_infer(model, enc_in, rays_d, dir_div=T, dir_block=rb, obj_feat=obj_feat)
        check(lib.foc_fixed_field_pack(ptr(sigma), ptr(rgb), ptr(nears), ptr(fars), None, None, 1.0, N, T, float(model.density_scale),
                                       float(weight_thresh), None, None, None, ptr(out), rb, stream_of(sigma)), "fixed_field_pack")
        return out
    from .combine import pack_field4
    with torch.autocast("cuda", dtype=torch.float16):
        res = model.run(rays_o[None], rays_d[None], yolo_details, num_steps=T, upsample_steps=0, perturb=False, weight_thresh=weight_thresh,
                        return_fields=True)
    out.copy_(pack_field4(res['densities'], res['rgbs']))
    return out
```

include/focnerf.h:

```cpp
#ifndef FOCNERF_H
#define FOCNERF_H

#include <stddef.h>
#include <stdint.h>

#ifdef __cplusplus
extern "C" {
#endif

#define FOC_OK            0
#define FOC_E_INVALID     1
#define FOC_E_DTYPE       2
#define FOC_E_LAUNCH      3

#define FOC_F32 0
#define FOC_F16 1

#define FOC_ABI_VERSION 2
int         foc_abi_version(void);
const char *foc_last_error(void);
int foc_set_option(const char *name, int value);
int foc_get_option(const char *name, int *value);
int foc_guard_pick_device(int stream_is_null, int stream_device, int pointer_device, int current_device);
const char *foc_arch(void);
// ... 129 lines not shown
                                   uint32_t interp, int dtype, const int32_t *offsets_host, void *workspace,
                                   uint64_t workspace_bytes, void *stream);
int foc_grid_encode_backward_binned_counted(const void *grad, const float *inputs, const void *embeddings,
                                            const int32_t *offsets, void *grad_embeddings,
                                            uint32_t B, uint32_t D, uint32_t C, uint32_t L, float S, uint32_t H,
                                            const void *dy_dx, void *grad_inputs, uint32_t gridtype,
                                            int align_corners, uint32_t interp, int dtype, int grad_is_bl,
                                            const int32_t *offsets_host, void *workspace, uint64_t workspace_bytes,
                                            void *stream);

int foc_grad_total_variation(const void *inputs, const void *embeddings, void *grad,
                             const int32_t *offsets, float weight,
                             uint32_t B, uint32_t D, uint32_t C, uint32_t L, float S, uint32_t H,
                             uint32_t gridtype, int align_corners, int dtype, void *stream);


int foc_freq_encode_forward(const float *inputs, uint32_t B, uint32_t D, uint32_t deg, uint32_t C,
                            float *outputs, void *stream);
int foc_freq_encode_backward(const float *grad, const float *outputs, uint32_t B, uint32_t D,
                             uint32_t deg, uint32_t C, float *grad_inputs, void *stream);


int foc_ffmlp_forward(const void *inputs, const void *weights, uint32_t B, uint32_t input_dim,
                      uint32_t output_dim, uint32_t hidden_dim, uint32_t num_layers,
                      uint32_t activation, uint32_t output_activation,
                      void *forward_buffer, void *outputs, void *stream);

int foc_ffmlp_inference(const void *inputs, const void *weights, uint32_t B, uint32_t input_dim,
                        uint32_t output_dim, uint32_t hidden_dim, uint32_t num_layers,
                        uint32_t activation, uint32_t output_activation,
                        void *inference_buffer, void *outputs, void *stream);

int foc_ffmlp_backward(const void *grad, const void *inputs, const void *weights,
                       const void *forward_buffer, uint32_t B, uint32_t input_dim,
                       uint32_t output_dim, uint32_t hidden_dim, uint32_t num_layers,
                       uint32_t activation, uint32_t output_activation, int calc_grad_inputs,
                       void *backward_buffer, void *grad_inputs, void *grad_weights,
                       void *workspace, uint64_t workspace_bytes, void *stream);
uint64_t foc_ffmlp_backward_workspace_bytes(uint32_t input_dim, uint32_t hidden_dim, uint32_t num_layers);

int foc_ffmlp_forward_planar(const void *inputs_planar, const void *weights, uint32_t B, uint32_t input_dim,
                             uint32_t output_dim, uint32_t hidden_dim, uint32_t num_layers,
                             uint32_t activation, uint32_t output_activation, void *outputs, void *stream);
int foc_ffmlp_backward_planar(const void *grad, const void *inputs_planar, const void *weights, uint32_t B,
                              uint32_t input_dim, uint32_t output_dim, uint32_t hidden_dim, uint32_t num_layers,
                              uint32_t activation, uint32_t output_activation, int calc_grad_inputs,
                              void *grad_inputs_planar, void *grad_weights, void *workspace, uint64_t workspace_bytes, void *stream);

int foc_nerf_field_inference(const void *enc, int enc_planar, const float *dirs, uint32_t dir_div,
                             uint32_t dir_block, uint32_t n_dirs, const void *sigma_weights, uint32_t sigma_layers, const void *color_weights,
                             uint32_t color_layers, uint32_t hidden_dim, uint32_t activation, uint32_t B,
                             float *sigma, float *rgb, const void *obj_feat, void *stream);
int foc_nerf_field_inference_pad(const void *enc, int enc_planar, const float *dirs, uint32_t dir_div,
                                 uint32_t dir_block, uint32_t n_dirs, const void *sigma_weights, uint32_t sigma_layers, const void *color_weights,
                                 uint32_t color_layers, uint32_t hidden_dim, uint32_t activation, uint32_t B,
                                 float *sigma, float *rgb, const void *obj_feat, float input_pad, void *stream);
int foc_nerf_field_inference_pad31(const void *enc, int enc_planar, const float *dirs, uint32_t dir_div,
                                   uint32_t dir_block, uint32_t n_dirs, const void *sigma_weights, uint32_t sigma_layers, const void *color_weights,
                                   uint32_t color_layers, uint32_t hidden_dim, uint32_t activation, uint32_t B,
                                   float *sigma, float *rgb, const void *obj_feat, float input_pad, void *stream);

int foc_field_normals(const float *xn, uint32_t M, const void *embeddings, const uint32_t *offsets, uint32_t D, uint32_t C, uint32_t L,
                      float S, uint32_t H, uint32_t gridtype, int align_corners, uint32_t interp, int dtype, const int32_t *offsets_host,
                      const void *sigma_weights, uint32_t sigma_layers, uint32_t hidden_dim, uint32_t activation, const float *rot9,
                      float *sigma, float *grad_raw, float *normal_rgb, void *grad_enc, void *stream);

int foc_color_head_forward(const void *h, const void *ray_sh, uint32_t samples_per_ray, const void *weights,
                           uint32_t B, uint32_t hidden_dim, uint32_t num_layers, uint32_t activation,
                           void *outputs, uint32_t out_width, const void *obj_feat, void *stream);
int foc_color_head_backward(const void *grad, const void *h, const void *ray_sh, uint32_t samples_per_ray,
                            const void *grad_h0, const void *weights, uint32_t B, uint32_t hidden_dim,
                            uint32_t num_layers, uint32_t activation, void *grad_h, void *grad_weights,
                            void *workspace, uint64_t workspace_bytes, uint32_t out_width, const void *obj_feat, float *grad_obj, void *stream);
int foc_color_head_forward_pad(const void *h, const void *ray_sh, uint32_t samples_per_ray, const void *weights,
                               uint32_t B, uint32_t hidden_dim, uint32_t num_layers, uint32_t activation,
                               void *outputs, uint32_t out_width, const void *obj_feat, float input_pad, void *stream);
int foc_color_head_backward_pad(const void *grad, const void *h, const void *ray_sh, uint32_t samples_per_ray,
                                const void *grad_h0, const void *weights, uint32_t B, uint32_t hidden_dim,
                                uint32_t num_layers, uint32_t activation, void *grad_h, void *grad_weights,
                                void *workspace, uint64_t workspace_bytes, uint32_t out_width, const void *obj_feat, float *grad_obj,
                                float input_pad, void *stream);
int foc_color_head_forward_pad31(const void *h, const void *ray_sh, uint32_t samples_per_ray, const void *weights,
                                 uint32_t B, uint32_t hidden_dim, uint32_t num_layers, uint32_t activation,
                                 void *outputs, uint32_t out_width, const void *obj_feat, float input_pad, void *stream);
int foc_color_head_backward_pad31(const void *grad, const void *h, const void *ray_sh, uint32_t samples_per_ray,
                                  const void *grad_h0, const void *weights, uint32_t B, uint32_t hidden_dim,
                                  uint32_t num_layers, uint32_t activation, void *grad_h, void *grad_weights,
                                  void *workspace, uint64_t workspace_bytes, uint32_t out_width, const void *obj_feat, float *grad_obj,
                                  float input_pad, void *stream);

int foc_field_forward_train(const void *planes, const void *sigma_weights, uint32_t sigma_layers, const void *ray_sh, uint32_t samples_per_ray,
                            const void *color_weights, uint32_t color_layers, uint32_t hidden_dim, uint32_t activation, uint32_t B,
                            void *h, void *c, uint32_t out_width, const void *obj_feat, void *stream);
int foc_field_forward_train_pad(const void *planes, const void *sigma_weights, uint32_t sigma_layers, const void *ray_sh, uint32_t samples_per_ray,
                                const void *color_weights, uint32_t color_layers, uint32_t hidden_dim, uint32_t activation, uint32_t B,
                                void *h, void *c, uint32_t out_width, const void *obj_feat, float input_pad, void *stream);
int foc_field_forward_train_pad31(const void *planes, const void *sigma_weights, uint32_t sigma_layers, const void *ray_sh, uint32_t samples_per_ray,
                                  const void *color_weights, uint32_t color_layers, uint32_t hidden_dim, uint32_t activation, uint32_t B,
                                  void *h, void *c, uint32_t out_width, const void *obj_feat, float input_pad, void *stream);

int foc_allocate_splitk(uint64_t size);
int foc_free_splitk(void);


int foc_combine_select(const float *dens, const float *rgb, float *max_dens, float *best_rgb,
                       uint64_t n, void *stream);

int foc_combine_pack_keys(const float *dens, uint32_t rank, uint64_t *keys, uint64_t n, void *stream);
int foc_combine_unpack(const uint64_t *keys, uint32_t rank, const float *rgb,
                       float *max_dens, float *masked_rgb, uint64_t n, void *stream);

int foc_composite_fixed_steps(const float *sigmas, const float *rgbs, const float *nears,
                              const float *fars, uint32_t N, uint32_t T, float bg,
                              float *image4, float *depth, void *stream);

#define FOC_COMBINE_MAX_OBJECTS 16

int foc_combine_select_composite(const float *const *fields4, uint32_t K, const float *nears, const float *fars,
                                 uint32_t N, uint32_t T, const float *bgs, uint32_t n_bg, float *image4, float *depth,
                                 float *merged4, void *stream);

int foc_combine_select4(const float *field4, float *acc4, uint64_t n, void *stream);

int foc_combine_select_composite_attr(const float *const *fields4, uint32_t K, const uint8_t *const *id_planes,
                                      const uint32_t *ids, uint32_t n_obj, const float *nears, const float *fars,
                                      uint32_t N, uint32_t T, const float *bgs, uint32_t n_bg, float *image4, float *depth,
                                      float *merged4, float *obj_weights, float *obj_depth, int32_t *instance,
                                      uint8_t *winner, void *stream);

typedef struct FocCulledField {
    const uint64_t *mask;
    const uint32_t *offsets;
    const float *sigma_c;
    const float *rgb_c;
    uint32_t m_occ;
    float density_scale;
    float thresh;
    float sigma_gain;
} FocCulledField;
int foc_combine_select_composite_culled(const FocCulledField *objs, uint32_t K, uint32_t struct_bytes, const uint32_t *ids,
                                        uint32_t n_obj, const float *nears, const float *fars, uint32_t N, uint32_t T,
                                        const float *bgs, uint32_t n_bg, float *image4, float *depth, float *merged4,
                                        float *obj_weights, float *obj_depth, int32_t *instance, uint8_t *winner, void *stream);

int foc_combine_select4_ids(const float *field4, uint32_t id, float *acc4, uint8_t *acc_ids, uint64_t n, void *stream);

int foc_mo_select(const void *sigma_new, const void *feat_new, void *sigma_best, void *feat_best, uint64_t n,
                  uint32_t feat_width, uint32_t elem_bytes, void *stream);


int foc_fixed_sample(const float *rays_o, const float *rays_d, const float *nears, const float *fars,
                     const float *aabb, const float *noise, uint32_t N, uint32_t T, float bound,
                     float *xyzs, float *enc_in, void *ray_sh, uint32_t ray_block, void *stream);

int foc_fixed_head_forward(const void *h, const float *rays_d, const float *nears, const float *fars,
                           const float *noise, uint32_t N, uint32_t T, float density_scale,
                           float *sigma, float *trans, float *weights, float *weights_sum, float *depth,
                           void *cin, const void *obj_feat, uint32_t cin_width, void *stream);
int foc_fixed_head_backward(const void *h, const float *sigma, const float *trans, const float *nears,
                            const float *fars, const float *noise, const float *grad_w, const float *grad_ws,
                            const float *grad_depth, const void *grad_cin, uint32_t N, uint32_t T,
                            float density_scale, void *grad_h, uint32_t cin_width, void *stream);

int foc_fixed_tail_forward(const void *h, const void *c, const float *nears, const float *fars, const float *noise,
                           const float *bg_ray, float bg_scalar, uint32_t N, uint32_t T, float density_scale, float thresh,
                           float *sigma, float *trans, float *weights, float *weights_sum, float *depth, float *image,
                           uint32_t c_width, float *ray_sumsq, void *stream);
int foc_fixed_tail_backward(const float *grad_image, const float *grad_ws, const float *grad_depth, const void *c,
                            const float *sigma, const float *trans, const float *weights, const float *nears,
                            const float *fars, const float *noise, const float *bg_ray, float bg_scalar, uint32_t N,
                            uint32_t T, float density_scale, float thresh, void *grad_c, void *grad_h0, uint32_t c_width,
                            const float *grad_sumsq, void *stream);

int foc_occ_tail_forward(const void *h, const void *c, uint32_t c_width, const float *deltas, const int32_t *rays,
                         uint32_t M, uint32_t N, float T_thresh, float density_scale, const float *bg_ray, float bg_scalar,
                         const float *nears, const float *fars, float *weights_sum, float *image_raw, float *image,
                         float *depth, void *stream);
int foc_occ_tail_backward(const float *grad_image, const float *grad_ws, const void *h, const void *c, uint32_t c_width,
                          const float *deltas, const int32_t *rays, const int32_t *counter, const float *weights_sum,
                          const float *image_raw, uint32_t M, uint32_t N, float T_thresh, float density_scale,
                          const float *bg_ray, float bg_scalar, void *grad_c, void *grad_h0, void *stream);
int foc_occ_tail_forward_sumsq(const void *h, const void *c, uint32_t c_width, const float *deltas, const int32_t *rays,
                               uint32_t M, uint32_t N, float T_thresh, float density_scale, const float *bg_ray, float bg_scalar,
                               const float *nears, const float *fars, float *weights_sum, float *image_raw, float *image,
                               float *depth, float *ray_sumsq, void *stream);
int foc_occ_tail_backward_sumsq(const float *grad_image, const float *grad_ws, const void *h, const void *c, uint32_t c_width,
                                const float *deltas, const int32_t *rays, const int32_t *counter, const float *weights_sum,
                                const float *image_raw, uint32_t M, uint32_t N, float T_thresh, float density_scale,
                                const float *bg_ray, float bg_scalar, void *grad_c, void *grad_h0, const float *grad_sumsq, void *stream);

int foc_fixed_tail_forward_dist(const void *h, const void *c, const float *nears, const float *fars, const float *noise,
                                const float *bg_ray, float bg_scalar, uint32_t N, uint32_t T, float density_scale, float thresh,
                                float *sigma, float *trans, float *weights, float *weights_sum, float *depth, float *image,
                                uint32_t c_width, float *ray_sumsq, float *ray_dist, float *ray_wm, void *stream);
int foc_fixed_tail_backward_dist(const float *grad_image, const float *grad_ws, const float *grad_depth, const void *c,
                                 const float *sigma, const float *trans, const float *weights, const float *weights_sum, const float *nears,
                                 const float *fars, const float *noise, const float *bg_ray, float bg_scalar, uint32_t N,
                                 uint32_t T, float density_scale, float thresh, void *grad_c, void *grad_h0, uint32_t c_width,
                                 const float *grad_sumsq, const float *ray_wm, const float *ray_dist, const float *grad_dist, void *stream);
int foc_occ_tail_forward_dist(const void *h, const void *c, uint32_t c_width, const float *deltas, const int32_t *rays,
                              uint32_t M, uint32_t N, float T_thresh, float density_scale, const float *bg_ray, float bg_scalar,
                              const float *nears, const float *fars, float *weights_sum, float *image_raw, float *image,
                              float *depth, float *ray_sumsq, float *ray_dist, float *ray_wm, void *stream);
int foc_occ_tail_backward_dist(const float *grad_image, const float *grad_ws, const void *h, const void *c, uint32_t c_width,
                               const float *deltas, const int32_t *rays, const int32_t *counter, const float *weights_sum,
                               const float *image_raw, uint32_t M, uint32_t N, float T_thresh, float density_scale,
                               const float *bg_ray, float bg_scalar, void *grad_c, void *grad_h0, const float *grad_sumsq,
                               const float *ray_wm, const float *ray_dist, const float *grad_dist, void *stream);
int foc_occ_tail_forward_depth(const void *h, const void *c, uint32_t c_width, const float *deltas, const int32_t *rays,
                               uint32_t M, uint32_t N, float T_thresh, float density_scale, const float *bg_ray, float bg_scalar,
                               const float *nears, const float *fars, float *weights_sum, float *image_raw, float *image,
                               float *depth, float *ray_sumsq, float *ray_dist, float *ray_wm, float *depth_raw, void *stream);
int foc_occ_tail_backward_depth(const float *grad_image, const float *grad_ws, const void *h, const void *c, uint32_t c_width,
                                const float *deltas, const int32_t *rays, const int32_t *counter, const float *weights_sum,
                                const float *image_raw, uint32_t M, uint32_t N, float T_thresh, float density_scale,
                                const float *bg_ray, float bg_scalar, void *grad_c, void *grad_h0, const float *grad_sumsq,
                                const float *ray_wm, const float *ray_dist, const float *grad_dist, const float *nears,
                                const float *fars, const float *depth_raw, const float *grad_depth, void *stream);

typedef struct FocOccTrainNode {
    uint32_t struct_bytes;
    uint32_t n_rays, max_steps, cascade, grid_size, cap, pad_align;
    float bound, dt_gamma, min_near;
    const float *rays_o, *rays_d, *aabb, *jitter;
    const uint8_t *bitfield;
    float *nears, *fars, *enc_in, *deltas;
    void *sh_rows;
    int32_t *rays, *counter, *march_scratch;
    uint32_t levels, base_resolution, gridtype, interp;
    int32_t align_corners, table_dtype;
    float per_level_scale_log2;
    const void *embeddings;
    const int32_t *offsets, *offsets_host;
    void *planes, *grid_workspace;
    uint64_t grid_workspace_bytes;
    uint32_t sigma_input_dim, sigma_hidden, sigma_layers, sigma_activation, sigma_output_activation;
    uint32_t color_hidden, color_layers, color_activation, c_width;
    const void *w_sigma, *w_color;
    void *h, *c;
    float T_thresh, density_scale, bg_scalar;
    const float *bg_ray;
    float *weights_sum, *image_raw, *image, *depth;
    int32_t precounted;
    const float *grad_image, *grad_ws;
    void *grad_c, *grad_h0, *grad_h, *grad_planes, *grad_w_color, *grad_w_sigma, *grad_embeddings, *mlp_workspace;
    uint64_t mlp_workspace_bytes;
} FocOccTrainNode;
int foc_occ_train_forward(const FocOccTrainNode *node, void *stream);
int foc_occ_train_backward(const FocOccTrainNode *node, void *stream);
int foc_occ_train_forward_pad31(const FocOccTrainNode *node, float input_pad, void *stream);
int foc_occ_train_backward_pad31(const FocOccTrainNode *node, float input_pad, void *stream);
typedef struct FocOccTrainObject {
    uint32_t struct_bytes;
    float input_pad;
    const void *obj_feat;
    float *ray_sumsq;
    const float *grad_sumsq;
    float *grad_obj;
} FocOccTrainObject;
int foc_occ_train_forward_obj(const FocOccTrainNode *node, const FocOccTrainObject *object, void *stream);
int foc_occ_train_backward_obj(const FocOccTrainNode *node, const FocOccTrainObject *object, void *stream);
typedef struct FocOccTrainTail {
    uint32_t struct_bytes;
    float *ray_dist, *ray_wm, *depth_raw;
    const float *grad_dist, *grad_depth;
} FocOccTrainTail;
int foc_occ_train_forward_tail(const FocOccTrainNode *node, const FocOccTrainObject *object, float input_pad,
                               const FocOccTrainTail *tail, void *stream);
int foc_occ_train_backward_tail(const FocOccTrainNode *node, const FocOccTrainObject *object, float input_pad,
                                const FocOccTrainTail *tail, void *stream);

int foc_view_tile_order(const float *rays_d, uint32_t N, uint32_t tile_h, uint32_t tile_w, int64_t *perm, void *state16,
                        void *stream);

int foc_fixed_composite_forward(const void *c, const float *weights, const float *bg_ray, float bg_scalar,
                                uint32_t N, uint32_t T, float thresh, float *image, void *stream);
int foc_fixed_composite_backward(const float *grad_image, const void *c, const float *weights,
                                 const float *bg_ray, float bg_scalar, uint32_t N, uint32_t T, float thresh,
                                 void *grad_c, float *grad_w, void *stream);

int foc_fixed_render_inference(const float *sigma, const float *rgb, const float *nears, const float *fars,
                               const float *noise, const float *bg_ray, float bg_scalar, uint32_t N, uint32_t T,
                               float density_scale, float thresh, float *image, float *depth, float *weights_sum,
                               float *rgb_masked, uint32_t ray_block, float *sigma_raymajor, void *stream);

int foc_fixed_field_pack(const float *sigma, const float *rgb, const float *nears, const float *fars,
                         const float *noise, const float *bg_ray, float bg_scalar, uint32_t N, uint32_t T,
                         float density_scale, float thresh, float *image, float *depth, float *weights_sum,
                         float *field4, uint32_t ray_block, void *stream);

uint64_t foc_fixed_cull_scratch_bytes(uint32_t N, uint32_t T);
int foc_fixed_cull(const float *rays_o, const float *rays_d, const float *nears, const float *fars, const float *aabb,
                   uint32_t N, uint32_t T, float bound, const uint8_t *bitfield, uint32_t cascade, uint32_t grid_size,
                   uint64_t *mask, uint32_t *offsets, uint32_t *count, void *scratch, uint64_t scratch_bytes, void *stream);
int foc_fixed_cull_emit(const float *rays_o, const float *rays_d, const float *nears, const float *fars, const float *aabb,
                        uint32_t N, uint32_t T, float bound, const uint64_t *mask, const uint32_t *offsets, uint32_t m_occ,
                        float *enc_in_c, float *dirs_c, void *stream);

int foc_fixed_field_pack_culled(const float *sigma_c, const float *rgb_c, const uint64_t *mask, const uint32_t *offsets,
                                uint32_t m_occ, const float *nears, const float *fars, uint32_t N, uint32_t T,
                                float density_scale, float thresh, float *field4, void *stream);

int foc_fixed_cull_placed(const float *rays_o, const float *rays_d, const float *nears, const float *fars, const float *scene_aabb,
                          uint32_t N, uint32_t T, const float *world_to_object, const float *obj_aabb, float bound,
                          const uint8_t *bitfield, uint32_t cascade, uint32_t grid_size, uint64_t *mask, uint32_t *offsets,
                          uint32_t *count, void *scratch, uint64_t scratch_bytes, void *stream);
int foc_fixed_cull_emit_placed(const float *rays_o, const float *rays_d, const float *nears, const float *fars,
                               const float *scene_aabb, uint32_t N, uint32_t T, const float *world_to_object, float dir_scale,
                               float bound, const uint64_t *mask, const uint32_t *offsets, uint32_t m_occ, float *enc_in_c,
                               float *dirs_c, void *stream);
int foc_fixed_field_pack_culled_gain(const float *sigma_c, const float *rgb_c, const uint64_t *mask, const uint32_t *offsets,
                                     uint32_t m_occ, const float *nears, const float *fars, uint32_t N, uint32_t T,
                                     float density_scale, float thresh, float sigma_gain, float *field4, void *stream);


int foc_sample_head_forward(const void *h, const float *dirs, uint64_t M, float *sigma, void *cin,
                            const void *obj_feat, uint32_t cin_width, void *stream);
int foc_sample_head_backward(const void *h, const float *grad_sigma, const void *grad_cin, uint64_t M,
                             void *grad_h, uint32_t cin_width, void *stream);
int foc_sh_encode(const float *dirs, uint64_t M, float *out, void *stream);
int foc_rgb_head_forward(const void *c, uint64_t M, float *rgb, void *stream);
int foc_rgb_head_backward(const void *c, const float *grad_rgb, uint64_t M, void *grad_c, void *stream);


int foc_mark_untrained_grid(const float *poses, uint32_t B, float fx, float fy, float cx, float cy, float bound,
// ... 93 lines not shown
```

Measured before the change: 1.388 billion.

## Recompute tail transmittance in backward from fp16 h0 plane; fuse near/far into sampling

```diff
diff --git a/focnerf_amd/_lib.py b/focnerf_amd/_lib.py
--- a/focnerf_amd/_lib.py
+++ b/focnerf_amd/_lib.py
@@ -209,8 +209,11 @@
     "foc_fixed_field_pack_culled_gain": (i32, [c_vp, c_vp, c_vp, c_vp, u32, c_vp, c_vp, u32, u32, f32, f32, f32, c_vp, c_vp]),
     "foc_composite_fixed_steps":(i32, [c_vp, c_vp, c_vp, c_vp, u32, u32, f32, c_vp, c_vp, c_vp]),
     "foc_fixed_sample": (i32, [c_vp, c_vp, c_vp, c_vp, c_vp, c_vp, u32, u32, f32, c_vp, c_vp, c_vp, u32, c_vp]),
+    "foc_fixed_sample_nf": (i32, [c_vp, c_vp, c_vp, f32, c_vp, u32, u32, f32, c_vp, c_vp, c_vp, c_vp, c_vp, u32, c_vp]),
     "foc_fixed_tail_forward": (i32, [c_vp, c_vp, c_vp, c_vp, c_vp, c_vp, f32, u32, u32, f32, f32, c_vp, c_vp, c_vp, c_vp, c_vp, c_vp, u32, c_vp, c_vp]),
     "foc_fixed_tail_backward": (i32, [c_vp, c_vp, c_vp, c_vp, c_vp, c_vp, c_vp, c_vp, c_vp, c_vp, c_vp, f32, u32, u32, f32, f32, c_vp, c_vp, u32, c_vp, c_vp]),
+    "foc_fixed_tail_forward_lean": (i32, [c_vp, c_vp, c_vp, c_vp, c_vp, c_vp, f32, u32, u32, f32, f32, c_vp, c_vp, c_vp, c_vp, u32, c_vp, c_vp]),
+    "foc_fixed_tail_backward_lean": (i32, [c_vp, c_vp, c_vp, c_vp, c_vp, c_vp, c_vp, c_vp, c_vp, f32, u32, u32, f32, f32, c_vp, c_vp, u32, c_vp, c_vp]),
     "foc_fixed_tail_forward_dist": (i32, [c_vp, c_vp, c_vp, c_vp, c_vp, c_vp, f32, u32, u32, f32, f32, c_vp, c_vp, c_vp, c_vp, c_vp, c_vp, u32, c_vp, c_vp,
                                           c_vp, c_vp]),
     "foc_fixed_tail_backward_dist": (i32, [c_vp, c_vp, c_vp, c_vp, c_vp, c_vp, c_vp, c_vp, c_vp, c_vp, c_vp, c_vp, f32, u32, u32, f32, f32, c_vp, c_vp, u32,
diff --git a/focnerf_amd/csrc/combine.hip b/focnerf_amd/csrc/combine.hip
--- a/focnerf_amd/csrc/combine.hip
+++ b/focnerf_amd/csrc/combine.hip
@@ -383,7 +383,7 @@
 static FocOptionRow foc_option_table[FOC_OPT_COUNT] = {
     {"FOC_MLP_BWD_FUSED", 1}, {"FOC_FIELD_FWD_FUSED", 1}, {"FOC_GB_MERGE_MAX_RES", 480}, {"FOC_GB_FACTORED", 1}, {"FOC_GB_TAIL_SPLIT", 16}, {"FOC_GRID_FUSE_SMALL", 1},
     {"FOC_GRID_PAIRS", 1}, {"FOC_GRID_FAST", 1}, {"FOC_MARCH_SERIAL", -1}, {"FOC_MARCH_RAYS_ROW_MAX", 131072}, {"FOC_OCC_MARCH_FORM", -1},
-    {"FOC_OCC_SAMPLE_MAJOR", 1}, {"FOC_OCC_FIELD_PIECE", 1 << 23}, {"FOC_DETERMINISTIC", 0},
+    {"FOC_OCC_SAMPLE_MAJOR", 1}, {"FOC_OCC_FIELD_PIECE", 1 << 23}, {"FOC_DETERMINISTIC", 0}, {"FOC_TAIL_LEAN", 1},
 };
 static int foc_option_parse(int which, const char *text) {
     if (which == FOC_OPT_OCC_MARCH_FORM) {
diff --git a/focnerf_amd/csrc/common.h b/focnerf_amd/csrc/common.h
--- a/focnerf_amd/csrc/common.h
+++ b/focnerf_amd/csrc/common.h
@@ -28,6 +28,7 @@
     FOC_OPT_OCC_SAMPLE_MAJOR,
     FOC_OPT_OCC_FIELD_PIECE,
     FOC_OPT_DETERMINISTIC,
+    FOC_OPT_TAIL_LEAN,
     FOC_OPT_COUNT
 };
 int foc_opt(FocOpt which);
diff --git a/focnerf_amd/csrc/fixedstep.hip b/focnerf_amd/csrc/fixedstep.hip
--- a/focnerf_amd/csrc/fixedstep.hip
+++ b/focnerf_amd/csrc/fixedstep.hip
@@ -2,10 +2,12 @@
 #include "fs_common.h"
 #include <float.h>
 
+template <bool NF>
 __global__ void __launch_bounds__(256) k_fs_sample(const float *__restrict__ rays_o, const float *__restrict__ rays_d, const float *__restrict__ nears,
                                                    const float *__restrict__ fars, const float *__restrict__ aabb, const float *__restrict__ noise,
                                                    uint32_t N, uint32_t T, float bound, float *__restrict__ xyzs, float *__restrict__ enc_in,
-                                                   _Float16 *__restrict__ ray_sh, uint32_t ray_block) {
+                                                   _Float16 *__restrict__ ray_sh, uint32_t ray_block, float min_near, float *__restrict__ nears_out,
+                                                   float *__restrict__ fars_out) {
     const uint64_t total = ray_block ? (uint64_t)((N + FS_RAY_BLOCK - 1) / FS_RAY_BLOCK) * FS_RAY_BLOCK * T : (uint64_t)N * T;
     const FsBox box = fs_box(aabb);
     const float two_b = 2 * bound;
@@ -21,10 +23,17 @@
         } else {
             n = (uint32_t)(s / T); i = (uint32_t)(s - (uint64_t)n * T);
         }
-        const FsGeom g = fs_geom(nears, fars, n, T);
+        const float ox = rays_o[n * 3], oy = rays_o[n * 3 + 1], oz = rays_o[n * 3 + 2], dx = rays_d[n * 3], dy = rays_d[n * 3 + 1], dz = rays_d[n * 3 + 2];
+        FsGeom g;
+        if constexpr (NF) {
+            float near, far;
+            rm_near_far(ox, oy, oz, dx, dy, dz, box.a0, box.a1, box.a2, box.a3, box.a4, box.a5, min_near, near, far);
+            if (i == 0 && own) { nears_out[n] = near; fars_out[n] = far; }
+            g = fs_geom_of(near, far, T);
+        } else g = fs_geom(nears, fars, n, T);
         const float z = fs_z(g, i, T, noise, (uint64_t)n * T + i);
         float x, y, w;
-        fs_point(rays_o[n * 3], rays_o[n * 3 + 1], rays_o[n * 3 + 2], rays_d[n * 3], rays_d[n * 3 + 1], rays_d[n * 3 + 2], z, box, x, y, w);
+        fs_point(ox, oy, oz, dx, dy, dz, z, box, x, y, w);
         if (xyzs) { xyzs[s * 3] = x; xyzs[s * 3 + 1] = y; xyzs[s * 3 + 2] = w; }
         if (enc_in) { enc_in[s * 3] = fs_norm(x, bound, two_b); enc_in[s * 3 + 1] = fs_norm(y, bound, two_b); enc_in[s * 3 + 2] = fs_norm(w, bound, two_b); }
         if (ray_sh && i == 0 && own) {
@@ -166,13 +175,14 @@
     }
 }
 
-template <bool NOISE, bool DIST>
+template <bool NOISE, bool DIST, bool LEAN>
 __global__ void __launch_bounds__(256) k_fs_tail_fwd(const _Float16 *__restrict__ h, const _Float16 *__restrict__ c, const float *__restrict__ nears,
                                                      const float *__restrict__ fars, const float *__restrict__ noise, const float *__restrict__ bg_ray,
                                                      float bg_scalar, uint32_t N, uint32_t T, float density_scale, float thresh,
                                                      float *__restrict__ sigma_out, float *__restrict__ trans_out, float *__restrict__ weights_out,
                                                      float *__restrict__ weights_sum, float *__restrict__ depth, float *__restrict__ image, uint32_t c_ld,
-                                                     float *__restrict__ ray_sumsq, float *__restrict__ ray_dist, float *__restrict__ ray_wm) {
+                                                     float *__restrict__ ray_sumsq, float *__restrict__ ray_dist, float *__restrict__ ray_wm,
+                                                     _Float16 *__restrict__ h0_plane) {
     const uint32_t lane = threadIdx.x & 63;
     const uint32_t n = blockIdx.x * 4 + (threadIdx.x >> 6);
     if (n >= N) return;
@@ -189,17 +199,15 @@
         const uint2 raw = *reinterpret_cast<const uint2 *>(c + s * c_ld);
         float u0 = 0.0f, u1 = 0.0f;
         if (NOISE) { u0 = noise[s]; u1 = noise[(uint64_t)n * T + min(ic + 1u, T - 1u)]; }
-        const float sigma = expf((float)h0);
         const FsSample p = fs_sample(g, i, ic, T, NOISE, u0, u1);
-        const float alpha = valid ? 1 - expf((-p.delta * density_scale) * sigma) : 0.0f;
-        const float om = valid ? (1 - alpha + 1e-15f) : 1.0f;
-        const float Tb = fs_trans_scan(om, lane, Tc);
-        const float w = alpha * Tb;
+        const FsHead hd = fs_head_fwd_step(h0, p, valid, density_scale, lane, Tc);
+        const float sigma = hd.sigma, Tb = hd.Tb, w = hd.alpha * Tb;
         if constexpr (DIST) {
             if (live) fs_dist_fwd_step(dist, w, fs_dist_m(g, p), p.delta, lane);
         }
         if (valid) {
-            sigma_out[s] = sigma; trans_out[s] = Tb; weights_out[s] = w;
+            if constexpr (LEAN) h0_plane[s] = h0;
+            else { sigma_out[s] = sigma; trans_out[s] = Tb; weights_out[s] = w; }
             ws += w; dp += w * p.oz; sq = fmaf(sigma, sigma, sq);
             if (w > thresh) {
                 const _Float16 *cc = reinterpret_cast<const _Float16 *>(&raw);
@@ -210,7 +218,7 @@
     ws = wave_sum(ws); dp = wave_sum(dp); r = wave_sum(r); gg = wave_sum(gg); b = wave_sum(b);
     if (ray_sumsq) {
         sq = wave_sum(sq);
-        if (lane == 0) ray_sumsq[n] = sq;
+        if (lane == 0) ray_sumsq[n] = foc_canon_nan(sq);
     }
     if constexpr (DIST) {
         const float ds = wave_sum(dist.acc);
@@ -218,23 +226,41 @@
     }
     if (lane == 0) {
         const FocBg bg = foc_bg(bg_ray, bg_scalar, n);
-        image[n * 3] = r + (1 - ws) * bg.b0; image[n * 3 + 1] = gg + (1 - ws) * bg.b1; image[n * 3 + 2] = b + (1 - ws) * bg.b2;
-        weights_sum[n] = ws; depth[n] = dp;
-    }
-}
-
-template <bool NOISE, bool DIST>
+        image[n * 3] = foc_canon_nan(r + (1 - ws) * bg.b0); image[n * 3 + 1] = foc_canon_nan(gg + (1 - ws) * bg.b1);
+        image[n * 3 + 2] = foc_canon_nan(b + (1 - ws) * bg.b2);
+        weights_sum[n] = foc_canon_nan(ws); depth[n] = foc_canon_nan(dp);
+    }
+}
+
+template <bool NOISE, bool DIST, bool LEAN>
 __global__ void __launch_bounds__(256) k_fs_tail_bwd(const float *__restrict__ grad_image, const float *__restrict__ grad_ws, const float *__restrict__ grad_depth,
                                                      const _Float16 *__restrict__ c, const float *__restrict__ sigma_in, const float *__restrict__ trans_in,
                                                      const float *__restrict__ weights, const float *__restrict__ nears, const float *__restrict__ fars,
                                                      const float *__restrict__ noise, const float *__restrict__ bg_ray, float bg_scalar, uint32_t N, uint32_t T,
                                                      float density_scale, float thresh, _Float16 *__restrict__ grad_c, _Float16 *__restrict__ grad_h0, uint32_t c_ld,
                                                      const float *__restrict__ grad_sumsq, const float *__restrict__ weights_sum,
-                                                     const float *__restrict__ ray_wm, const float *__restrict__ grad_dist) {
+                                                     const float *__restrict__ ray_wm, const float *__restrict__ grad_dist,
+                                                     const _Float16 *__restrict__ h0_plane) {
+    extern __shared__ float fs_carry[];
     const uint32_t lane = threadIdx.x & 63;
     const uint32_t n = blockIdx.x * 4 + (threadIdx.x >> 6);
     if (n >= N) return;
     const FsGeom g = fs_geom(nears, fars, n, T);
+    const uint32_t n_chunks = (T + 63) / 64;
+    float *const carry = fs_carry + (threadIdx.x >> 6) * n_chunks;
+    if constexpr (LEAN) {
+        float Tc = 1.0f;
+        for (uint32_t cidx = 0; cidx < n_chunks; cidx++) {
+            if (lane == 0) carry[cidx] = Tc;
+            if (cidx + 1 == n_chunks) break;
+            const uint32_t i = cidx * 64 + lane;
+            const uint64_t s = (uint64_t)n * T + i;
+            const _Float16 h0 = h0_plane[s];
+            float u0 = 0.0f, u1 = 0.0f;
+            if (NOISE) { u0 = noise[s]; u1 = noise[(uint64_t)n * T + min(i + 1u, T - 1u)]; }
+            fs_head_fwd_step(h0, fs_sample(g, i, i, T, NOISE, u0, u1), true, density_scale, lane, Tc);
+        }
+    }
     const float gws = grad_ws ? grad_ws[n] : 0.0f, gdp = grad_depth ? grad_depth[n] : 0.0f;
     const float gsq2 = grad_sumsq ? 2.0f * grad_sumsq[n] : 0.0f;
     float gdist = 0.0f, W_total = 0.0f, WM_total = 0.0f;
@@ -246,24 +272,33 @@
     const FsRayGrad q = fs_ray_grad(grad_image, bg_ray, bg_scalar, n);
     const FocExp15 e15 = foc_exp15();
     float S_carry = 0.0f;
-    const uint32_t n_chunks = (T + 63) / 64;
     for (uint32_t cidx = n_chunks; cidx-- > 0;) {
         const uint32_t i = cidx * 64 + lane;
         const bool valid = i < T;
         const uint32_t ic = valid ? i : T - 1;
         const uint64_t s = (uint64_t)n * T + ic;
-        const float sigma = sigma_in[s], Tb = trans_in[s], w = weights[s];
+        float sigma, Tb, w;
+        _Float16 h0 = (_Float16)0;
+        if constexpr (LEAN) h0 = h0_plane[s];
+        else { sigma = sigma_in[s]; Tb = trans_in[s]; w = weights[s]; }
         const uint2 raw = *reinterpret_cast<const uint2 *>(c + s * c_ld);
         float u0 = 0.0f, u1 = 0.0f;
         if (NOISE) { u0 = noise[s]; u1 = noise[(uint64_t)n * T + min(ic + 1u, T - 1u)]; }
+        const FsSample p = fs_sample(g, i, ic, T, NOISE, u0, u1);
+        if constexpr (LEAN) {
+            float Tc = carry[cidx];
+            const FsHead hd = fs_head_fwd_step(h0, p, valid, density_scale, lane, Tc);
+            sigma = hd.sigma; Tb = hd.Tb; w = hd.alpha * Tb;
+        }
         h8 o0;
         const h8 o1 = {0, 0, 0, 0, 0, 0, 0, 0};
         const float gw = fs_composite_bwd_sample(q, w, thresh, reinterpret_cast<const _Float16 *>(&raw), o0);
+#pragma unroll
+        for (int k = 0; k < 3; k++) o0[k] = foc_canon_nan(o0[k]);
         if (valid) {
             if (c_ld == 4u) *reinterpret_cast<uint2 *>(grad_c + s * 4) = *reinterpret_cast<const uint2 *>(&o0);
             else { h8 *dst = reinterpret_cast<h8 *>(grad_c + s * 16); dst[0] = o0; dst[1] = o1; }
         }
-        const FsSample p = fs_sample(g, i, ic, T, NOISE, u0, u1);
         float gi = gw + gws;
         if constexpr (DIST) {
             if (gdist != 0.0f) gi = fmaf(gdist, fs_dist_bwd_step(dist, valid ? w : 0.0f, fs_dist_m(g, p), p.delta, W_total, WM_total, lane), gi);
@@ -271,7 +306,7 @@
         float dsigma = fs_head_bwd_step(p, valid, sigma, Tb, gi, gdp, density_scale, lane, S_carry);
         if (gsq2 != 0.0f) dsigma = fmaf(gsq2, sigma, dsigma);
         const float dh0 = dsigma * foc_trunc_exp_bwd_of_sigma(sigma, e15);
-        if (valid) grad_h0[s] = foc_f2h(dh0);
+        if (valid) grad_h0[s] = foc_canon_nan(foc_f2h(dh0));
     }
 }
 
@@ -399,9 +434,23 @@
     FOC_REQUIRE(T >= 2, FOC_E_INVALID, "fixed_sample: T must be >= 2");
     FOC_REQUIRE(ray_block == 0 || ray_block == FS_RAY_BLOCK, FOC_E_INVALID, "fixed_sample: ray_block must be 0 (ray-major) or %u (got %u)", FS_RAY_BLOCK, ray_block);
     const uint64_t rows = ray_block ? (uint64_t)foc_div_up(N, FS_RAY_BLOCK) * FS_RAY_BLOCK * T : (uint64_t)N * T;
-    hipLaunchKernelGGL(k_fs_sample, dim3(foc_grid_1d(rows, 256, 256 * 16)), dim3(256), 0, (hipStream_t)stream, rays_o, rays_d, nears, fars, aabb,
-                       noise, N, T, bound, xyzs, enc_in, (_Float16 *)ray_sh, ray_block);
+    hipLaunchKernelGGL(k_fs_sample<false>, dim3(foc_grid_1d(rows, 256, 256 * 16)), dim3(256), 0, (hipStream_t)stream, rays_o, rays_d, nears, fars, aabb,
+                       noise, N, T, bound, xyzs, enc_in, (_Float16 *)ray_sh, ray_block, 0.0f, (float *)nullptr, (float *)nullptr);
     FOC_CHECK_LAUNCH("fixed_sample");
+    return FOC_OK;
+}
+
+int foc_fixed_sample_nf(const float *rays_o, const float *rays_d, const float *aabb, float min_near, const float *noise, uint32_t N, uint32_t T,
+                        float bound, float *nears, float *fars, float *xyzs, float *enc_in, void *ray_sh, uint32_t ray_block, void *stream) {
+    FocDeviceGuard foc_guard_(stream, rays_o);
+    if (N == 0) return FOC_OK;
+    FOC_REQUIRE(rays_o && rays_d && nears && fars && aabb && (xyzs || enc_in), FOC_E_INVALID, "fixed_sample_nf: null pointer");
+    FOC_REQUIRE(T >= 2, FOC_E_INVALID, "fixed_sample_nf: T must be >= 2");
+    FOC_REQUIRE(ray_block == 0 || ray_block == FS_RAY_BLOCK, FOC_E_INVALID, "fixed_sample_nf: ray_block must be 0 (ray-major) or %u (got %u)", FS_RAY_BLOCK, ray_block);
+    const uint64_t rows = ray_block ? (uint64_t)foc_div_up(N, FS_RAY_BLOCK) * FS_RAY_BLOCK * T : (uint64_t)N * T;
+    hipLaunchKernelGGL(k_fs_sample<true>, dim3(foc_grid_1d(rows, 256, 256 * 16)), dim3(256), 0, (hipStream_t)stream, rays_o, rays_d, (const float *)nullptr,
+                       (const float *)nullptr, aabb, noise, N, T, bound, xyzs, enc_in, (_Float16 *)ray_sh, ray_block, min_near, nears, fars);
+    FOC_CHECK_LAUNCH("fixed_sample_nf");
     return FOC_OK;
 }
 
@@ -458,24 +507,36 @@
 
 static int fixed_tail_forward(const char *who, const void *h, const void *c, const float *nears, const float *fars, const float *noise, const float *bg_ray,
                               float bg_scalar, uint32_t N, uint32_t T, float density_scale, float thresh, float *sigma, float *trans, float *weights,
-                              float *weights_sum, float *depth, float *image, uint32_t c_width, float *ray_sumsq, float *ray_dist, float *ray_wm, void *stream) {
+                              float *weights_sum, float *depth, float *image, uint32_t c_width, float *ray_sumsq, float *ray_dist, float *ray_wm,
+                              void *h0_plane, void *stream) {
     FocDeviceGuard foc_guard_(stream, h);
     if (N == 0) return FOC_OK;
     FOC_REQUIRE(c_width == 16 || c_width == 4, FOC_E_INVALID, "%s: c_width must be 16 or 4 (got %u)", who, c_width);
-    FOC_REQUIRE(h && c && nears && fars && sigma && trans && weights && weights_sum && depth && image, FOC_E_INVALID, "%s: null pointer", who);
+    FOC_REQUIRE(h && c && nears && fars && (h0_plane || (sigma && trans && weights)) && weights_sum && depth && image, FOC_E_INVALID, "%s: null pointer", who);
     FOC_REQUIRE(T >= 2, FOC_E_INVALID, "%s: T must be >= 2", who);
-    auto kern = ray_dist ? (noise ? k_fs_tail_fwd<true, true> : k_fs_tail_fwd<false, true>) : (noise ? k_fs_tail_fwd<true, false> : k_fs_tail_fwd<false, false>);
+    auto kern = h0_plane ? (noise ? k_fs_tail_fwd<true, false, true> : k_fs_tail_fwd<false, false, true>)
+                : ray_dist ? (noise ? k_fs_tail_fwd<true, true, false> : k_fs_tail_fwd<false, true, false>)
+                           : (noise ? k_fs_tail_fwd<true, false, false> : k_fs_tail_fwd<false, false, false>);
     hipLaunchKernelGGL(kern, dim3(foc_div_up(N, 4)), dim3(256), 0, (hipStream_t)stream, (const _Float16 *)h, (const _Float16 *)c, nears, fars, noise,
-                       bg_ray, bg_scalar, N, T, density_scale, thresh, sigma, trans, weights, weights_sum, depth, image, c_width, ray_sumsq, ray_dist, ray_wm);
+                       bg_ray, bg_scalar, N, T, density_scale, thresh, sigma, trans, weights, weights_sum, depth, image, c_width, ray_sumsq, ray_dist, ray_wm,
+                       (_Float16 *)h0_plane);
     FOC_CHECK_LAUNCH(who);
     return FOC_OK;
+}
+
+int foc_fixed_tail_forward_lean(const void *h, const void *c, const float *nears, const float *fars, const float *noise, const float *bg_ray, float bg_scalar,
+                                uint32_t N, uint32_t T, float density_scale, float thresh, void *h0, float *weights_sum, float *depth, float *image,
+                                uint32_t c_width, float *ray_sumsq, void *stream) {
+    FOC_REQUIRE(h0 || N == 0, FOC_E_INVALID, "fixed_tail_forward_lean: null h0");
+    return fixed_tail_forward("fixed_tail_forward_lean", h, c, nears, fars, noise, bg_ray, bg_scalar, N, T, density_scale, thresh, nullptr, nullptr, nullptr,
+                              weights_sum, depth, image, c_width, ray_sumsq, nullptr, nullptr, h0, stream);
 }
 
 int foc_fixed_tail_forward(const void *h, const void *c, const float *nears, const float *fars, const float *noise, const float *bg_ray, float bg_scalar,
                            uint32_t N, uint32_t T, float density_scale, float thresh, float *sigma, float *trans, float *weights, float *weights_sum,
                            float *depth, float *image, uint32_t c_width, float *ray_sumsq, void *stream) {
     return fixed_tail_forward("fixed_tail_forward", h, c, nears, fars, noise, bg_ray, bg_scalar, N, T, density_scale, thresh, sigma, trans, weights, weights_sum,
-                              depth, image, c_width, ray_sumsq, nullptr, nullptr, stream);
+                              depth, image, c_width, ray_sumsq, nullptr, nullptr, nullptr, stream);
 }
 
 int foc_fixed_tail_forward_dist(const void *h, const void *c, const float *nears, const float *fars, const float *noise, const float *bg_ray, float bg_scalar,
@@ -483,24 +544,37 @@
                                 float *depth, float *image, uint32_t c_width, float *ray_sumsq, float *ray_dist, float *ray_wm, void *stream) {
     FOC_REQUIRE((ray_dist && ray_wm) || N == 0, FOC_E_INVALID, "fixed_tail_forward_dist: null ray_dist / ray_wm");
     return fixed_tail_forward("fixed_tail_forward_dist", h, c, nears, fars, noise, bg_ray, bg_scalar, N, T, density_scale, thresh, sigma, trans, weights,
-                              weights_sum, depth, image, c_width, ray_sumsq, ray_dist, ray_wm, stream);
+                              weights_sum, depth, image, c_width, ray_sumsq, ray_dist, ray_wm, nullptr, stream);
 }
 
 static int fixed_tail_backward(const char *who, const float *grad_image, const float *grad_ws, const float *grad_depth, const void *c, const float *sigma,
                                const float *trans, const float *weights, const float *nears, const float *fars, const float *noise, const float *bg_ray,
                                float bg_scalar, uint32_t N, uint32_t T, float density_scale, float thresh, void *grad_c, void *grad_h0, uint32_t c_width,
-                               const float *grad_sumsq, const float *weights_sum, const float *ray_wm, const float *grad_dist, void *stream) {
+                               const float *grad_sumsq, const float *weights_sum, const float *ray_wm, const float *grad_dist, const void *h0_plane,
+                               void *stream) {
     FocDeviceGuard foc_guard_(stream, grad_image);
     if (N == 0) return FOC_OK;
     FOC_REQUIRE(c_width == 16 || c_width == 4, FOC_E_INVALID, "%s: c_width must be 16 or 4 (got %u)", who, c_width);
-    FOC_REQUIRE(grad_image && c && sigma && trans && weights && nears && fars && grad_c && grad_h0, FOC_E_INVALID, "%s: null pointer", who);
+    FOC_REQUIRE(grad_image && c && (h0_plane || (sigma && trans && weights)) && nears && fars && grad_c && grad_h0, FOC_E_INVALID, "%s: null pointer", who);
     FOC_REQUIRE(T >= 2, FOC_E_INVALID, "%s: T must be >= 2", who);
-    auto kern = grad_dist ? (noise ? k_fs_tail_bwd<true, true> : k_fs_tail_bwd<false, true>) : (noise ? k_fs_tail_bwd<true, false> : k_fs_tail_bwd<false, false>);
-    hipLaunchKernelGGL(kern, dim3(foc_div_up(N, 4)), dim3(256), 0, (hipStream_t)stream, grad_image, grad_ws, grad_depth, (const _Float16 *)c, sigma,
+    const size_t lds = h0_plane ? (size_t)4 * foc_div_up(T, 64) * sizeof(float) : 0;
+    FOC_REQUIRE(lds <= 65536, FOC_E_INVALID, "%s: T = %u is more than the 262144 samples per ray the chunk carries have room for", who, T);
+    auto kern = h0_plane ? (noise ? k_fs_tail_bwd<true, false, true> : k_fs_tail_bwd<false, false, true>)
+                : grad_dist ? (noise ? k_fs_tail_bwd<true, true, false> : k_fs_tail_bwd<false, true, false>)
+                            : (noise ? k_fs_tail_bwd<true, false, false> : k_fs_tail_bwd<false, false, false>);
+    hipLaunchKernelGGL(kern, dim3(foc_div_up(N, 4)), dim3(256), lds, (hipStream_t)stream, grad_image, grad_ws, grad_depth, (const _Float16 *)c, sigma,
                        trans, weights, nears, fars, noise, bg_ray, bg_scalar, N, T, density_scale, thresh, (_Float16 *)grad_c, (_Float16 *)grad_h0, c_width,
-                       grad_sumsq, weights_sum, ray_wm, grad_dist);
+                       grad_sumsq, weights_sum, ray_wm, grad_dist, (const _Float16 *)h0_plane);
     FOC_CHECK_LAUNCH(who);
     return FOC_OK;
+}
+
+int foc_fixed_tail_backward_lean(const float *grad_image, const float *grad_ws, const float *grad_depth, const void *c, const void *h0, const float *nears,
+                                 const float *fars, const float *noise, const float *bg_ray, float bg_scalar, uint32_t N, uint32_t T, float density_scale,
+                                 float thresh, void *grad_c, void *grad_h0, uint32_t c_width, const float *grad_sumsq, void *stream) {
+    FOC_REQUIRE(h0 || N == 0, FOC_E_INVALID, "fixed_tail_backward_lean: null h0");
+    return fixed_tail_backward("fixed_tail_backward_lean", grad_image, grad_ws, grad_depth, c, nullptr, nullptr, nullptr, nears, fars, noise, bg_ray, bg_scalar, N,
+                               T, density_scale, thresh, grad_c, grad_h0, c_width, grad_sumsq, nullptr, nullptr, nullptr, h0, stream);
 }
 
 int foc_fixed_tail_backward(const float *grad_image, const float *grad_ws, const float *grad_depth, const void *c, const float *sigma, const float *trans,
@@ -508,7 +582,7 @@
                             uint32_t N, uint32_t T, float density_scale, float thresh, void *grad_c, void *grad_h0, uint32_t c_width, const float *grad_sumsq,
                             void *stream) {
     return fixed_tail_backward("fixed_tail_backward", grad_image, grad_ws, grad_depth, c, sigma, trans, weights, nears, fars, noise, bg_ray, bg_scalar, N, T,
-                               density_scale, thresh, grad_c, grad_h0, c_width, grad_sumsq, nullptr, nullptr, nullptr, stream);
+                               density_scale, thresh, grad_c, grad_h0, c_width, grad_sumsq, nullptr, nullptr, nullptr, nullptr, stream);
 }
 
 int foc_fixed_tail_backward_dist(const float *grad_image, const float *grad_ws, const float *grad_depth, const void *c, const float *sigma, const float *trans,
@@ -518,7 +592,7 @@
     (void)ray_dist;
     FOC_REQUIRE(!grad_dist || (weights_sum && ray_wm) || N == 0, FOC_E_INVALID, "fixed_tail_backward_dist: grad_dist needs weights_sum and ray_wm");
     return fixed_tail_backward("fixed_tail_backward_dist", grad_image, grad_ws, grad_depth, c, sigma, trans, weights, nears, fars, noise, bg_ray, bg_scalar, N,
-                               T, density_scale, thresh, grad_c, grad_h0, c_width, grad_sumsq, weights_sum, ray_wm, grad_dist, stream);
+                               T, density_scale, thresh, grad_c, grad_h0, c_width, grad_sumsq, weights_sum, ray_wm, grad_dist, nullptr, stream);
 }
 
 int foc_fixed_render_inference(const float *sigma, const float *rgb, const float *nears, const float *fars, const float *noise, const float *bg_ray,
diff --git a/focnerf_amd/csrc/fs_common.h b/focnerf_amd/csrc/fs_common.h
--- a/focnerf_amd/csrc/fs_common.h
+++ b/focnerf_amd/csrc/fs_common.h
@@ -9,13 +9,16 @@
     return (uint64_t)(n / FS_RAY_BLOCK) * FS_RAY_BLOCK * T + (uint64_t)i * FS_RAY_BLOCK + n % FS_RAY_BLOCK;
 }
 
-__device__ __forceinline__ FsGeom fs_geom(const float *__restrict__ nears, const float *__restrict__ fars, uint32_t n, uint32_t T) {
+__device__ __forceinline__ FsGeom fs_geom_of(float near, float far, uint32_t T) {
     FsGeom g;
-    g.near = nears[n]; g.far = fars[n];
+    g.near = near; g.far = far;
     g.span = g.far - g.near;
     g.sample_dist = g.span / (float)T;
     g.step = 1.0f / (float)(T - 1);
     return g;
+}
+__device__ __forceinline__ FsGeom fs_geom(const float *__restrict__ nears, const float *__restrict__ fars, uint32_t n, uint32_t T) {
+    return fs_geom_of(nears[n], fars[n], T);
 }
 __device__ __forceinline__ float fs_z0(const FsGeom &g, uint32_t i, uint32_t T) {
     const float lin = (i < T / 2) ? (g.step * (float)i) : fmaf(-g.step, (float)(T - 1 - i), 1.0f);
@@ -53,6 +56,16 @@
     const float Tb = Tc * wave_prod_scan(om, lane, P);
     Tc *= __shfl(P, 63, 64);
     return Tb;
+}
+
+struct FsHead { float sigma, alpha, Tb; };
+__device__ __forceinline__ FsHead fs_head_fwd_step(_Float16 h0, const FsSample &p, bool valid, float density_scale, uint32_t lane, float &Tc) {
+    FsHead o;
+    o.sigma = expf((float)h0);
+    o.alpha = valid ? 1 - expf((-p.delta * density_scale) * o.sigma) : 0.0f;
+    const float om = valid ? (1 - o.alpha + 1e-15f) : 1.0f;
+    o.Tb = fs_trans_scan(om, lane, Tc);
+    return o;
 }
 
 __device__ __forceinline__ float wave_suffix_incl_sum(float v, int lane) {
diff --git a/focnerf_amd/csrc/raymarching.hip b/focnerf_amd/csrc/raymarching.hip
--- a/focnerf_amd/csrc/raymarching.hip
+++ b/focnerf_amd/csrc/raymarching.hip
@@ -8,30 +8,6 @@
 #define RM_RPI   0.3183098861837907f
 
 __device__ __forceinline__ float rm_sign(float x) { return copysignf(1.0f, x); }
-
-__device__ __forceinline__ void rm_near_far(float ox, float oy, float oz, float dx, float dy, float dz, float a0, float a1, float a2, float a3, float a4, float a5,
-                                            float min_near, float &near_out, float &far_out) {
-    const float rdx = 1 / dx, rdy = 1 / dy, rdz = 1 / dz;
-    float near = (a0 - ox) * rdx, far = (a3 - ox) * rdx, t;
-    if (near > far) { t = near; near = far; far = t; }
-    float near_y = (a1 - oy) * rdy, far_y = (a4 - oy) * rdy;
-    if (near_y > far_y) { t = near_y; near_y = far_y; far_y = t; }
-    bool miss = (near > far_y || near_y > far);
-    if (!miss) {
-        if (near_y > near) near = near_y;
-        if (far_y < far) far = far_y;
-        float near_z = (a2 - oz) * rdz, far_z = (a5 - oz) * rdz;
-        if (near_z > far_z) { t = near_z; near_z = far_z; far_z = t; }
-        miss = (near > far_z || near_z > far);
-        if (!miss) {
-            if (near_z > near) near = near_z;
-            if (far_z < far) far = far_z;
-            if (near < min_near) near = min_near;
-        }
-    }
-    near_out = miss ? FLT_MAX : near;
-    far_out = miss ? FLT_MAX : far;
-}
 
 __global__ void __launch_bounds__(256) k_near_far_from_aabb(const float *__restrict__ rays_o, const float *__restrict__ rays_d,
                                      const float *__restrict__ aabb, uint32_t N, float min_near,
diff --git a/focnerf_amd/csrc/sample_math.h b/focnerf_amd/csrc/sample_math.h
--- a/focnerf_amd/csrc/sample_math.h
+++ b/focnerf_amd/csrc/sample_math.h
@@ -1,5 +1,6 @@
 #pragma once
 #include "common.h"
+#include <float.h>
 
 typedef _Float16 h8 __attribute__((ext_vector_type(8)));
 
@@ -46,6 +47,33 @@
 }
 __device__ __forceinline__ float foc_trunc_exp_bwd_of_sigma(float sigma, const FocExp15 &e) { return fminf(fmaxf(sigma, e.lo), e.hi); }
 
+__device__ __forceinline__ float foc_canon_nan(float x) { return x == x ? x : __builtin_nanf(""); }
+__device__ __forceinline__ _Float16 foc_canon_nan(_Float16 x) { return x == x ? x : (_Float16)__builtin_nanf(""); }
+
+__device__ __forceinline__ void rm_near_far(float ox, float oy, float oz, float dx, float dy, float dz, float a0, float a1, float a2, float a3, float a4, float a5,
+                                            float min_near, float &near_out, float &far_out) {
+    const float rdx = 1 / dx, rdy = 1 / dy, rdz = 1 / dz;
+    float near = (a0 - ox) * rdx, far = (a3 - ox) * rdx, t;
+    if (near > far) { t = near; near = far; far = t; }
+    float near_y = (a1 - oy) * rdy, far_y = (a4 - oy) * rdy;
+    if (near_y > far_y) { t = near_y; near_y = far_y; far_y = t; }
+    bool miss = (near > far_y || near_y > far);
+    if (!miss) {
+        if (near_y > near) near = near_y;
+        if (far_y < far) far = far_y;
+        float near_z = (a2 - oz) * rdz, far_z = (a5 - oz) * rdz;
+        if (near_z > far_z) { t = near_z; near_z = far_z; far_z = t; }
+        miss = (near > far_z || near_z > far);
+        if (!miss) {
+            if (near_z > near) near = near_z;
+            if (far_z < far) far = far_z;
+            if (near < min_near) near = min_near;
+        }
+    }
+    near_out = miss ? FLT_MAX : near;
+    far_out = miss ? FLT_MAX : far;
+}
+
 struct FocBg { float b0, b1, b2; };
 __device__ __forceinline__ FocBg foc_bg(const float *__restrict__ bg_ray, float bg_scalar, uint32_t k) {
     return FocBg{bg_ray ? bg_ray[k * 3] : bg_scalar, bg_ray ? bg_ray[k * 3 + 1] : bg_scalar, bg_ray ? bg_ray[k * 3 + 2] : bg_scalar};
diff --git a/focnerf_amd/fixedstep.py b/focnerf_amd/fixedstep.py
--- a/focnerf_amd/fixedstep.py
+++ b/focnerf_amd/fixedstep.py
@@ -30,6 +30,17 @@
     if want_ray_sh:
         return enc_in, xyzs, ray_sh
     return enc_in, xyzs
+
+
+def fixed_sample_nf(rays_o, rays_d, aabb, min_near, noise, T, bound):
+    N, dev = rays_o.shape[0], rays_o.device
+    nears = torch.empty(N, dtype=torch.float32, device=dev)
+    fars = torch.empty(N, dtype=torch.float32, device=dev)
+    enc_in = torch.empty(N * T, 3, dtype=torch.float32, device=dev)
+    ray_sh = torch.empty(N, 16, dtype=torch.float16, device=dev)
+    check(lib.foc_fixed_sample_nf(ptr(rays_o), ptr(rays_d), ptr(aabb.contiguous()), float(min_near), ptr(noise), N, T, float(bound), ptr(nears), ptr(fars),
+                                  None, ptr(enc_in), ptr(ray_sh), 0, stream_of(rays_o)), "fixed_sample_nf")
+    return nears, fars, enc_in, ray_sh
 
 
 def ray_sh_rows(rays_d):
@@ -125,7 +136,7 @@
 
     @staticmethod
     def forward(ctx, h, cweights, ray_sh, nears, fars, noise, bg_ray, bg_scalar, N, T, density_scale, thresh, num_layers, activation, obj_feat=None,
-                want_sumsq=False, c_pre=None, w16_pre=None, input_pad=0.0, want_dist=False):
+                want_sumsq=False, c_pre=None, w16_pre=None, input_pad=0.0, want_dist=False, lean=False):
         from .field import _half_of, pad_twin, object_feature_half
         h = h.contiguous()
         assert h.dtype == torch.float16 and h.shape == (N * T, 16)
@@ -143,31 +154,38 @@
             args = (ptr(h), ptr(ray_sh), T, ptr(w16), M, 64, int(num_layers), int(activation), ptr(c), _C_WIDTH, ptr(obj16))
             fn, extra = pad_twin("foc_color_head_forward", input_pad, obj16 is not None)
             check(fn(*args, *extra, st), "color_head_forward")
-        sigma = torch.empty(M, dtype=torch.float32, device=dev)
-        trans = torch.empty(M, dtype=torch.float32, device=dev)
-        weights = torch.empty(M, dtype=torch.float32, device=dev)
+        if lean and want_dist:
+            raise RuntimeError("_render_tail: the distortion's kernels read the per-sample weights; lean=True has none")
+        empty = torch.empty(0, device=dev)
+        sigma = torch.empty(M, dtype=torch.float32, device=dev) if not lean else None
+        trans = torch.empty(M, dtype=torch.float32, device=dev) if not lean else None
+        weights = torch.empty(M, dtype=torch.float32, device=dev) if not lean else None
+        h0 = torch.empty(M, dtype=torch.float16, device=dev) if lean else None
         ws = torch.empty(N, dtype=torch.float32, device=dev)
         depth = torch.empty(N, dtype=torch.float32, device=dev)
         image = torch.empty(N, 3, dtype=torch.float32, device=dev)
         sumsq = torch.empty(N, dtype=torch.float32, device=dev) if want_sumsq else None
-        tail = (ptr(h), ptr(c), ptr(nears), ptr(fars), ptr(noise), ptr(bg_ray), float(bg_scalar), N, T, float(density_scale), float(thresh), ptr(sigma),
-                ptr(trans), ptr(weights), ptr(ws), ptr(depth), ptr(image), _C_WIDTH, ptr(sumsq))
+        rays = (ptr(h), ptr(c), ptr(nears), ptr(fars), ptr(noise), ptr(bg_ray), float(bg_scalar), N, T, float(density_scale), float(thresh))
+        tail = rays + (ptr(sigma), ptr(trans), ptr(weights), ptr(ws), ptr(depth), ptr(image), _C_WIDTH, ptr(sumsq))
         dist = wm = None
-        if want_dist:
+        if lean:
+            check(lib.foc_fixed_tail_forward_lean(*rays, ptr(h0), ptr(ws), ptr(depth), ptr(image), _C_WIDTH, ptr(sumsq), st), "fixed_tail_forward_lean")
+        elif want_dist:
             dist, wm = torch.empty(N, dtype=torch.float32, device=dev), torch.empty(N, dtype=torch.float32, device=dev)
             check(lib.foc_fixed_tail_forward_dist(*tail, ptr(dist), ptr(wm), st), "fixed_tail_forward_dist")
         else:
             check(lib.foc_fixed_tail_forward(*tail, st), "fixed_tail_forward")
-        empty = torch.empty(0, device=dev)
         ctx.bg_grad = bg_ray is not None and ctx.needs_input_grad[6]
-        ctx.save_for_backward(h, w16, sigma, trans, weights, c, ray_sh, nears, fars, noise if noise is not None else empty,
+        ctx.save_for_backward(h, w16, h0 if lean else sigma, trans if not lean else empty, weights if not lean else empty, c, ray_sh, nears, fars,
+                              noise if noise is not None else empty,
                               bg_ray if bg_ray is not None else empty, obj16 if obj16 is not None else empty,
                               ws if ctx.bg_grad or want_dist else empty, wm if want_dist else empty)
+        ctx.lean = bool(lean)
         ctx.outputs = (bool(want_sumsq), bool(want_dist))
         ctx.flags = (noise is not None, bg_ray is not None, obj16 is not None, obj_feat.dtype if obj_feat is not None else None,
                      tuple(obj_feat.shape) if obj_feat is not None else None)
         ctx.dims = (N, T, float(density_scale), float(thresh), float(bg_scalar), int(num_layers), int(activation), float(input_pad))
-        ctx.mark_non_differentiable(sigma, weights, c)
+        ctx.mark_non_differentiable(*(t for t in (sigma, weights, c) if t is not None))
         ctx.set_materialize_grads(False)
         return (image, ws, depth, sigma, weights, c) + ((sumsq,) if want_sumsq else ()) + ((dist,) if want_dist else ())
 
@@ -192,7 +210,11 @@
         g_sumsq = g_sumsq.contiguous().float() if g_sumsq is not None else None
         grad_c = torch.empty_like(c)
         grad_h0 = torch.empty(M, dtype=torch.float16, device=dev)
-        if g_dist is not None:
+        if ctx.lean:
+            check(lib.foc_fixed_tail_backward_lean(ptr(g_image), ptr(g_ws), ptr(g_depth), ptr(c), ptr(sigma), ptr(nears), ptr(fars), ptr(noise), ptr(bg_ray),
+                                                   bg_scalar, N, T, ds, thresh, ptr(grad_c), ptr(grad_h0), _C_WIDTH, ptr(g_sumsq), st),
+                  "fixed_tail_backward_lean")
+        elif g_dist is not None:
             g_dist = g_dist.contiguous().float()
             check(lib.foc_fixed_tail_backward_dist(ptr(g_image), ptr(g_ws), ptr(g_depth), ptr(c), ptr(sigma), ptr(trans), ptr(weights), ptr(ws), ptr(nears),
                                                    ptr(fars), ptr(noise), ptr(bg_ray), bg_scalar, N, T, ds, thresh, ptr(grad_c), ptr(grad_h0), _C_WIDTH,
@@ -211,7 +233,7 @@
         check(fn(*args, *extra, st), "color_head_backward")
         g_obj = g_obj32.to(obj_dtype).view(obj_shape) if g_obj32 is not None else None
         g_bg = g_image * (1 - ws).unsqueeze(-1) if ctx.bg_grad else None
-        return (grad_h, g_w, None, None, None, None, g_bg) + (None,) * 7 + (g_obj, None, None, None, None, None)
+        return (grad_h, g_w, None, None, None, None, g_bg) + (None,) * 7 + (g_obj, None, None, None, None, None, None)
 
 
 class _masked_norm(Function):
@@ -263,8 +285,8 @@
     N, T = rays_o.shape[0], int(num_steps)
     dev = rays_o.device
     aabb = model.aabb_train if model.training else model.aabb_infer
-    nears, fars = raymarching.near_far_from_aabb(rays_o, rays_d, aabb, model.min_near)
     noise = torch.rand(N * T, dtype=torch.float32, device=dev) if perturb else None
+    from ._lib import get_option
     from .field import field_plan, field_infer
     plan = field_plan(model)
     if getattr(model, "bg_radius", 0) > 0:
@@ -275,8 +297,13 @@
         raise ValueError("render_fixed_steps: distortion=True needs the training route (gradients enabled): the inference paths form no "
                          "differentiable weights; call it under torch.enable_grad() with model.train()")
     rb = ray_block_default() if fused_infer else 0
-    enc_in, _, ray_sh = fixed_sample(rays_o, rays_d, nears, fars, aabb, noise, T, model.bound, want_ray_sh=True) if want_tail else \
-        fixed_sample(rays_o, rays_d, nears, fars, aabb, noise, T, model.bound, ray_block=rb) + (None,)
+    lean_opt = get_option("FOC_TAIL_LEAN") != 0
+    if want_tail and lean_opt:
+        nears, fars, enc_in, ray_sh = fixed_sample_nf(rays_o, rays_d, aabb, model.min_near, noise, T, model.bound)
+    else:
+        nears, fars = raymarching.near_far_from_aabb(rays_o, rays_d, aabb, model.min_near)
+        enc_in, _, ray_sh = fixed_sample(rays_o, rays_d, nears, fars, aabb, noise, T, model.bound, want_ray_sh=True) if want_tail else \
+            fixed_sample(rays_o, rays_d, nears, fars, aabb, noise, T, model.bound, ray_block=rb) + (None,)
 
     if fused_infer:
         obj_feat = model.encode_object_feature(yolo_details, dev) if plan.uses_object_feature else None
@@ -334,9 +361,10 @@
         if fused_tail:
             cn = fused_mlp(model, "color_net")
             bg_ray, bg_scalar = _background(bg_color, N, dev)
+            lean = lean_opt and not distortion and not return_fields
             outs = _render_tail.apply(h, cweights, ray_sh, nears, fars, noise, bg_ray, bg_scalar, N, T, model.density_scale, weight_thresh,
                                       cn.num_layers, cn.activation, obj_feat, want_crit and yolo_details[0].numel() == N, c_pre,
-                                      wc16 if c_pre is not None else None, plan.colour_input_pad, *((True,) if distortion else ()))
+                                      wc16 if c_pre is not None else None, plan.colour_input_pad, bool(distortion), lean)
             image, weights_sum, depth, sigma, weights, c = outs[:6]
             ray_dist = outs[-1] if distortion else None
             if len(outs) - bool(distortion) == 7:
diff --git a/include/focnerf.h b/include/focnerf.h
--- a/include/focnerf.h
+++ b/include/focnerf.h
@@ -305,6 +305,9 @@
 int foc_fixed_sample(const float *rays_o, const float *rays_d, const float *nears, const float *fars,
                      const float *aabb, const float *noise, uint32_t N, uint32_t T, float bound,
                      float *xyzs, float *enc_in, void *ray_sh, uint32_t ray_block, void *stream);
+int foc_fixed_sample_nf(const float *rays_o, const float *rays_d, const float *aabb, float min_near, const float *noise,
+                        uint32_t N, uint32_t T, float bound, float *nears, float *fars, float *xyzs, float *enc_in,
+                        void *ray_sh, uint32_t ray_block, void *stream);
 
 int foc_fixed_head_forward(const void *h, const float *rays_d, const float *nears, const float *fars,
                            const float *noise, uint32_t N, uint32_t T, float density_scale,
@@ -324,6 +327,13 @@
                             const float *fars, const float *noise, const float *bg_ray, float bg_scalar, uint32_t N,
                             uint32_t T, float density_scale, float thresh, void *grad_c, void *grad_h0, uint32_t c_width,
                             const float *grad_sumsq, void *stream);
+int foc_fixed_tail_forward_lean(const void *h, const void *c, const float *nears, const float *fars, const float *noise,
+                                const float *bg_ray, float bg_scalar, uint32_t N, uint32_t T, float density_scale, float thresh,
+                                void *h0, float *weights_sum, float *depth, float *image, uint32_t c_width, float *ray_sumsq, void *stream);
+int foc_fixed_tail_backward_lean(const float *grad_image, const float *grad_ws, const float *grad_depth, const void *c,
+                                 const void *h0, const float *nears, const float *fars, const float *noise, const float *bg_ray,
+                                 float bg_scalar, uint32_t N, uint32_t T, float density_scale, float thresh, void *grad_c, void *grad_h0,
+                                 uint32_t c_width, const float *grad_sumsq, void *stream);
 
 int foc_occ_tail_forward(const void *h, const void *c, uint32_t c_width, const float *deltas, const int32_t *rays,
                          uint32_t M, uint32_t N, float T_thresh, float density_scale, const float *bg_ray, float bg_scalar,
```

After: 1.391 billion (median of 2 runs). About the same (+0.2%).
